# L0SG/grouped-ssd-pytorch

Measured on AMD Instinct MI355X. Metric: 512x512 4-phase CT img/s (fwd+loss), higher is better.
Workload: dtype f32; 1 GPU; gssdpp (BASELINE configs[2], GSSD++: self-attention + SA-base + 1 DCN layer x 4 deformable groups, dcn_cat_sab) fwd + MultiBoxLoss, train-mode BN, batch 32, [B,12,300,300] slices; batch_per_gpu=32, global_batch=32

## Files before the change

### grouped-ssd-pytorch_amd/gssd/_lib.py

```python
import ctypes as C
import os

import torch

_HERE = os.path.dirname(os.path.abspath(__file__))
LIB_PATH = os.environ.get('GSSD_LIB_PATH') or os.path.join(_HERE, 'lib', 'libgssd_hip.so')

c_fp = C.c_void_p
c_i = C.c_int
c_f = C.c_float
c_d = C.c_double
c_i64 = C.c_int64


class ConvDesc(C.Structure):
    _fields_ = [
        ('in_', c_fp), ('wgt', c_fp), ('bias', c_fp), ('out', c_fp), ('out_b', c_fp), ('alpha', c_fp),
        ('gate', c_fp), ('resid', c_fp), ('out2', c_fp), ('in_scale', c_fp), ('in_shift', c_fp), ('in_pad', c_fp),
        ('stats', c_fp), ('wgt_wino', c_fp), ('pool_sign', c_fp), ('wgt_x6', c_fp), ('wgt_patch', c_fp),
        ('B', c_i), ('H', c_i), ('W', c_i), ('in_stride', c_i), ('in_ch_off', c_i), ('Ho', c_i), ('Wo', c_i),
        ('Cout', c_i), ('groups', c_i), ('cin_g', c_i), ('KH', c_i), ('KW', c_i), ('stride', c_i), ('pad', c_i),
        ('dil', c_i), ('K', c_i), ('wgt_row_stride', c_i), ('out_stride', c_i), ('out_ch_off', c_i),
        ('out_mode', c_i), ('relu', c_i), ('m_per_image', c_i), ('split_n', c_i), ('split_k', c_i),
        ('out_b_stride', c_i), ('flags', c_i), ('stats_rep', c_i),
        ('in_batch_stride', c_i64), ('wgt_batch_stride', c_i64), ('out_batch_stride', c_i64),
        ('outb_batch_stride', c_i64), ('out_off', c_i64), ('outb_off', c_i64),
    ]


class DcnGeom(C.Structure):
    _fields_ = [(n, C.c_int32) for n in ('B', 'H', 'W', 'C', 'x_stride', 'Ho', 'Wo', 'kh', 'kw', 'sh', 'sw', 'ph', 'pw', 'dh', 'dw', 'dg',
                                         'off_stride', 'mask_stride', 'mask_logit')]


class PlanOp(C.Structure):
    _fields_ = [('kind', c_i), ('fn', c_i), ('stream', c_i), ('nargs', c_i), ('args', C.c_uint64 * 24)]


PLAN_LAUNCH, PLAN_WAIT = 0, 1


class SnItem(C.Structure):
    _fields_ = [('w', c_fp), ('u', c_fp), ('v', c_fp), ('inv_sigma', c_fp), ('rows', c_i), ('cols', c_i)]


OUT_NHWC, OUT_TRANSPOSED, OUT_HEADS, OUT_SPLIT_T = 0, 1, 2, 3
CONV_OUT_F32, CONV_OUTB_BF16_PERM32, CONV_HEADS_SLICES, CONV_POOL2, CONV_RESID_F32, CONV_F16_OK = 1, 2, 4, 8, 16, 32
CONV_IN_NCHW3, CONV_OUT_GROUPCAT = 64, 128

SIGNATURES = {
    'gssd_abi_version': (c_i, []),
    'gssd_event_create': (c_i, [C.POINTER(C.c_void_p)]),
    'gssd_event_destroy': (c_i, [c_fp]),
    'gssd_event_record_node': (c_i, [c_fp, c_fp]),
    'gssd_event_elapsed_ms': (c_i, [c_fp, c_fp, C.POINTER(C.c_float)]),
    'gssd_conv_desc_size': (c_i, []),
    'gssd_last_error': (C.c_char_p, []),
    'gssd_build_arch': (C.c_char_p, []),
    'gssd_pack_input_nhwc': (c_i, [c_fp, c_fp, c_i, c_i, c_i, c_i, c_i, c_i, c_fp]),
    'gssd_unpack_nhwc_to_nchw': (c_i, [c_fp, c_fp, c_i, c_i, c_i, c_i, c_i, c_fp]),
    'gssd_pack_conv_weight': (c_i, [c_fp, c_fp, c_i, c_i, c_i, c_i, c_i, c_i, c_fp]),
    'gssd_conv2d_nhwc_f32': (c_i, [C.POINTER(ConvDesc), c_fp]),
    'gssd_conv2d_nhwc_bf16': (c_i, [C.POINTER(ConvDesc), c_fp]),
    'gssd_conv_x6_tile': (c_i, [c_i, c_i, c_i64]),
    'gssd_conv_x6_weight_elems': (c_i64, [c_i, c_i, c_i, c_i, c_i]),
    'gssd_conv_x6_pack_weight': (c_i, [c_fp, c_fp, c_i, c_i, c_i, c_i, c_i, c_i, c_fp]),
    'gssd_conv_x6_takes': (c_i, [C.POINTER(ConvDesc)]),
    'gssd_conv_wino_x6_takes': (c_i, [C.POINTER(ConvDesc)]),
    'gssd_conv_thin_x6_takes': (c_i, [C.POINTER(ConvDesc)]),
    'gssd_conv_thin_nchw3_takes': (c_i, [C.POINTER(ConvDesc)]),
    'gssd_plan_fn_count': (c_i, []),
    'gssd_plan_fn_name': (C.c_char_p, [c_i]),
    'gssd_plan_fn_index': (c_i, [C.c_char_p]),
    'gssd_plan_fn_nargs': (c_i, [c_i]),
    'gssd_plan_op_size': (c_i, []),
    'gssd_plan_run': (c_i, [C.POINTER(PlanOp), c_i, C.POINTER(c_fp), c_i, C.POINTER(c_i)]),
    'gssd_pack_conv_weight_bf16': (c_i, [c_fp, c_fp, c_i, c_i, c_i, c_i, c_i, c_i, c_fp]),
    'gssd_cast_f32_bf16': (c_i, [c_fp, c_fp, c_i64, c_fp]),
    'gssd_cast_rows_f32_bf16': (c_i, [c_fp, c_fp, c_i64, c_i, c_i, c_i, c_fp]),
    'gssd_transpose_cast_f32_bf16': (c_i, [c_fp, c_fp, c_i64, c_i, c_i64, c_i64, c_fp]),
    'gssd_cast_bf16_f32': (c_i, [c_fp, c_fp, c_i64, c_fp]),
    'gssd_pack_input_nhwc_bf16': (c_i, [c_fp, c_fp, c_i, c_i, c_i, c_i, c_i, c_fp]),
    'gssd_bn_relu_pool_bf16': (c_i, [c_fp, c_fp, c_i, c_i, c_i, c_i, c_i, c_i, c_i, c_i, c_i, c_fp, c_d, c_fp, c_fp,
                                     c_fp, c_fp, c_f, c_f, c_i, c_i, c_i, c_fp]),
    'gssd_bn_finalize_bf16': (c_i, [c_fp, c_d, c_fp, c_fp, c_fp, c_fp, c_f, c_f, c_i, c_i, c_fp, c_fp, c_fp, c_i, c_fp]),
    'gssd_l2norm_bf16': (c_i, [c_fp, c_fp, c_fp, c_i64, c_i, c_f, c_fp]),
    'gssd_dcn_packed_weight_elems_bf16': (C.c_longlong, [c_i, c_i]),
    'gssd_dcn_pack_weight_bf16': (c_i, [c_fp, c_fp, c_i, c_i, c_i, c_fp]),
    'gssd_dcn_forward_bf16': (c_i, [c_fp, c_fp, c_fp, c_fp, c_fp, c_i, c_i, c_i, c_i, c_i, c_i, c_i, c_fp]),
    'gssd_winograd_weight_elems': (C.c_longlong, [c_i, c_i, c_i]),
    'gssd_winograd_weight_f32': (c_i, [c_fp, c_fp, c_i, c_i, c_i, c_i, c_fp]),
    'gssd_conv2d_wgrad_f32': (c_i, [C.POINTER(ConvDesc), c_fp, c_fp, c_fp]),
    'gssd_conv2d_wgrad_bf16': (c_i, [C.POINTER(ConvDesc), c_fp, c_fp, c_fp]),
    'gssd_conv2d_wgrad_bf16_supported': (c_i, [C.POINTER(ConvDesc)]),
    'gssd_unpack_conv_weight_grad': (c_i, [c_fp, c_fp, c_i, c_i, c_i, c_i, c_i, c_i, c_i, c_fp]),
    'gssd_pack_conv_weight_dgrad': (c_i, [c_fp, c_fp, c_i, c_i, c_i, c_i, c_i, c_fp]),
    'gssd_bn_relu_pool_f32': (c_i, [c_fp, c_fp, c_i, c_i, c_i, c_i, c_i, c_i, c_i, c_i, c_i, c_fp, c_d, c_fp, c_fp,
                                    c_fp, c_fp, c_f, c_f, c_i, c_i, c_i, c_fp]),
    'gssd_bn_finalize_f32': (c_i, [c_fp, c_d, c_fp, c_fp, c_fp, c_fp, c_f, c_f, c_i, c_i, c_fp, c_fp, c_fp, c_i, c_fp]),
    'gssd_bn_bwd_reduce_f32': (c_i, [c_fp, c_fp, c_fp, c_fp, c_fp, c_fp, c_i, c_i, c_i, c_i, c_i, c_i, c_i, c_i, c_i, c_i, c_fp]),
    'gssd_bn_bwd_finalize_f32': (c_i, [c_fp, c_d, c_fp, c_fp, c_f, c_i, c_fp, c_fp, c_fp, c_fp, c_fp, c_i, c_fp]),
    'gssd_bn_bwd_apply_f32': (c_i, [c_fp, c_fp, c_fp, c_fp, c_fp, c_i64, c_i, c_fp, c_fp]),
    'gssd_bn_bwd_reduce_mixed': (c_i, [c_fp, c_i, c_fp, c_fp, c_fp, c_fp, c_fp, c_fp, c_i, c_i, c_i, c_i, c_i, c_i, c_i, c_i, c_i, c_i, c_fp]),
    'gssd_bn_bwd_apply_mixed': (c_i, [c_fp, c_i, c_fp, c_fp, c_fp, c_fp, c_fp, c_i, c_fp, c_fp, c_fp, c_i64, c_i, c_fp, c_i, c_fp]),
    'gssd_bn_bwd_apply_masked_f32': (c_i, [c_fp, c_fp, c_fp, c_fp, c_i, c_fp, c_fp, c_fp, c_fp, c_i64, c_i, c_fp, c_fp]),
    'gssd_colsum_f32': (c_i, [c_fp, c_i64, c_i, c_i, c_fp, c_fp]),
    'gssd_cast_f64_f32': (c_i, [c_fp, c_fp, c_i, c_i, c_fp]),
    'gssd_l2norm_bwd_f32': (c_i, [c_fp, c_fp, c_fp, c_fp, c_fp, c_fp, c_i64, c_i, c_f, c_fp]),
    'gssd_heads_gather_f32': (c_i, [c_fp, c_fp, c_fp, c_i, c_i, c_i, c_i, c_i, c_i, c_fp]),
    'gssd_upsample_insert_f32': (c_i, [c_fp, c_fp, c_i, c_i, c_i, c_i, c_i, c_i, c_i, c_fp]),
    'gssd_l2norm_f32': (c_i, [c_fp, c_fp, c_fp, c_i64, c_i, c_f, c_fp]),
    'gssd_self_attn_core_f32': (c_i, [c_fp, c_fp, c_fp, c_i, c_i, c_i, c_i, c_i, c_i, c_fp]),
    'gssd_self_attn_core_kv_f32': (c_i, [c_fp, c_fp, c_fp, c_fp, c_i, c_i, c_i, c_i, c_i, c_i, c_i, c_i, c_fp, c_fp]),
    'gssd_sa_pool_kv_f32': (c_i, [c_fp, c_fp, c_fp, c_fp, c_i, c_i, c_i, c_i, c_i, c_i, c_i, c_fp]),
    'gssd_sa_unpool_f32': (c_i, [c_fp, c_fp, c_i, c_i, c_i, c_i, c_i, c_fp]),
    'gssd_pack_conv_weights_batched': (c_i, [c_fp, c_i, c_fp]),
    'gssd_gemm_slot_takes': (c_i, [c_fp]),
    'gssd_conv_flat_bf16_takes': (c_i, [c_fp]),
    'gssd_conv_flat_bf16_tile': (c_i, [c_i]),
    'gssd_heads_reduce_f32': (c_i, [c_fp, c_fp, c_fp, c_i, c_i, c_i, c_fp]),
    'gssd_interp_add_f32': (c_i, [c_fp, c_fp, c_fp, c_fp, c_i, c_i, c_i, c_i, c_i, c_i, c_fp]),
    'gssd_pixellink_final_f32': (c_i, [c_fp, c_fp, c_fp, c_fp, c_i, c_fp, c_fp, c_fp, c_fp, c_fp, c_fp, c_i, c_i, c_fp]),
    'gssd_pixellink_loss_f32': (c_i, [c_fp, c_fp, c_fp, c_fp, c_fp, c_fp, c_fp, c_fp, c_i, c_i, c_i, c_i, c_fp]),
    'gssd_interp_add_bwd_f32': (c_i, [c_fp, c_fp, c_fp, c_fp, c_i, c_i, c_i, c_i, c_i, c_i, c_i, c_fp]),
    'gssd_pixellink_final_bwd_f32': (c_i, [c_fp] * 6 + [c_i, c_fp, c_fp, c_fp, c_fp, c_fp, c_fp, c_i, c_fp, c_fp, c_i, c_i, c_i, c_fp]),
    'gssd_pixellink_loss_bwd_f32': (c_i, [c_fp] * 10 + [c_i, c_i, c_i, c_fp]),
    'gssd_pixellink_decode_f32': (c_i, [c_fp, c_fp, c_fp, c_fp, c_fp, c_i, c_i, c_i, C.c_float, C.c_float, c_i, c_fp]),
    'gssd_self_attn_flash_bwd_bf16': (c_i, [c_fp, c_fp, c_fp, c_fp, c_fp, c_fp, c_fp, c_fp, c_i, c_i, c_i, c_i, c_fp]),
    'gssd_cast_split_f32_bf16': (c_i, [c_fp, c_fp, c_fp, c_i64, c_fp]),
    'gssd_self_attn_flash_bwd_supported': (c_i, [c_i, c_i]),
    'gssd_self_attn_core_x6_supported': (c_i, [c_i, c_i]),
    'gssd_self_attn_core_x6_ws_bytes': (C.c_longlong, [c_i, c_i, c_i, c_i]),
    'gssd_self_attn_core_x6_f32': (c_i, [c_fp, c_fp, c_fp, c_i, c_i, c_i, c_i, c_i, c_fp, c_fp, c_fp]),
    'gssd_self_attn_core_bf16v': (c_i, [c_fp, c_fp, c_fp, c_i, c_i, c_i, c_i, c_i, c_fp, c_fp]),
    'gssd_softmax_rows_f32': (c_i, [c_fp, c_i64, c_i, c_i, c_fp]),
    'gssd_slice_and_cat_f32': (c_i, [c_fp, c_fp, c_fp, c_i64, c_i, c_i, c_i, c_fp]),
    'gssd_spectral_norm_f32': (c_i, [c_fp, c_i, c_i, c_f, c_fp]),
    'gssd_dcn_im2col_f32': (c_i, [c_fp, c_fp, c_fp, c_i, c_i, c_i, c_i, c_i, c_i, c_fp]),
    'gssd_dcn_im2col_bf16': (c_i, [c_fp, c_fp, c_fp, c_i, c_i, c_i, c_i, c_i, c_i, c_fp]),
    'gssd_dcn_packed_weight_elems_x6': (C.c_longlong, [c_i, c_i]),
    'gssd_dcn_pack_weight_x6': (c_i, [c_fp, c_fp, c_i, c_i, c_i, c_fp]),
    'gssd_dcn_forward_x6': (c_i, [c_fp, c_fp, c_fp, c_fp, c_fp, c_i, c_i, c_i, c_i, c_i, c_i, c_i, c_fp]),
    'gssd_conv_patch_x6_weight_elems': (C.c_longlong, [c_i, c_i]),
    'gssd_conv_patch_x6_pack_weight': (c_i, [c_fp, c_fp, c_i, c_i, c_i, c_fp]),
    'gssd_conv_patch_x6_takes': (c_i, [C.POINTER(ConvDesc)]),
    'gssd_dcn_forward_x6_ex': (c_i, [c_fp, c_fp, c_fp, c_fp, c_fp, c_i, c_i, c_i, c_i, c_i, c_i, c_i, c_i, c_fp]),
    'gssd_dcn_packed_weight_elems': (C.c_longlong, [c_i, c_i]),
    'gssd_dcn_pack_weight_f32': (c_i, [c_fp, c_fp, c_i, c_i, c_i, c_fp]),
    'gssd_dcn_streamk': (c_i, [c_i]),
    'gssd_dcn_streamk_status': (c_i, [c_fp]),
    'gssd_dcn_streamk_reset': (c_i, [c_fp]),
    'gssd_dcn_streamk_release': (c_i, [c_fp]),
    'gssd_dcn_forward_f32': (c_i, [c_fp, c_fp, c_fp, c_fp, c_fp, c_i, c_i, c_i, c_i, c_i, c_i, c_i, c_fp]),
    'gssd_resample_ksize': (c_i, [c_i, c_i, c_i]),
    'gssd_resample_coeffs': (c_i, [c_i, c_i, c_i, c_fp, c_fp]),
    'gssd_resize_u8_horizontal': (c_i, [c_fp, c_fp, c_fp, c_fp, c_i, c_i, c_i, c_i, c_i, c_i, c_fp]),
    'gssd_resize_u8_vertical': (c_i, [c_fp, c_fp, c_fp, c_fp, c_i, c_i, c_i, c_i, c_i, c_i, c_i, c_fp, c_fp]),
    'gssd_input_finish_f32': (c_i, [c_fp, c_fp, c_f, c_f, c_f, c_fp, c_i, c_i, c_i, c_i, c_i, c_fp]),
    'gssd_aug_desc_size': (c_i, []),
    'gssd_augment_minmax': (c_i, [c_fp, c_i, c_i, c_i, c_fp, c_fp]),
    'gssd_augment_horizontal': (c_i, [c_fp, c_fp, c_fp, c_f, c_f, c_f, c_fp, c_i, c_i, c_i, c_i, c_i, c_fp]),
    'gssd_augment_vertical': (c_i, [c_fp, c_fp, c_fp, c_fp, c_i, c_i, c_i, c_fp]),
    'gssd_pixellink_targets': (c_i, [c_fp, c_fp, c_i, c_i, c_i, c_fp, c_fp, c_fp, c_fp, c_fp]),
    'gssd_pixellink_final5_f32': (c_i, [c_fp] * 5 + [c_i] + [c_fp] * 6 + [c_i, c_i, c_fp]),
    'gssd_pixellink_final5_bwd_f32': (c_i, [c_fp] * 7 + [c_i] + [c_fp] * 7 + [c_i, c_fp, c_fp, c_i, c_i, c_i, c_fp]),
    'gssd_self_attn_flash_bwd_f32_supported': (c_i, [c_i, c_i]),
    'gssd_self_attn_flash_bwd_f32': (c_i, [c_fp, c_i, c_fp, c_i, c_fp, c_i, c_fp, c_fp, c_fp, c_fp, c_i, c_fp, c_fp, c_i, c_i, c_i, c_i, c_i,
                                           c_i, c_fp]),
    'gssd_eval_match': (c_i, [c_fp, C.c_longlong, c_i, c_i, c_fp, c_fp, c_fp, c_i, c_d, c_fp, c_i, c_i, c_fp, c_fp, c_fp]),
    'gssd_eval_workspace_bytes': (C.c_longlong, [c_i]),
    'gssd_eval_ap': (c_i, [c_fp, c_fp, c_i, c_i, c_d, c_i, c_fp, C.c_longlong, c_fp, c_fp]),
    'gssd_bgemm_f32': (c_i, [c_fp, c_fp, c_fp, c_i, c_i, c_i, c_i, c_i, c_i, c_i, c_i, C.c_longlong, C.c_longlong, C.c_longlong, c_i, c_f,
                             c_i, c_fp]),
    'gssd_softmax_bwd_rows_f32': (c_i, [c_fp, c_fp, c_i64, c_i, c_i, c_fp]),
    'gssd_sn_weight_grad_f32': (c_i, [c_fp, c_i, c_fp, c_fp, c_fp, c_fp, c_fp, c_fp, c_fp, c_i, c_i, c_fp]),
    'gssd_scaled_transpose_f32': (c_i, [c_fp, c_fp, c_fp, c_i, c_i, c_fp]),
    'gssd_dot_f32': (c_i, [c_fp, c_fp, c_i64, c_fp, c_fp]),
    'gssd_rowdot_f32': (c_i, [c_fp, c_fp, c_fp, c_i64, c_i, c_fp]),
    'gssd_bgemm_ex_f32': (c_i, [c_fp, c_fp, c_fp, c_i, c_i, c_i, c_i, c_i, c_i, c_i, c_i, C.c_longlong, C.c_longlong, C.c_longlong, c_i, c_f,
                                c_i, c_fp, c_fp, c_fp]),
    'gssd_axpby_f32': (c_i, [c_fp, c_fp, c_fp, c_i64, c_f, c_f, c_fp]),
    'gssd_scale_cast_f64_f32': (c_i, [c_fp, c_fp, c_fp, c_i, c_fp]),
    'gssd_sa_sigma_grad_f32': (c_i, [c_fp, c_fp, c_fp, c_i, c_fp, c_fp]),
    'gssd_dcn_col2im_f32': (c_i, [c_fp, c_fp, c_fp, c_fp, c_fp, c_i, c_i, c_i, c_i, c_i, c_i, c_fp]),
    'gssd_dcn_geo_im2col_f32': (c_i, [c_fp, c_fp, c_fp, c_fp, C.POINTER(DcnGeom), c_i, c_i, c_fp]),
    'gssd_dcn_geo_col2im_f32': (c_i, [c_fp] * 7 + [C.POINTER(DcnGeom), c_i, c_i, c_fp]),
    'gssd_match_batch': (c_i, [c_fp, c_fp, c_fp, c_i, c_i, c_f, c_f, c_f, c_fp, c_fp, c_fp]),
    'gssd_reduce_max_f32': (c_i, [c_fp, c_i64, c_fp, c_i, c_fp]),
    'gssd_hnm_loss': (c_i, [c_fp, c_fp, c_fp, c_fp, c_fp, c_i, c_i, c_i, c_i, c_i, c_fp, c_fp, c_fp, c_fp]),
    'gssd_loss_finalize': (c_i, [c_fp, c_i, c_fp, c_fp, c_fp]),
    'gssd_loss_finalize_global': (c_i, [c_fp, c_i, c_fp, c_i, c_fp, c_fp, c_fp]),
    'gssd_loss_backward': (c_i, [c_fp, c_fp, c_fp, c_fp, c_fp, c_fp, c_fp, c_fp, c_i, c_i, c_i, c_fp, c_fp, c_fp]),
    'gssd_detect': (c_i, [c_fp, c_fp, c_fp, c_i, c_i, c_i, c_i, c_f, c_f, c_f, c_f, c_i, c_i, c_fp, c_fp, c_fp, c_fp]),
    'gssd_softmax_lastdim_f32': (c_i, [c_fp, c_fp, c_i64, c_i, c_fp]),
}


class GssdError(RuntimeError):
    pass


def _load():
    if not os.path.exists(LIB_PATH):
        raise GssdError(
            f'{LIB_PATH} is missing: the HIP kernels are not built.  Run `make -C '
            f'{os.path.join(_HERE, "csrc")}` (needs hipcc, --offload-arch=gfx950) or '
            f'`python -c "import __graft_entry__ as g; g.build()"`.  There is no CPU fallback.')
    lib = C.CDLL(LIB_PATH)
    for name, (res, args) in SIGNATURES.items():
        try:
            fn = getattr(lib, name)
        except AttributeError as e:
            raise GssdError(f'{LIB_PATH} does not export {name}; rebuild it') from e
        fn.restype = res
        fn.argtypes = args
    if lib.gssd_plan_op_size() != C.sizeof(PlanOp):
        raise GssdError(f'{LIB_PATH}: struct gssd_plan_op is {lib.gssd_plan_op_size()} bytes in the library, {C.sizeof(PlanOp)} in this '
                        f'binding; rebuild the library')
    if lib.gssd_conv_desc_size() != C.sizeof(ConvDesc):
        raise GssdError(f'{LIB_PATH}: struct gssd_conv_desc is {lib.gssd_conv_desc_size()} bytes in the library, '
                        f'{C.sizeof(ConvDesc)} in this binding; rebuild the library')
    return lib


lib = _load()


def check(rc):
    if rc != 0:
        raise GssdError(f'libgssd_hip: error {rc}: {lib.gssd_last_error().decode()}')
```

### grouped-ssd-pytorch_amd/gssd/csrc/conv_bf16.hip

```cpp
#include <stdlib.h>
#include "common.h"
#include "kernel_util.h"

namespace {

constexpr int BK = 64;

__device__ __attribute__((aligned(16))) u16 g_zero_page_h[8] = {0, 0, 0, 0, 0, 0, 0, 0};

template <int BN>
__device__ __forceinline__ int tile_chan_of_row(int row) { return BN < 32 ? row : chan_of_row(row); }

template <int BM, int BN, int WM, int WN, int NSTG>
__global__ __launch_bounds__(WM * WN * 64) void conv_bf16_kernel(const gssd_conv_desc p, const int M, const int tiles_per_group) {
    extern __shared__ __attribute__((aligned(16))) u16 smem_h[];
    constexpr int WTM = BM / WM, WTN = BN / WN, MT = WTM / 16, NT = WTN / 16;
    constexpr int NW = WM * WN, NTHR = NW * 64;
    constexpr int AR = BM / (8 * NW);
    constexpr int BPIECES = BN / 8;
    constexpr int BR = (BPIECES + NW - 1) / NW;
    constexpr int STAGE = (BM + BN) * BK;
    static_assert(NT == 1 || NT % 2 == 0, "channel pairing needs an even tile count per wave");

    const int tid = threadIdx.x, lane = tid & 63;
// ... 308 lines not shown

    if (p.stats) {
        __syncthreads();
        float* red = reinterpret_cast<float*>(smem_h);
#pragma unroll
        for (int u = 0; u < NG; ++u)
#pragma unroll
            for (int c = 0; c < CPL; ++c) {
                float s = ssum[u][c], q = ssq[u][c];
#pragma unroll
                for (int o = 1; o < 16; o <<= 1) {
                    s += __shfl_xor(s, o, 64);
                    q += __shfl_xor(q, o, 64);
                }
                if (r == 0) {
                    const int cl = wn * WTN + (NT == 1 ? 4 * kq : 32 * u + 8 * kq) + c;
                    red[(wm * BN + cl) * 2 + 0] = s;
                    red[(wm * BN + cl) * 2 + 1] = q;
                }
            }
        __syncthreads();
        if (tid < BN && n0g + tid < cout_g) {
            double s = 0.0, q = 0.0;
#pragma unroll
            for (int w = 0; w < WM; ++w) {
                s += (double)red[(w * BN + tid) * 2 + 0];
                q += (double)red[(w * BN + tid) * 2 + 1];
            }
            const int n = g * cout_g + n0g + tid;
            double* st = gssd_stats_replica(p.stats, p.stats_rep, p.Cout);
            unsafeAtomicAdd(st + n, s);
            unsafeAtomicAdd(st + p.Cout + n, q);
        }
    }
}

template <int BM, int BN, int WM, int WN, int NSTG = 2>
int launch_cfg(const gssd_conv_desc& d, int M, int images, hipStream_t stream) {
    static unsigned attr_mask = 0;
    constexpr size_t smem_base = NSTG * (size_t)(BM + BN) * BK * sizeof(u16);
    const size_t smem = smem_base + (d.in_scale ? 2 * (size_t)d.cin_g * sizeof(float) : 0);
    auto kern = conv_bf16_kernel<BM, BN, WM, WN, NSTG>;
    if (const int rc = gssd_max_dynamic_lds(&attr_mask, kern, smem_base + 8192)) return rc;
    const int cout_g = d.Cout / d.groups;
    const int tiles = (cout_g + BN - 1) / BN;
    const int mtiles = (M + BM - 1) / BM;
    dim3 grid = d.m_per_image ? dim3(mtiles, d.groups * tiles, images) : dim3((mtiles + 7) / 8 * 8 * d.groups * tiles, 1, d.split_k);
    hipLaunchKernelGGL(kern, grid, dim3(WM * WN * 64), smem, stream, d, M, tiles);
    GSSD_CHECK_LAUNCH();
    return GSSD_OK;
}

__global__ void pack_weight_bf16_kernel(const float* __restrict__ w, u16* __restrict__ wp, int Cout, int cin_g, int KH, int KW,
                                        int cin_g_pad, int Kpad) {
    const long long total = (long long)Cout * Kpad;
    for (long long i = blockIdx.x * (long long)blockDim.x + threadIdx.x; i < total; i += (long long)gridDim.x * blockDim.x) {
        const int k = (int)(i % Kpad), n = (int)(i / Kpad);
        const int tap = k / cin_g_pad, c = k - tap * cin_g_pad;
        float v = 0.f;
        if (tap < KH * KW && c < cin_g) v = w[((size_t)n * cin_g + c) * KH * KW + tap];
        wp[i] = f2bf(v);
    }
}

__global__ void cast_f32_bf16_kernel(const float* __restrict__ x, u16* __restrict__ y, long long n) {
    for (long long i = blockIdx.x * (long long)blockDim.x + threadIdx.x; i < n; i += (long long)gridDim.x * blockDim.x) y[i] = f2bf(x[i]);
}

__global__ void cast_bf16_f32_kernel(const u16* __restrict__ x, float* __restrict__ y, long long n) {
    const long long n8 = n >> 3;
    for (long long i = blockIdx.x * (long long)blockDim.x + threadIdx.x; i < n8; i += (long long)gridDim.x * blockDim.x) {
        const bf16x8 v = *reinterpret_cast<const bf16x8*>(x + 8 * i);
        f32x4 a, b;
#pragma unroll
        for (int e = 0; e < 4; ++e) {
            a[e] = (float)v[e];
            b[e] = (float)v[e + 4];
        }
        *reinterpret_cast<f32x4*>(y + 8 * i) = a;
        *reinterpret_cast<f32x4*>(y + 8 * i + 4) = b;
    }
    if (blockIdx.x == 0 && threadIdx.x < (n & 7)) y[8 * n8 + threadIdx.x] = bf2f(x[8 * n8 + threadIdx.x]);
}

__global__ void cast_split_bf16_kernel(const float* __restrict__ x, u16* __restrict__ hi, u16* __restrict__ lo, long long n) {
    for (long long i = blockIdx.x * (long long)blockDim.x + threadIdx.x; i < n; i += (long long)gridDim.x * blockDim.x) {
        const float v = x[i];
        const u16 h = f2bf(v);
        hi[i] = h;
        lo[i] = f2bf(v - bf2f(h));
    }
}

__global__ void cast_rows_bf16_kernel(const float* __restrict__ x, u16* __restrict__ y, long long rows, int cols, int ld_x, int ld_y) {
    const long long total = rows * ld_y;
    for (long long i = blockIdx.x * (long long)blockDim.x + threadIdx.x; i < total; i += (long long)gridDim.x * blockDim.x) {
        const long long r = i / ld_y;
        const int c = (int)(i - r * ld_y);
        y[i] = c < cols ? f2bf(x[r * ld_x + c]) : (u16)0;
    }
}

}

extern "C" int gssd_cast_split_f32_bf16(const float* x, void* hi, void* lo, int64_t n, gssd_stream_t stream) {
    GSSD_CHECK_ARG(x && hi && lo && n > 0);
    hipLaunchKernelGGL(cast_split_bf16_kernel, dim3((int)((n + 255) / 256 > 8192 ? 8192 : (n + 255) / 256)), dim3(256), 0, as_stream(stream), x,
                       reinterpret_cast<u16*>(hi), reinterpret_cast<u16*>(lo), (long long)n);
    GSSD_CHECK_LAUNCH();
    return GSSD_OK;
}

extern "C" int gssd_cast_rows_f32_bf16(const float* x, void* y, int64_t rows, int cols, int ld_x, int ld_y, gssd_stream_t stream) {
    GSSD_CHECK_ARG(x && y && rows > 0 && cols > 0 && ld_x >= cols && ld_y >= cols);
    const long long total = rows * ld_y;
    hipLaunchKernelGGL(cast_rows_bf16_kernel, dim3((int)((total + 255) / 256 > 8192 ? 8192 : (total + 255) / 256)), dim3(256), 0,
                       as_stream(stream), x, reinterpret_cast<u16*>(y), (long long)rows, cols, ld_x, ld_y);
    GSSD_CHECK_LAUNCH();
    return GSSD_OK;
}

extern "C" int gssd_cast_bf16_f32(const void* x, float* y, int64_t n, gssd_stream_t stream) {
    GSSD_CHECK_ARG(x && y && n > 0 && ((uintptr_t)x % 16) == 0 && ((uintptr_t)y % 16) == 0);
    const long long thr = (n / 8 + 255) / 256;
    hipLaunchKernelGGL(cast_bf16_f32_kernel, dim3((int)(thr > 16384 ? 16384 : (thr < 1 ? 1 : thr))), dim3(256), 0, as_stream(stream),
                       reinterpret_cast<const u16*>(x), y, (long long)n);
    GSSD_CHECK_LAUNCH();
    return GSSD_OK;
}

extern "C" int gssd_pack_conv_weight_bf16(const float* w_oihw, void* w_packed, int Cout, int cin_g, int KH, int KW, int cin_g_pad,
                                          int Kpad, gssd_stream_t stream) {
    GSSD_CHECK_ARG(w_oihw && w_packed && Cout > 0 && cin_g > 0 && KH > 0 && KW > 0 && cin_g_pad >= cin_g && cin_g_pad % 8 == 0);
    GSSD_CHECK_ARG(Kpad >= KH * KW * cin_g_pad && Kpad % 8 == 0);
    const long long total = (long long)Cout * Kpad;
    hipLaunchKernelGGL(pack_weight_bf16_kernel, dim3((int)((total + 255) / 256 > 8192 ? 8192 : (total + 255) / 256)), dim3(256), 0,
                       as_stream(stream), w_oihw, reinterpret_cast<u16*>(w_packed), Cout, cin_g, KH, KW, cin_g_pad, Kpad);
    GSSD_CHECK_LAUNCH();
    return GSSD_OK;
}

extern "C" int gssd_cast_f32_bf16(const float* x, void* y, int64_t n, gssd_stream_t stream) {
    GSSD_CHECK_ARG(x && y && n > 0);
    hipLaunchKernelGGL(cast_f32_bf16_kernel, dim3((int)((n + 255) / 256 > 8192 ? 8192 : (n + 255) / 256)), dim3(256), 0,
                       as_stream(stream), x, reinterpret_cast<u16*>(y), (long long)n);
    GSSD_CHECK_LAUNCH();
    return GSSD_OK;
}

extern "C" int gssd_conv2d_nhwc_bf16(const gssd_conv_desc* dp, gssd_stream_t stream) {
    GSSD_CHECK_ARG(dp != nullptr);
    const gssd_conv_desc& d = *dp;
    GSSD_CHECK_ARG(d.in && d.wgt && d.out);
    GSSD_CHECK_ARG(!(d.flags & (GSSD_CONV_IN_NCHW3 | GSSD_CONV_OUT_GROUPCAT)));
    GSSD_CHECK_ARG(d.B > 0 && d.H > 0 && d.W > 0 && d.Ho > 0 && d.Wo > 0);
    GSSD_CHECK_ARG(d.groups > 0 && d.Cout > 0 && d.Cout % d.groups == 0);
    GSSD_CHECK_ARG(d.cin_g > 0 && d.cin_g % 8 == 0 && d.in_stride % 8 == 0 && d.in_ch_off % 8 == 0);
    GSSD_CHECK_ARG(d.KH > 0 && d.KW > 0 && d.stride > 0 && d.dil > 0 && d.pad >= 0);
    GSSD_CHECK_ARG(d.K == d.KH * d.KW * d.cin_g && d.wgt_row_stride >= d.K && d.wgt_row_stride % 8 == 0);
    GSSD_CHECK_ARG(((uintptr_t)d.in % 16) == 0 && ((uintptr_t)d.wgt % 16) == 0 && ((uintptr_t)d.out % 16) == 0);
    GSSD_CHECK_ARG(d.out_mode >= 0 && d.out_mode <= 3);
    const bool out_f32 = (d.flags & GSSD_CONV_OUT_F32) != 0;
    if (d.out_mode == GSSD_OUT_TRANSPOSED)
        GSSD_CHECK_ARG(d.m_per_image && out_f32 && d.out_stride % 4 == 0 && d.out_batch_stride % 4 == 0 && !d.gate && !d.resid);
    if (d.out_mode == GSSD_OUT_HEADS) GSSD_CHECK_ARG(d.out_b && d.split_n > 0 && d.split_n < d.Cout && !d.m_per_image && out_f32);
    if (d.out_mode == GSSD_OUT_SPLIT_T) {
        GSSD_CHECK_ARG(d.m_per_image && d.groups == 1 && d.out_b && d.split_n > 0 && d.split_n < d.Cout && d.split_n % 64 == 0 && out_f32);
        GSSD_CHECK_ARG(d.out_b_stride % 4 == 0 && d.out_b_stride >= d.Ho * d.Wo && d.outb_batch_stride % 4 == 0);
        if (d.flags & GSSD_CONV_OUTB_BF16_PERM32) GSSD_CHECK_ARG(d.out_b_stride % 32 == 0 && d.outb_batch_stride % 8 == 0);
        GSSD_CHECK_ARG(!d.gate && !d.resid && !d.relu && !d.stats && d.split_k == 1);
    }
    if (d.out_mode == GSSD_OUT_NHWC) GSSD_CHECK_ARG((d.out_stride % 8 == 0 && d.out_ch_off % 8 == 0) || out_f32);
    if (d.m_per_image) GSSD_CHECK_ARG(d.in_batch_stride % 8 == 0 && d.wgt_batch_stride % 8 == 0);
    GSSD_CHECK_ARG(d.split_k >= 1 && d.split_k <= 64);
    GSSD_CHECK_ARG((d.in_scale == nullptr) == (d.in_shift == nullptr) && (d.in_scale == nullptr) == (d.in_pad == nullptr));
    if (d.split_k > 1)
        GSSD_CHECK_ARG(out_f32 && !d.m_per_image && !d.stats && !d.relu && !d.gate && !d.resid &&
                       (d.out_mode == GSSD_OUT_HEADS || d.out_mode == GSSD_OUT_NHWC));
    GSSD_CHECK_ARG((d.H + 2 * d.pad - d.dil * (d.KH - 1) - 1) / d.stride + 1 == d.Ho);
    GSSD_CHECK_ARG((d.W + 2 * d.pad - d.dil * (d.KW - 1) - 1) / d.stride + 1 == d.Wo);
    const int images = d.m_per_image ? d.B : 1;
    const long long Mll = (long long)(d.m_per_image ? 1 : d.B) * d.Ho * d.Wo;
    GSSD_CHECK_ARG(Mll < (1ll << 31));
    GSSD_CHECK_ARG((long long)(d.m_per_image ? 1 : d.B) * d.H * d.W * d.in_stride < (1ll << 31));
    GSSD_CHECK_ARG((long long)(d.Cout / d.groups + 256) * d.wgt_row_stride < (1ll << 31));
    const int M = (int)Mll;
    const int cout_g = d.Cout / d.groups;
    hipStream_t s = as_stream(stream);
    {
        const int rc = gssd_try_conv_thin_bf16(d, s);
        if (rc != 1) return rc;
    }
    if (d.flags & GSSD_CONV_POOL2) {
        gssd_set_error("GSSD_CONV_POOL2: no bf16 kernel with a pooled epilogue takes this descriptor (thin trunk shapes only)");
        return GSSD_EINVAL;
    }
    {
        const int rc = gssd_try_conv_flat_bf16(d, s);
        if (rc != 1) return rc;
    }
    if (d.in_scale) GSSD_CHECK_ARG(d.cin_g <= 1024 && !d.m_per_image);
    static const bool no_small = getenv("GSSD_NO_SMALL_TILES") != nullptr;
    if (!no_small && cout_g > 32 && d.split_k == 1 && !(d.out_mode == GSSD_OUT_SPLIT_T && d.split_n % 64 != 0)) {
        const long long mtot = (long long)M * images;
        if (mtot <= 512 || (d.m_per_image && mtot <= 4096 && M <= 128)) return launch_cfg<32, 64, 1, 4, 3>(d, M, images, s);
        if (mtot <= 4096) return launch_cfg<64, 64, 2, 2, 3>(d, M, images, s);
    }
    static const int big = [] { const char* e = getenv("GSSD_BF16_BIG_TILES"); return e ? atoi(e) : 0; }();
    if (big && !d.m_per_image && d.split_k == 1 && M >= 8192 && cout_g % 128 == 0 && d.K % BK == 0 && d.K >= 256 &&
        (d.out_mode == GSSD_OUT_NHWC || (d.out_mode == GSSD_OUT_SPLIT_T && d.split_n % 128 == 0))) {
        if (big == 2) return launch_cfg<256, 128, 4, 2, 3>(d, M, images, s);
        if (big == 3) return launch_cfg<192, 128, 4, 2, 3>(d, M, images, s);
        if (big == 4) return launch_cfg<128, 128, 2, 2, 4>(d, M, images, s);
        if (big == 5) return launch_cfg<128, 128, 2, 2, 3>(d, M, images, s);
        if (big == 6) return launch_cfg<128, 128, 4, 2, 4>(d, M, images, s);
        return launch_cfg<256, 128, 4, 2>(d, M, images, s);
    }
    if (cout_g > 64) {
        const long long mt = (M + 127) / 128, z = d.m_per_image ? images : d.split_k;
        const long long b128 = mt * d.groups * ((cout_g + 127) / 128) * z, b64 = mt * d.groups * ((cout_g + 63) / 64) * z;
        const double e128 = (double)b128 / (double)(((b128 + 511) / 512) * 512);
        const double e64 = 0.94 * (double)b64 / (double)(((b64 + 767) / 768) * 768);
        if (e64 > e128 || d.K <= 256 || (d.out_mode == GSSD_OUT_SPLIT_T && d.split_n % 128 != 0)) return launch_cfg<128, 64, 2, 2>(d, M, images, s);
        return launch_cfg<128, 128, 2, 2>(d, M, images, s);
    }
    if (cout_g > 32) return launch_cfg<128, 64, 2, 2>(d, M, images, s);
    if (cout_g > 16) return launch_cfg<128, 32, 4, 1>(d, M, images, s);
    return launch_cfg<128, 16, 4, 1>(d, M, images, s);
}
```

### grouped-ssd-pytorch_amd/gssd/csrc/conv_igemm.hip

```cpp
#include <stdlib.h>
#include "common.h"
#include "kernel_util.h"

namespace {

constexpr int BK = 32;

__device__ __attribute__((aligned(16))) float g_zero_page[4] = {0.f, 0.f, 0.f, 0.f};

template <int BM, int BN, int WM, int WN, int NSTG>
__global__ __launch_bounds__(WM * WN * 64) void conv_igemm_kernel(const gssd_conv_desc p, const int M,
                                                         const int tiles_per_group) {
    extern __shared__ __attribute__((aligned(16))) float smem[];
    constexpr int WTM = BM / WM, WTN = BN / WN, MT = WTM / 16, NT = WTN / 16;
    constexpr int NW = WM * WN, NTHR = NW * 64;
    constexpr int AR = BM / (8 * NW);
    constexpr int BPIECES = BN / 8;
    constexpr int BR = (BPIECES + NW - 1) / NW;
    constexpr int STAGE = (BM + BN) * BK;

    const int tid = threadIdx.x, lane = tid & 63;
    const int wave = __builtin_amdgcn_readfirstlane(tid >> 6);
    const int wm = wave / WN, wn = wave % WN;
    const int r = lane & 15, kq = lane >> 4;
// ... 204 lines not shown
                    f32x4 o;
#pragma unroll
                    for (int e = 0; e < 4; ++e) o[e] = (mb + e < M) ? v[e] : 0.f;
                    *reinterpret_cast<f32x4*>(p.out_b + (size_t)bi * p.outb_batch_stride + (size_t)(n - p.split_n) * p.out_b_stride + ml) = o;
                }
            } else if (p.out_mode == GSSD_OUT_TRANSPOSED) {
                if (mb < p.out_stride) {
                    f32x4 o;
#pragma unroll
                    for (int e = 0; e < 4; ++e) {
                        float t = v[e];
                        if (p.relu) t = fmaxf(t, 0.f);
                        o[e] = (mb + e < M) ? t : 0.f;
                    }
                    *reinterpret_cast<f32x4*>(p.out + (size_t)img * p.out_batch_stride + (size_t)n * p.out_stride + mb) = o;
                }
            } else {
#pragma unroll
                for (int e = 0; e < 4; ++e) {
                    const int m = mb + e;
                    if (m >= M) continue;
                    float t = v[e];
                    if (p.out_mode == GSSD_OUT_HEADS) {
                        const int b = m / HoWo, pix = m - b * HoWo;
                        float* dst = (n < p.split_n)
                                         ? p.out + ((size_t)b * p.out_batch_stride + p.out_off + (size_t)pix * p.split_n + n)
                                         : p.out_b + ((size_t)b * p.outb_batch_stride + p.outb_off +
                                                      (size_t)pix * (p.Cout - p.split_n) + (n - p.split_n));
                        if (p.flags & GSSD_CONV_HEADS_SLICES) {
                            dst[(size_t)kz * ((n < p.split_n) ? (size_t)p.B * p.out_batch_stride
                                                                   : (size_t)p.B * p.outb_batch_stride)] = t;
                        } else if (p.split_k > 1) {
                            unsafeAtomicAdd(dst, t);
                        } else {
                            *dst = t;
                        }
                    } else {
                        const size_t o = (size_t)img * p.out_batch_stride + (size_t)m * p.out_stride + p.out_ch_off + n;
                        if (p.gate) {
                            t *= gate;
                            if (p.out2) p.out2[o] = t;
                            if (p.resid) t += p.resid[o];
                        } else if (p.resid) {
                            t += p.resid[o];
                        }
                        if (p.relu) t = fmaxf(t, 0.f);
                        if (p.split_k > 1) unsafeAtomicAdd(p.out + o, t);
                        else p.out[o] = t;
                    }
                }
            }
        }
    }

    if (p.stats) {
        __syncthreads();
        float* red = smem;
#pragma unroll
        for (int j = 0; j < NT; ++j) {
            float s = ssum[j], q = ssq[j];
            s += __shfl_xor(s, 16, 64);
            s += __shfl_xor(s, 32, 64);
            q += __shfl_xor(q, 16, 64);
            q += __shfl_xor(q, 32, 64);
            if (kq == 0) {
                red[(wm * BN + wn * WTN + j * 16 + r) * 2 + 0] = s;
                red[(wm * BN + wn * WTN + j * 16 + r) * 2 + 1] = q;
            }
        }
        __syncthreads();
        if (tid < BN && n0g + tid < cout_g) {
            double s = 0.0, q = 0.0;
#pragma unroll
            for (int w = 0; w < WM; ++w) {
                s += (double)red[(w * BN + tid) * 2 + 0];
                q += (double)red[(w * BN + tid) * 2 + 1];
            }
            const int n = g * cout_g + n0g + tid;
            double* st = gssd_stats_replica(p.stats, p.stats_rep, p.Cout);
            unsafeAtomicAdd(st + n, s);
            unsafeAtomicAdd(st + p.Cout + n, q);
        }
    }
}

template <int BM, int BN, int WM, int WN, int NSTG = 2>
int launch_cfg(const gssd_conv_desc& d, int M, int images, hipStream_t stream) {
    static unsigned attr_mask = 0;
    constexpr size_t smem_base = NSTG * (size_t)(BM + BN) * BK * sizeof(float);
    const size_t smem = smem_base + (d.in_scale ? 2 * (size_t)d.cin_g * sizeof(float) : 0);
    auto kern = conv_igemm_kernel<BM, BN, WM, WN, NSTG>;
    if (const int rc = gssd_max_dynamic_lds(&attr_mask, kern, smem_base + 4096)) return rc;
    const int cout_g = d.Cout / d.groups;
    const int tiles = (cout_g + BN - 1) / BN;
    const int mtiles = (M + BM - 1) / BM;
    dim3 grid = d.m_per_image ? dim3(mtiles, d.groups * tiles, images) : dim3((mtiles + 7) / 8 * 8 * d.groups * tiles, 1, d.split_k);
    static_assert(BM % (8 * WM * WN) == 0, "A rows must split evenly over the waves");
    hipLaunchKernelGGL(kern, grid, dim3(WM * WN * 64), smem, stream, d, M, tiles);
    GSSD_CHECK_LAUNCH();
    return GSSD_OK;
}

}

extern "C" int gssd_conv2d_nhwc_f32(const gssd_conv_desc* dp, gssd_stream_t stream) {
    GSSD_CHECK_ARG(dp != nullptr);
    const gssd_conv_desc& d = *dp;
    GSSD_CHECK_ARG(d.in && d.wgt && d.out);
    GSSD_CHECK_ARG(d.B > 0 && d.H > 0 && d.W > 0 && d.Ho > 0 && d.Wo > 0);
    GSSD_CHECK_ARG(d.groups > 0 && d.Cout > 0 && d.Cout % d.groups == 0);
    GSSD_CHECK_ARG(d.cin_g > 0 && d.cin_g % 4 == 0 && d.in_stride % 4 == 0 && d.in_ch_off % 4 == 0);
    GSSD_CHECK_ARG(d.KH > 0 && d.KW > 0 && d.stride > 0 && d.dil > 0 && d.pad >= 0);
    GSSD_CHECK_ARG(d.K == d.KH * d.KW * d.cin_g && d.wgt_row_stride >= d.K && d.wgt_row_stride % 4 == 0);
    GSSD_CHECK_ARG(((uintptr_t)d.in % ((d.flags & GSSD_CONV_IN_NCHW3) ? 4 : 16)) == 0 && ((uintptr_t)d.wgt % 16) == 0);
    GSSD_CHECK_ARG(d.out_mode >= 0 && d.out_mode <= 3);
    if (d.out_mode == GSSD_OUT_SPLIT_T) {
        GSSD_CHECK_ARG((d.m_per_image || (d.Ho * d.Wo) % 4 == 0) && d.groups == 1 && d.out_b && d.split_n > 0 && d.split_n < d.Cout &&
                       d.split_n % 64 == 0);
        GSSD_CHECK_ARG(d.out_b_stride % 4 == 0 && d.out_b_stride >= d.Ho * d.Wo && d.outb_batch_stride % 4 == 0 && ((uintptr_t)d.out_b % 16) == 0);
        GSSD_CHECK_ARG(!d.gate && !d.resid && !d.relu && !d.stats && d.split_k == 1);
    }
    if (d.out_mode == GSSD_OUT_TRANSPOSED) {
        GSSD_CHECK_ARG(d.m_per_image && d.out_stride % 4 == 0 && ((uintptr_t)d.out % 16) == 0);
        GSSD_CHECK_ARG(d.out_batch_stride % 4 == 0 && !d.gate && !d.resid);
    }
    if (d.out_mode == GSSD_OUT_HEADS) GSSD_CHECK_ARG(d.out_b && d.split_n > 0 && d.split_n < d.Cout && !d.m_per_image);
    if (d.m_per_image) GSSD_CHECK_ARG(d.in_batch_stride % 4 == 0 && d.wgt_batch_stride % 4 == 0);
    GSSD_CHECK_ARG(d.split_k >= 1 && d.split_k <= 64);
    GSSD_CHECK_ARG((d.in_scale == nullptr) == (d.in_shift == nullptr) && (d.in_scale == nullptr) == (d.in_pad == nullptr));
    if (d.split_k > 1) GSSD_CHECK_ARG(!d.m_per_image && !d.stats && !d.relu && !d.gate && !d.resid && d.out_mode != GSSD_OUT_TRANSPOSED);
    GSSD_CHECK_ARG((d.H + 2 * d.pad - d.dil * (d.KH - 1) - 1) / d.stride + 1 == d.Ho);
    GSSD_CHECK_ARG((d.W + 2 * d.pad - d.dil * (d.KW - 1) - 1) / d.stride + 1 == d.Wo);

    const int images = d.m_per_image ? d.B : 1;
    const long long Mll = (long long)(d.m_per_image ? 1 : d.B) * d.Ho * d.Wo;
    GSSD_CHECK_ARG(Mll < (1ll << 31));
    GSSD_CHECK_ARG((long long)(d.m_per_image ? 1 : d.B) * d.H * d.W * d.in_stride < (1ll << 31));
    GSSD_CHECK_ARG((long long)(d.Cout / d.groups + 256) * d.wgt_row_stride < (1ll << 31));
    const int M = (int)Mll;
    const int cout_g = d.Cout / d.groups;
    hipStream_t s = as_stream(stream);
    if (d.flags & GSSD_CONV_IN_NCHW3) {
        const int rc = gssd_try_conv_thin(d, s);
        if (rc != 1) return rc;
        gssd_set_error("GSSD_CONV_IN_NCHW3: not conv1_1's shape (see gssd_conv_thin_nchw3_takes)");
        return GSSD_EINVAL;
    }
    if (d.flags & GSSD_CONV_OUT_GROUPCAT) {
        const int rc = d.wgt_x6 ? gssd_try_conv_x6(d, s) : 1;
        if (rc != 1) return rc;
        gssd_set_error("GSSD_CONV_OUT_GROUPCAT: csrc/conv_x6.hip does not take this descriptor (see gssd_conv_x6_takes)");
        return GSSD_EINVAL;
    }
    if (d.wgt_patch) {
        const int rc = gssd_try_conv_patch_x6(d, s);
        if (rc != 1) return rc;
    }
    if (d.wgt_x6) {
        const int rc = gssd_try_conv_x6(d, s);
        if (rc != 1) return rc;
    }
    {
        const int rc = gssd_try_conv_thin_x6(d, s);
        if (rc != 1) return rc;
    }
    {
        const int rc = gssd_try_conv_thin_wino(d, s);
        if (rc != 1) return rc;
    }
    {
        const int rc = gssd_try_conv_thin(d, s);
        if (rc != 1) return rc;
    }
    {
        const int rc = gssd_try_conv_wino(d, s);
        if (rc != 1) return rc;
    }
    if (d.flags & GSSD_CONV_POOL2) {
        gssd_set_error("GSSD_CONV_POOL2: no fp32 kernel with a pooled epilogue takes this descriptor (Winograd trunk shapes only)");
        return GSSD_EINVAL;
    }
    if (d.in_scale) GSSD_CHECK_ARG(d.cin_g <= 512 && !d.m_per_image);
    {
        static const bool no_slot = getenv("GSSD_NO_GEMM_SLOT") != nullptr;
        const int rc = no_slot ? 1 : gssd_try_gemm_slot(d, s);
        if (rc != 1) return rc;
    }
    static const bool no_small = getenv("GSSD_NO_SMALL_TILES") != nullptr;
    if (!no_small && cout_g > 32 && d.split_k == 1 && !(d.out_mode == GSSD_OUT_SPLIT_T && d.split_n % 64 != 0)) {
        const long long mtot = (long long)M * images;
        if (mtot <= 512 || (d.m_per_image && mtot <= 4096 && M <= 128)) return launch_cfg<32, 64, 1, 4, 3>(d, M, images, s);
        if (mtot <= 4096) return launch_cfg<64, 64, 2, 2, 3>(d, M, images, s);
    }
    if (cout_g > 64) {
        const long long mt = (M + 127) / 128, z = d.m_per_image ? images : d.split_k;
        const long long b128 = mt * d.groups * ((cout_g + 127) / 128) * z, b64 = mt * d.groups * ((cout_g + 63) / 64) * z;
        const double e128 = (double)b128 / (double)(((b128 + 511) / 512) * 512);
        const double e64 = 0.94 * (double)b64 / (double)(((b64 + 767) / 768) * 768);
        if (e64 > e128 || d.K <= 256 || (d.out_mode == GSSD_OUT_SPLIT_T && d.split_n % 128 != 0)) return launch_cfg<128, 64, 2, 2>(d, M, images, s);
        return launch_cfg<128, 128, 2, 2>(d, M, images, s);
    }
    if (cout_g > 32) return launch_cfg<128, 64, 2, 2>(d, M, images, s);
    if (cout_g > 16) return launch_cfg<128, 32, 4, 1>(d, M, images, s);
    return launch_cfg<128, 16, 4, 1>(d, M, images, s);
}
```

### grouped-ssd-pytorch_amd/gssd/csrc/conv_x6.hip

```cpp
#include <stdlib.h>
#include <type_traits>
#include "common.h"
#include "kernel_util.h"

namespace {

#ifndef X6_SCHED
#define X6_SCHED 0
#endif
#ifndef X6_KO
#define X6_KO 0
#endif
#ifndef X6_LOCAL_SUM
#define X6_LOCAL_SUM 1
#endif
constexpr int BM = 128, BKC = 32;
constexpr int NP = 3;
constexpr int A_STAGE = BM * BKC;


#ifndef X6_V2
#define X6_V2 1
#endif

// ... 145 lines not shown
        }
    };

    gather_issue(gvA, gokA, false);
    b_issue(0, 0);
    if (nchunks > 1) advance_ld();
    if (xf) __syncthreads();
#pragma unroll
    for (int part = 0; part < 4; ++part) finish_part(part, gvA, gokA, 0);
    if (nchunks > 1) advance_fin();
    gather_issue(gvA, gokA, false);
    if (nchunks > 2) advance_ld();
    __syncthreads();

    auto chunk = [&](const int ch, f32x4 (&gv_use)[2][2], const bool (&gok_use)[2], f32x4 (&gv_ld)[2][2], bool (&gok_ld)[2]) {
        const int buf = ch & 1;
        const u16* Ab = As + buf * NP * A_STAGE + wm * WTM * BKC + fo;
        const u16* Bb = Bs + (NBS == 2 ? buf : 0) * NP * B_STAGE + wn * WTN * BKC + fo;
        bf16x8 afr[2][NP], bf[NP][NT];
        auto a_row = [&](int i) {
#pragma unroll
            for (int pl = 0; pl < NP; ++pl) {
                if (X6_KO & 16) asm volatile("" : "=v"(afr[i & 1][pl]));
                else afr[i & 1][pl] = *reinterpret_cast<const bf16x8*>(Ab + pl * A_STAGE + i * 16 * BKC);
            }
        };
        a_row(0);
#pragma unroll
        for (int pl = 0; pl < NP; ++pl) {
#pragma unroll
            for (int j = 0; j < NT; ++j) {
                if (X6_KO & 16) {
                    asm volatile("" : "=v"(bf[pl][j]));
                    continue;
                }
                bf[pl][j] = *reinterpret_cast<const bf16x8*>(Bb + pl * B_STAGE + j * 16 * BKC);
            }
        }
        if (NBS == 1) {
            asm volatile("s_waitcnt lgkmcnt(0)" ::: "memory");
            __builtin_amdgcn_s_barrier();
        }
        b_issue(min(ch + 1, nchunks - 1), buf ^ 1);
        __builtin_amdgcn_sched_barrier(0);
        gather_issue(gv_ld, gok_ld, true);
        if (!(X6_KO & 8)) {
            constexpr int YOUNGER = ((X6_KO & 4) ? 0 : NP * (B_STAGE / 512 / 4)) + 4;
            asm volatile("s_waitcnt vmcnt(%4)" : "+v"(gv_use[0][0]), "+v"(gv_use[0][1]), "+v"(gv_use[1][0]), "+v"(gv_use[1][1]) : "n"(YOUNGER));
        }
        __builtin_amdgcn_sched_barrier(0);
#pragma unroll
        for (int i = 0; i < MT; ++i) {
            if (i + 1 < MT) a_row(i + 1);
            const bf16x8 (&af)[NP] = afr[i & 1];
#pragma unroll
            for (int j = 0; j < NT; ++j) {
                if (X6_KO & 2) continue;
#if X6_LOCAL_SUM
                f32x4 c = zero4;
#else
                f32x4 c = acc[i][j];
#endif
                c = __builtin_amdgcn_mfma_f32_16x16x32_bf16(bf[1][j], af[1], c, 0, 0, 0);
                c = __builtin_amdgcn_mfma_f32_16x16x32_bf16(bf[2][j], af[0], c, 0, 0, 0);
                c = __builtin_amdgcn_mfma_f32_16x16x32_bf16(bf[0][j], af[2], c, 0, 0, 0);
                c = __builtin_amdgcn_mfma_f32_16x16x32_bf16(bf[1][j], af[0], c, 0, 0, 0);
                c = __builtin_amdgcn_mfma_f32_16x16x32_bf16(bf[0][j], af[1], c, 0, 0, 0);
                c = __builtin_amdgcn_mfma_f32_16x16x32_bf16(bf[0][j], af[0], c, 0, 0, 0);
#if X6_LOCAL_SUM
#pragma unroll
                for (int e = 0; e < 4; ++e) acc[i][j][e] += c[e];
#else
                acc[i][j] = c;
#endif
            }
            finish_part(i, gv_use, gok_use, buf ^ 1);
        }
#if X6_SCHED
#define X6_ROW(DS_READS)                                                                                                   \
    __builtin_amdgcn_sched_group_barrier(0x100, DS_READS, 0);                     \
    _Pragma("unroll") for (int k = 0; k < NT * 6; ++k) {                                                                   \
        __builtin_amdgcn_sched_group_barrier(0x008, 1, 0);                                                                 \
        __builtin_amdgcn_sched_group_barrier(0x002, BN == 64 ? X6_SCHED + 2 : BN == 128 ? X6_SCHED + 1 : X6_SCHED, 0);     \
    }                                                                                                                      \
    __builtin_amdgcn_sched_group_barrier(0x200, NP, 0);
        static_assert(MT == 4, "the schedule below is written for four fragment rows");
        X6_ROW(NP + (XF ? 2 : 0))
        X6_ROW(NP + (XF ? 2 : 0))
        X6_ROW(NP + (XF ? 2 : 0))
        X6_ROW((XF ? 2 : 0))
#undef X6_ROW
#endif
        __builtin_amdgcn_sched_barrier(0);
        if (ch + 2 < nchunks) advance_fin();
        if (ch + 3 < nchunks) advance_ld();
        if (X6_KO & 8) asm volatile("s_waitcnt vmcnt(0) lgkmcnt(0)\n\ts_barrier" ::: "memory");
        else asm volatile("s_waitcnt vmcnt(4) lgkmcnt(0)\n\ts_barrier" ::: "memory");
    };
    for (int ch = 0; ch < nchunks; ch += 2) {
        chunk(ch, gvA, gokA, gvB, gokB);
        if (ch + 1 < nchunks) chunk(ch + 1, gvB, gokB, gvA, gokA);
    }
    asm volatile("s_waitcnt vmcnt(0)" : "+v"(gvA[0][0]), "+v"(gvA[0][1]), "+v"(gvA[1][0]), "+v"(gvA[1][1]),
                                        "+v"(gvB[0][0]), "+v"(gvB[0][1]), "+v"(gvB[1][0]), "+v"(gvB[1][1]) : : "memory");
    __syncthreads();

    float* red = reinterpret_cast<float*>(smem_h);
    const float gate = p.gate ? *p.gate : 0.f;
    const bool split_t = p.out_mode == GSSD_OUT_SPLIT_T && n0g >= p.split_n;
    const bool gcat = (p.flags & GSSD_CONV_OUT_GROUPCAT) != 0;
#pragma unroll
    for (int u = 0; u < NT / 2; ++u) {
        const int nl = wn * WTN + 32 * u + 8 * kq;
        const int ng = n0g + nl;
        const bool n_ok = ng + 8 <= cout_g;
        const int n = g * cout_g + ng;
        const int ncat = gcat ? (n / p.split_n) * p.split_n : 0;
        float bv[8], av[8], ssum[8], ssq[8];
#pragma unroll
        for (int c = 0; c < 8; ++c) {
            bv[c] = (p.bias && n_ok) ? p.bias[n + c] : 0.f;
            av[c] = (p.alpha && n_ok) ? p.alpha[n + c] : 1.f;
            ssum[c] = ssq[c] = 0.f;
        }
#pragma unroll
        for (int i = 0; i < MT; ++i) {
            const int m = m0 + wm * WTM + i * 16 + r;
            if (m >= M || !n_ok) continue;
            float v[8];
#pragma unroll
            for (int c = 0; c < 8; ++c) {
                v[c] = acc[i][2 * u + (c >> 2)][c & 3] * av[c] + bv[c];
                ssum[c] += v[c];
                ssq[c] += v[c] * v[c];
            }
            if (split_t) {
                const int bi = m / HoWo, ml = m - bi * HoWo;
                float* dst = p.out_b + (size_t)bi * p.outb_batch_stride + (size_t)(n - p.split_n) * p.out_b_stride + ml;
#pragma unroll
                for (int c = 0; c < 8; ++c) dst[(size_t)c * p.out_b_stride] = v[c];
                continue;
            }
            const size_t o = (size_t)m * p.out_stride + p.out_ch_off + n + ncat;
            const size_t ro = gcat ? (size_t)m * p.Cout + n : o;
            if (p.gate) {
#pragma unroll
                for (int c = 0; c < 8; ++c) v[c] *= gate;
                if (p.out2) {
                    *reinterpret_cast<f32x4*>(p.out2 + o) = f32x4{v[0], v[1], v[2], v[3]};
                    *reinterpret_cast<f32x4*>(p.out2 + o + 4) = f32x4{v[4], v[5], v[6], v[7]};
                }
            }
            if (p.resid) {
                const f32x4 r0 = *reinterpret_cast<const f32x4*>(p.resid + ro), r1 = *reinterpret_cast<const f32x4*>(p.resid + ro + 4);
#pragma unroll
                for (int c = 0; c < 4; ++c) {
                    v[c] += r0[c];
                    v[4 + c] += r1[c];
                }
            }
            if (p.relu) {
#pragma unroll
                for (int c = 0; c < 8; ++c) v[c] = fmaxf(v[c], 0.f);
            }
            *reinterpret_cast<f32x4*>(p.out + o) = f32x4{v[0], v[1], v[2], v[3]};
            *reinterpret_cast<f32x4*>(p.out + o + 4) = f32x4{v[4], v[5], v[6], v[7]};
        }
        if (p.stats) {
#pragma unroll
            for (int c = 0; c < 8; ++c) {
                float s = ssum[c], q = ssq[c];
#pragma unroll
                for (int o = 1; o < 16; o <<= 1) {
                    s += __shfl_xor(s, o, 64);
                    q += __shfl_xor(q, o, 64);
                }
                if (r == 0) {
                    red[(wm * BN + nl + c) * 2 + 0] = s;
                    red[(wm * BN + nl + c) * 2 + 1] = q;
                }
            }
        }
    }
    if (p.stats) {
        __syncthreads();
        if (tid < BN && n0g + tid < cout_g) {
            const double s = (double)red[tid * 2 + 0] + (double)red[(BN + tid) * 2 + 0];
            const double q = (double)red[tid * 2 + 1] + (double)red[(BN + tid) * 2 + 1];
            const int n = g * cout_g + n0g + tid;
            double* st = gssd_stats_replica(p.stats, p.stats_rep, p.Cout);
            unsafeAtomicAdd(st + n, s);
            unsafeAtomicAdd(st + p.Cout + n, q);
        }
    }
}

#if X6_V2
template <int BN>
struct Cfg2 {
    static constexpr int WTN = BN / 2, NT = WTN / 16, NTH = NT / 2, MT = 4;
    static constexpr int NG = NTH * MT;
    static constexpr int HB_ROWS = BN / 2, HB_PLANE = HB_ROWS * BKC, HB_ELEMS = NP * HB_PLANE;
    static constexpr int PH = NP * HB_ROWS / 16;
    static constexpr int DPW = 2 * PH / 4;
    static constexpr int NY = (PH + 3) / 4;
    static constexpr int LDS_BYTES = (NP * A_STAGE + 4 * HB_ELEMS) * 2;
    static_assert(BN == 64 || BN == 128, "tiles");
};

template <int BN, bool XF, bool F16>
__global__ __launch_bounds__(256, 2) void conv_x6_v2_kernel(const gssd_conv_desc p, const int M, const int ntn, const int mtiles,
                                                           const long long plane_elems) {
    using K = Cfg2<BN>;
    constexpr int NPL = (F16 && BN == 64) ? 2 : NP;
    constexpr int WTM = 64, WTN = K::WTN, MT = K::MT, NT = K::NT, NTH = K::NTH, NG = K::NG;
    constexpr int PH = NPL * K::HB_ROWS / 16;
    constexpr int DPW = 2 * PH / 4;
    constexpr int NY = (PH + 3) / 4;
    constexpr int HB_PLANE = K::HB_PLANE, HB_ELEMS = K::HB_ELEMS, B_STAGE = BN * BKC;
    extern __shared__ __attribute__((aligned(16))) u16 smem_h[];
    u16* const As = smem_h;
    u16* const Bh = smem_h + NP * A_STAGE;
    float* const xtab = reinterpret_cast<float*>(smem_h + NP * A_STAGE + 4 * HB_ELEMS);
    const int tid = threadIdx.x, lane = tid & 63;
    const int wave = __builtin_amdgcn_readfirstlane(tid >> 6);
    const int wm = wave >> 1, wn = wave & 1;
    const int r = lane & 15, kq = lane >> 4;
    const int ny = p.groups * ntn;
    const int slot = blockIdx.x >> 3;
    const int mt = (slot / ny) * 8 + (blockIdx.x & 7);
    const int by = slot % ny;
    if (mt >= mtiles) return;
    const int g = by / ntn, nt = by - g * ntn;
    const int cout_g = p.Cout / p.groups;
    const int n0g = nt * BN;
    const int m0 = mt * BM;
    const int HoWo = p.Ho * p.Wo;
    const int taps = p.KH * p.KW;
    const int cpc = p.cin_g / BKC;
    const int nchunks = cpc * taps;
    const float* __restrict__ in = p.in + p.in_ch_off + g * p.cin_g;
    const u16* wslab = reinterpret_cast<const u16*>(p.wgt_x6) + (F16 ? 3 * plane_elems : 0) + (size_t)by * nchunks * B_STAGE;
    constexpr bool xf = XF;

    f32x4 acc[MT][NT];
    const f32x4 zero4 = {0.f, 0.f, 0.f, 0.f};
#pragma unroll
    for (int i = 0; i < MT; ++i)
#pragma unroll
        for (int j = 0; j < NT; ++j) acc[i][j] = zero4;

    const int gq = tid & 3, gp = tid >> 2;
    const int a_wr0 = gp * BKC + ((gq ^ swz64(gp)) << 3);
    const int fo = r * BKC + ((kq ^ swz64(r)) << 3);
    int g_iy0[2], g_ix0[2], g_off[2];
#pragma unroll
    for (int j = 0; j < 2; ++j) {
        const int m = m0 + gp + 64 * j;
        const bool ok = m < M;
        const int mm = ok ? m : 0;
        const int b = mm / HoWo, pix = mm - b * HoWo;
        const int oy = pix / p.Wo, ox = pix - oy * p.Wo;
        g_iy0[j] = ok ? oy * p.stride - p.pad : -(1 << 20);
        g_ix0[j] = ox * p.stride - p.pad;
        g_off[j] = ((b * p.H + oy * p.stride - p.pad) * p.W + g_ix0[j]) * p.in_stride + gq * 8;
    }
    if (xf) {
        const float* xsc = p.in_scale + p.in_ch_off + g * p.cin_g;
        const float* xsh = p.in_shift + p.in_ch_off + g * p.cin_g;
        for (int c = tid; c < p.cin_g; c += 256) {
            xtab[c] = xsc[c];
            xtab[p.cin_g + c] = xsh[c];
        }
    }

    int ld_ty = 0, ld_tx = 0, ld_c = 0, ld_tap = 0;
    f32x4 gv[2][2];
    bool gok[2] = {false, false};
    const float* src[2] = {in, in};
    gv[0][0] = gv[0][1] = gv[1][0] = gv[1][1] = zero4;
    auto load_addr = [&]() {
        const int dy = ld_ty * p.dil, dx = ld_tx * p.dil;
        const int toff = (dy * p.W + dx) * p.in_stride + ld_c * BKC;
#pragma unroll
        for (int j = 0; j < 2; ++j) {
            gok[j] = (unsigned)(g_iy0[j] + dy) < (unsigned)p.H && (unsigned)(g_ix0[j] + dx) < (unsigned)p.W;
            src[j] = in + (gok[j] ? g_off[j] + toff : gq * 8);
        }
    };
    auto load_req = [&](int q) {
        if (X6_KO & 8) return;
        const int j = q >> 1;
        if (q & 1) asm volatile("global_load_dwordx4 %0, %1, off offset:16" : "=v"(gv[j][1]) : "v"(src[j]) : "memory");
        else asm volatile("global_load_dwordx4 %0, %1, off" : "=v"(gv[j][0]) : "v"(src[j]) : "memory");
    };
    int fin_c = 0;
    auto advance_ld = [&]() {
        ++ld_tap;
        if (++ld_tx == p.KW) {
            ld_tx = 0;
            ++ld_ty;
        }
        if (ld_tap == taps) {
            ld_tap = ld_ty = ld_tx = 0;
            ++ld_c;
        }
    };
// ... 88 lines not shown
        }
    };
    auto mma_row = [&](int i, int j, int which) {
        if (X6_KO & 2) return;
#if X6_LOCAL_SUM
        f32x4 c = zero4;
#else
        f32x4 c = acc[i][j];
#endif
        if constexpr (F16) {
            c = __builtin_amdgcn_mfma_f32_16x16x32_f16(__builtin_bit_cast(f16x8, breg[which][2]), __builtin_bit_cast(f16x8, areg[i][1]), c, 0, 0, 0);
            c = __builtin_amdgcn_mfma_f32_16x16x32_f16(__builtin_bit_cast(f16x8, breg[which][1]), __builtin_bit_cast(f16x8, areg[i][2]), c, 0, 0, 0);
            c = __builtin_amdgcn_mfma_f32_16x16x32_f16(__builtin_bit_cast(f16x8, breg[which][0]), __builtin_bit_cast(f16x8, areg[i][0]), c, 0, 0, 0);
        } else {
            c = __builtin_amdgcn_mfma_f32_16x16x32_bf16(breg[which][1], areg[i][1], c, 0, 0, 0);
            c = __builtin_amdgcn_mfma_f32_16x16x32_bf16(breg[which][2], areg[i][0], c, 0, 0, 0);
            c = __builtin_amdgcn_mfma_f32_16x16x32_bf16(breg[which][0], areg[i][2], c, 0, 0, 0);
            c = __builtin_amdgcn_mfma_f32_16x16x32_bf16(breg[which][1], areg[i][0], c, 0, 0, 0);
            c = __builtin_amdgcn_mfma_f32_16x16x32_bf16(breg[which][0], areg[i][1], c, 0, 0, 0);
            c = __builtin_amdgcn_mfma_f32_16x16x32_bf16(breg[which][0], areg[i][0], c, 0, 0, 0);
        }
#if X6_LOCAL_SUM
#pragma unroll
        for (int e = 0; e < 4; ++e) acc[i][j][e] += c[e];
#else
        acc[i][j] = c;
#endif
    };
    constexpr int NGQ = (X6_KO & 8) ? 0 : 4, NDQ = (X6_KO & 4) ? 0 : DPW, NYQ = (X6_KO & 4) ? 0 : NY;
#define X6_LOADS_WAIT(N) \
    if (!(X6_KO & 8)) asm volatile("s_waitcnt vmcnt(%4)" : "+v"(gv[0][0]), "+v"(gv[0][1]), "+v"(gv[1][0]), "+v"(gv[1][1]) : "n"(N))

    load_addr();
#pragma unroll
    for (int q = 0; q < 4; ++q) load_req(q);
    if (xf) __syncthreads();
    if (!(X6_KO & 4)) {
        for (int pc = wave; pc < PH; pc += 4) {
            const int pl = pc / (2 * NTH), g8 = pc - pl * (2 * NTH);
            const int G = (g8 / NTH) * NT + (g8 % NTH);
            dma16(wslab + (size_t)pl * plane_elems + G * 512 + lane * 8, Bh + pl * HB_PLANE + g8 * 512);
        }
    }
    asm volatile("s_waitcnt vmcnt(0)" : "+v"(gv[0][0]), "+v"(gv[0][1]), "+v"(gv[1][0]), "+v"(gv[1][1]));
#pragma unroll
    for (int part = 0; part < 4; ++part) finish_part(part);
    if (nchunks > 1) {
        advance_ld();
    }
    asm volatile("s_waitcnt vmcnt(0) lgkmcnt(0)" ::: "memory");
    __syncthreads();

    auto iteration = [&](int it, auto first_c, auto last_c) {
        constexpr bool FIRST = decltype(first_c)::value, LAST = decltype(last_c)::value;
        const int par = it & 1;
        const int cy = min(it, nchunks - 1), cx = min(it + 1, nchunks - 1);
        __builtin_amdgcn_sched_barrier(0);
        if (!FIRST) {
#pragma unroll
            for (int jj = 0; jj < NTH; ++jj) {
                if (jj + 1 == NTH && !LAST) {
                    constexpr int K_B1 = NTH == 1 ? 0 : NYQ + NGQ;
                    if (X6_KO & 64) asm volatile("s_waitcnt vmcnt(%0) lgkmcnt(0)" ::"n"(K_B1) : "memory");
                    else asm volatile("s_waitcnt vmcnt(%0) lgkmcnt(0)\n\ts_barrier" ::"n"(K_B1) : "memory");
                }
                if (jj + 1 < NTH) b_load((jj + 1) & 1, 1, par ^ 1, jj + 1);
#pragma unroll
                for (int i = 0; i < MT; ++i) {
                    const int gidx = jj * MT + i;
                    if (!LAST && gidx == 0) load_addr();
                    if (jj + 1 == NTH && !LAST && i == 0) b_load((jj + 1) & 1, 0, par, 0);
                    mma_row(i, NTH + jj, jj & 1);
                    if (!LAST) {
                        if (NTH == 2) {
                            if (gidx < NY) dma_piece(gidx, cy, cx, par);
                            if (gidx < 4) load_req(gidx);
                            if (gidx >= 4 && gidx < 4 + DPW - NY) dma_piece(gidx - 4 + NY, cy, cx, par);
                        } else {
                            if (gidx < NY) dma_piece(gidx, cy, cx, par);
                            if (gidx < 2) {
                                load_req(2 * gidx);
                                load_req(2 * gidx + 1);
                            }
                            if (gidx >= NY && gidx < DPW) dma_piece(gidx, cy, cx, par);
                        }
                        if (jj + 1 == NTH) a_load_row(i);
                    }
                    __builtin_amdgcn_sched_barrier(0);
                }
            }
        } else {
            load_addr();
#pragma unroll
            for (int q = 0; q < NY; ++q) dma_piece(q, cy, cx, par);
#pragma unroll
            for (int q = 0; q < 4; ++q) load_req(q);
#pragma unroll
            for (int q = NY; q < DPW; ++q) dma_piece(q, cy, cx, par);
#pragma unroll
            for (int i = 0; i < MT; ++i) a_load_row(i);
            b_load(NTH & 1, 0, par, 0);
        }
        if (!LAST) {
#pragma unroll
            for (int jj = 0; jj < NTH; ++jj) {
                if (jj + 1 < NTH) b_load((NTH + jj + 1) & 1, 0, par, jj + 1);
#pragma unroll
                for (int i = 0; i < MT; ++i) {
                    const int gidx = jj * MT + i;
                    mma_row(i, jj, (NTH + jj) & 1);
                    if (gidx == 0) {
                        __builtin_amdgcn_sched_barrier(0);
                        constexpr int K_B2 = NDQ - NYQ;
                        if (X6_KO & 64) asm volatile("s_waitcnt vmcnt(%0) lgkmcnt(0)" ::"n"(K_B2) : "memory");
                        else asm volatile("s_waitcnt vmcnt(%0) lgkmcnt(0)\n\ts_barrier" ::"n"(K_B2) : "memory");
                        X6_LOADS_WAIT(DPW - NY);
                    }
#ifndef X6_FIN
#define X6_FIN 1
#endif
                    if (NTH == 2) {
                        if (X6_FIN) {
                            if (gidx == 1) finish_part(0);
                            if (gidx == 3) finish_part(1);
                            if (gidx == 5) finish_part(2);
                            if (gidx == 7) finish_part(3);
                        } else {
                            if (gidx == 1) finish_part(0);
                            if (gidx == 2) finish_part(1);
                            if (gidx == 4) finish_part(2);
                            if (gidx == 5) finish_part(3);
                        }
                    } else {
                        if (gidx == 1) finish_part(0), finish_part(1);
                        if (gidx == 2) finish_part(2);
                        if (gidx == 3) finish_part(3);
                    }
                    if (gidx == NG - 1) b_load(0, 1, par, 0);
                    if (!(X6_FIN && NTH == 2) || (gidx & 1) == 0 || gidx == NG - 1) __builtin_amdgcn_sched_barrier(0);
                }
            }
            if (it + 2 < nchunks) advance_ld();
            fin_c = ld_c;
        }
    };
    fin_c = ld_c;
    iteration(0, std::true_type{}, std::false_type{});
    for (int it = 1; it < nchunks; ++it) iteration(it, std::false_type{}, std::false_type{});
    iteration(nchunks, std::false_type{}, std::true_type{});
    asm volatile("s_waitcnt vmcnt(0) lgkmcnt(0)" : "+v"(gv[0][0]), "+v"(gv[0][1]), "+v"(gv[1][0]), "+v"(gv[1][1]) : : "memory");
    __syncthreads();
#undef X6_LOADS_WAIT

    float* red = reinterpret_cast<float*>(smem_h);
    const float gate = p.gate ? *p.gate : 0.f;
    const bool split_t = p.out_mode == GSSD_OUT_SPLIT_T && n0g >= p.split_n;
    const bool gcat = (p.flags & GSSD_CONV_OUT_GROUPCAT) != 0;
#pragma unroll
    for (int u = 0; u < NT / 2; ++u) {
        const int nl = wn * WTN + 32 * u + 8 * kq;
        const int ng = n0g + nl;
        const bool n_ok = ng + 8 <= cout_g;
        const int n = g * cout_g + ng;
        const int ncat = gcat ? (n / p.split_n) * p.split_n : 0;
        float bv[8], av[8], ssum[8], ssq[8];
#pragma unroll
        for (int c = 0; c < 8; ++c) {
            bv[c] = (p.bias && n_ok) ? p.bias[n + c] : 0.f;
            av[c] = (p.alpha && n_ok) ? p.alpha[n + c] : 1.f;
            ssum[c] = ssq[c] = 0.f;
        }
#pragma unroll
        for (int i = 0; i < MT; ++i) {
            const int m = m0 + wm * WTM + i * 16 + r;
            if (m >= M || !n_ok) continue;
            float v[8];
#pragma unroll
            for (int c = 0; c < 8; ++c) {
                v[c] = acc[i][2 * u + (c >> 2)][c & 3] * av[c] + bv[c];
                ssum[c] += v[c];
                ssq[c] += v[c] * v[c];
            }
            if (split_t) {
                const int bi = m / HoWo, ml = m - bi * HoWo;
                float* dst = p.out_b + (size_t)bi * p.outb_batch_stride + (size_t)(n - p.split_n) * p.out_b_stride + ml;
#pragma unroll
                for (int c = 0; c < 8; ++c) dst[(size_t)c * p.out_b_stride] = v[c];
                continue;
            }
            const size_t o = (size_t)m * p.out_stride + p.out_ch_off + n + ncat;
            const size_t ro = gcat ? (size_t)m * p.Cout + n : o;
            if (p.gate) {
#pragma unroll
                for (int c = 0; c < 8; ++c) v[c] *= gate;
                if (p.out2) {
                    *reinterpret_cast<f32x4*>(p.out2 + o) = f32x4{v[0], v[1], v[2], v[3]};
                    *reinterpret_cast<f32x4*>(p.out2 + o + 4) = f32x4{v[4], v[5], v[6], v[7]};
                }
            }
            if (p.resid) {
                const f32x4 r0 = *reinterpret_cast<const f32x4*>(p.resid + ro), r1 = *reinterpret_cast<const f32x4*>(p.resid + ro + 4);
#pragma unroll
                for (int c = 0; c < 4; ++c) {
                    v[c] += r0[c];
                    v[4 + c] += r1[c];
                }
            }
            if (p.relu) {
#pragma unroll
                for (int c = 0; c < 8; ++c) v[c] = fmaxf(v[c], 0.f);
            }
            *reinterpret_cast<f32x4*>(p.out + o) = f32x4{v[0], v[1], v[2], v[3]};
            *reinterpret_cast<f32x4*>(p.out + o + 4) = f32x4{v[4], v[5], v[6], v[7]};
        }
        if (p.stats) {
#pragma unroll
            for (int c = 0; c < 8; ++c) {
                float s = ssum[c], q = ssq[c];
#pragma unroll
                for (int o = 1; o < 16; o <<= 1) {
                    s += __shfl_xor(s, o, 64);
                    q += __shfl_xor(q, o, 64);
                }
                if (r == 0) {
                    red[(wm * BN + nl + c) * 2 + 0] = s;
                    red[(wm * BN + nl + c) * 2 + 1] = q;
                }
            }
        }
    }
    if (p.stats) {
        __syncthreads();
        if (tid < BN && n0g + tid < cout_g) {
            const double s = (double)red[tid * 2 + 0] + (double)red[(BN + tid) * 2 + 0];
            const double q = (double)red[tid * 2 + 1] + (double)red[(BN + tid) * 2 + 1];
            const int n = g * cout_g + n0g + tid;
            double* st = gssd_stats_replica(p.stats, p.stats_rep, p.Cout);
            unsafeAtomicAdd(st + n, s);
            unsafeAtomicAdd(st + p.Cout + n, q);
        }
    }
}

#endif

__global__ void conv_x6_pack_kernel(const float* __restrict__ w, u16* __restrict__ wp, int Cout, int groups, int cin_g, int taps, int row_stride,
                                    int BN, long long total) {
    const int cout_g = Cout / groups, ntn = (cout_g + BN - 1) / BN, nchunks = (cin_g / BKC) * taps;
    for (long long i = blockIdx.x * (long long)blockDim.x + threadIdx.x; i < total; i += (long long)gridDim.x * blockDim.x) {
        const int e = (int)(i & 7);
        const int slot = (int)((i >> 3) & 3);
        const int row = (int)((i >> 5) % BN);
        long long t = (i >> 5) / BN;
        const int chunk = (int)(t % nchunks);
        t /= nchunks;
        const int nt = (int)(t % ntn), g = (int)(t / ntn);
        const int q = slot ^ swz64(row);
        const int tap = chunk % taps, c32 = chunk / taps;
        const int c = c32 * BKC + q * 8 + e;
        const int ng = nt * BN + chan_of_row(row);
        const float v = ng < cout_g ? w[(size_t)(g * cout_g + ng) * row_stride + tap * cin_g + c] : 0.f;
        __bf16 h, m, l;
        split3(v, h, m, l);
        wp[i] = __builtin_bit_cast(u16, h);
        wp[i + total] = __builtin_bit_cast(u16, m);
        wp[i + 2 * total] = __builtin_bit_cast(u16, l);
        const _Float16 fh = (_Float16)v;
        wp[i + 3 * total] = __builtin_bit_cast(u16, fh);
        wp[i + 4 * total] = __builtin_bit_cast(u16, (_Float16)((v - (float)fh) * 64.f));
        wp[i + 5 * total] = __builtin_bit_cast(u16, (_Float16)(fh * (_Float16)0.015625f));
    }
}

template <int BN, bool XF>
int launch(const gssd_conv_desc& d, int M, hipStream_t stream) {
    static unsigned attr_mask = 0;
    auto kern = conv_x6_kernel<BN, XF>;
    if (const int rc = gssd_max_dynamic_lds(&attr_mask, kern, Cfg<BN>::LDS_BYTES + 4096)) return rc;
    const int cout_g = d.Cout / d.groups;
    const int ntn = (cout_g + BN - 1) / BN, mtiles = (M + BM - 1) / BM;
    const long long plane = (long long)d.groups * ntn * BN * d.KH * d.KW * d.cin_g;
    hipLaunchKernelGGL(kern, dim3((mtiles + 7) / 8 * 8 * d.groups * ntn), dim3(256), Cfg<BN>::LDS_BYTES + (d.in_scale ? 8 * d.cin_g : 0), stream, d, M, ntn, mtiles, plane);
    GSSD_CHECK_LAUNCH();
    return GSSD_OK;
}

#if X6_V2
template <int BN, bool XF, bool F16>
int launch2_impl(const gssd_conv_desc& d, int M, hipStream_t stream) {
    static unsigned attr_mask = 0;
    auto kern = conv_x6_v2_kernel<BN, XF, F16>;
    constexpr int lds = Cfg2<BN>::LDS_BYTES;
    if (const int rc = gssd_max_dynamic_lds(&attr_mask, kern, lds + 4096)) return rc;
    const int cout_g = d.Cout / d.groups;
    const int ntn = (cout_g + BN - 1) / BN, mtiles = (M + BM - 1) / BM;
    const long long plane = (long long)d.groups * ntn * BN * d.KH * d.KW * d.cin_g;
    hipLaunchKernelGGL(kern, dim3((mtiles + 7) / 8 * 8 * d.groups * ntn), dim3(256), lds + (d.in_scale ? 8 * d.cin_g : 0), stream, d, M, ntn, mtiles, plane);
    GSSD_CHECK_LAUNCH();
    return GSSD_OK;
}
template <int BN, bool XF>
int launch2(const gssd_conv_desc& d, int M, hipStream_t stream) {
    if (gssd_x6_f16_enabled() && (d.flags & GSSD_CONV_F16_OK)) return launch2_impl<BN, XF, true>(d, M, stream);
    return launch2_impl<BN, XF, false>(d, M, stream);
}
#endif

bool shape_ok(int cin_g, int cout_g, int groups) {
    return cin_g > 0 && cin_g % BKC == 0 && cout_g >= 32 && cout_g % 8 == 0 && groups > 0;
}

}

extern "C" int gssd_conv_x6_tile(int cout_g, int groups, long long M) {
    static const int forced = getenv("GSSD_X6_BN") ? atoi(getenv("GSSD_X6_BN")) : 0;
    if (forced == 64 || forced == 128 || forced == 256) return forced;
    (void)groups;
    (void)M;
    return cout_g > 64 ? 128 : 64;
}

extern "C" long long gssd_conv_x6_weight_elems(int Cout, int groups, int cin_g, int taps, int BN) {
    if (Cout <= 0 || groups <= 0 || Cout % groups != 0 || taps <= 0 || !(BN == 64 || BN == 128 || BN == 256)) return -1;
    if (!shape_ok(cin_g, Cout / groups, groups)) return -1;
    const int cout_g = Cout / groups;
    return 6ll * groups * ((cout_g + BN - 1) / BN) * BN * taps * cin_g;
}

extern "C" int gssd_conv_x6_pack_weight(const float* w_packed, void* w_x6, int Cout, int groups, int cin_g, int taps, int row_stride, int BN,
                                        gssd_stream_t stream) {
    const long long n = gssd_conv_x6_weight_elems(Cout, groups, cin_g, taps, BN);
    GSSD_CHECK_ARG(w_packed && w_x6 && n > 0 && row_stride >= taps * cin_g);
    const long long total = n / 6;
    hipLaunchKernelGGL(conv_x6_pack_kernel, dim3((int)((total + 255) / 256 > 16384 ? 16384 : (total + 255) / 256)), dim3(256), 0,
                       as_stream(stream), w_packed, reinterpret_cast<u16*>(w_x6), Cout, groups, cin_g, taps, row_stride, BN, total);
    GSSD_CHECK_LAUNCH();
    return GSSD_OK;
}

extern "C" int gssd_conv_x6_takes(const gssd_conv_desc* dp) {
    if (!dp) return 0;
    const gssd_conv_desc& d = *dp;
    if (!d.wgt_x6 || d.groups <= 0 || d.Cout % d.groups != 0) return 0;
    if (!shape_ok(d.cin_g, d.Cout / d.groups, d.groups)) return 0;
    if (d.split_k > 1 || (d.flags & ~(GSSD_CONV_OUT_F32 | GSSD_CONV_F16_OK | GSSD_CONV_OUT_GROUPCAT)) || (d.out2 && !d.gate)) return 0;
    if (d.flags & GSSD_CONV_OUT_GROUPCAT) {
        if (d.out_mode != GSSD_OUT_NHWC || d.groups != 1 || d.m_per_image || d.relu || d.stats || d.split_n <= 0 || d.split_n % 8 != 0 ||
            d.Cout % d.split_n != 0 || d.out_stride < 2 * d.Cout)
            return 0;
    }
    if (d.out_mode == GSSD_OUT_SPLIT_T) {
        const int bn = gssd_conv_x6_tile(d.Cout / d.groups, d.groups, (long long)d.B * d.Ho * d.Wo);
        if (d.groups != 1 || !d.out_b || d.split_n <= 0 || d.split_n % bn != 0 || d.out_b_stride < d.Ho * d.Wo) return 0;
    } else if (d.out_mode != GSSD_OUT_NHWC) {
        return 0;
    }
    if (d.m_per_image) {
        if (d.wgt_batch_stride != 0 || d.in_batch_stride != (long long)d.H * d.W * d.in_stride ||
            d.out_batch_stride != (long long)d.Ho * d.Wo * d.out_stride)
            return 0;
    }
    if ((d.resid && ((uintptr_t)d.resid % 16)) || (d.out2 && ((uintptr_t)d.out2 % 16))) return 0;
    if (d.in_stride % 4 || d.in_ch_off % 4 || d.out_stride % 4 || d.out_ch_off % 4) return 0;
    if (((uintptr_t)d.in % 16) || ((uintptr_t)d.out % 16) || ((uintptr_t)d.wgt_x6 % 16)) return 0;
    if ((long long)d.B * d.H * d.W * d.in_stride >= (1ll << 31)) return 0;
    if (d.in_scale && d.cin_g > 512) return 0;
    return 1;
}

int gssd_try_conv_x6(const gssd_conv_desc& d, hipStream_t stream) {
    if (!gssd_conv_x6_takes(&d)) return 1;
    const long long Mll = (long long)d.B * d.Ho * d.Wo;
    const int M = (int)Mll;
    switch (gssd_conv_x6_tile(d.Cout / d.groups, d.groups, Mll)) {
#if X6_V2
        case 64: return d.in_scale ? launch2<64, true>(d, M, stream) : launch2<64, false>(d, M, stream);
        case 128: return d.in_scale ? launch2<128, true>(d, M, stream) : launch2<128, false>(d, M, stream);
#else
        case 64: return d.in_scale ? launch<64, true>(d, M, stream) : launch<64, false>(d, M, stream);
        case 128: return d.in_scale ? launch<128, true>(d, M, stream) : launch<128, false>(d, M, stream);
#endif
        default: return d.in_scale ? launch<256, true>(d, M, stream) : launch<256, false>(d, M, stream);
    }
}
```

### grouped-ssd-pytorch_amd/gssd/csrc/flash_attn_x6.hip

```cpp
#include <math.h>
#include <stdlib.h>
#include "common.h"
#include "kernel_util.h"

namespace {

constexpr int NP = 3;

__device__ __attribute__((aligned(16))) u16 g_zero16_x6[8] = {0, 0, 0, 0, 0, 0, 0, 0};

template <bool F16>
__global__ void split_planes_kernel(const float* __restrict__ in, u16* __restrict__ out, long long rows, int cols, int ld_in, int cols_out,
                                    long long plane, int perm32) {
    const long long i = blockIdx.x * (long long)blockDim.x + threadIdx.x;
    const int units = cols_out >> 3;
    if (i >= rows * units) return;
    const long long row = i / units;
    const int u = (int)(i - row * units);
    const float* src = in + row * ld_in;
    bf16x8 h, m, l;
#pragma unroll
    for (int e = 0; e < 8; ++e) {
        int c = 8 * u + e;
        if (perm32) {
// ... 140 lines not shown
        float mx = -INFINITY;
#pragma unroll
        for (int kt = 0; kt < KT; ++kt)
#pragma unroll
            for (int e = 0; e < 4; ++e) {
                if (key0 + kt * 16 + 4 * kq + e >= N) s[kt][e] = -INFINITY;
                mx = fmaxf(mx, s[kt][e]);
            }
        mx = fmaxf(mx, __shfl_xor(mx, 16, 64));
        mx = fmaxf(mx, __shfl_xor(mx, 32, 64));
        const float m_new = fmaxf(m_run, mx);
        const float alpha = __expf(m_run - m_new);
        float psum = 0.f;
        bf16x8 pb[KB][NPX];
        if constexpr (F16) {
#pragma unroll
            for (int kb = 0; kb < KB; ++kb) {
                u32x4 ph, pl;
#pragma unroll
                for (int e2 = 0; e2 < 4; ++e2) {
                    const float p0 = __expf(s[2 * kb + (e2 >> 1)][(2 * e2) & 3] - m_new), p1 = __expf(s[2 * kb + (e2 >> 1)][(2 * e2 + 1) & 3] - m_new);
                    psum += p0;
                    psum += p1;
                    const f32x2 ps = f32x2{p0, p1} * 1024.f;
                    unsigned h, l;
                    split2_pair(ps[0], ps[1], h, l);
                    ph[e2] = h;
                    pl[e2] = l;
                }
                pb[kb][0] = __builtin_bit_cast(bf16x8, ph);
                pb[kb][1] = __builtin_bit_cast(bf16x8, pl);
            }
        } else {
#pragma unroll
            for (int kb = 0; kb < KB; ++kb)
#pragma unroll
                for (int e = 0; e < 8; ++e) {
                    const float p = __expf(s[2 * kb + (e >> 2)][e & 3] - m_new);
                    psum += p;
                    __bf16 h, m, l;
                    split3(p, h, m, l);
                    pb[kb][0][e] = h;
                    pb[kb][1][e] = m;
                    pb[kb][NPX - 1][e] = l;
                }
        }
        l_run = l_run * alpha + psum;
        m_run = m_new;
        if (__any(alpha != 1.f)) {
#pragma unroll
            for (int c = 0; c < CT; ++c) o[c] *= alpha;
        }
#pragma unroll
        for (int c = 0; c < CT; ++c) {
            const int row = c * 16 + r;
            f32x4 acc = zero4, accx = zero4;
#pragma unroll
            for (int kb = 0; kb < KB; ++kb) {
                bf16x8 vf[NPX];
                const int unit = (4 * kb + kq) ^ (BKV == 32 ? ((row & 8) ? 3 : 0) : (row & 7));
#pragma unroll
                for (int pl = 0; pl < NPX; ++pl) vf[pl] = *reinterpret_cast<const bf16x8*>(Vs + pl * V_PLANE + row * BKV + (unit << 3));
                if constexpr (F16) {
                    accx = __builtin_amdgcn_mfma_f32_16x16x32_f16(__builtin_bit_cast(f16x8, vf[1]), __builtin_bit_cast(f16x8, pb[kb][0]), accx, 0, 0, 0);
                    accx = __builtin_amdgcn_mfma_f32_16x16x32_f16(__builtin_bit_cast(f16x8, vf[0]), __builtin_bit_cast(f16x8, pb[kb][1]), accx, 0, 0, 0);
                    acc = __builtin_amdgcn_mfma_f32_16x16x32_f16(__builtin_bit_cast(f16x8, vf[0]), __builtin_bit_cast(f16x8, pb[kb][0]), acc, 0, 0, 0);
                } else {
                    acc = __builtin_amdgcn_mfma_f32_16x16x32_bf16(vf[1], pb[kb][1], acc, 0, 0, 0);
                    acc = __builtin_amdgcn_mfma_f32_16x16x32_bf16(vf[NPX - 1], pb[kb][0], acc, 0, 0, 0);
                    acc = __builtin_amdgcn_mfma_f32_16x16x32_bf16(vf[0], pb[kb][NPX - 1], acc, 0, 0, 0);
                    acc = __builtin_amdgcn_mfma_f32_16x16x32_bf16(vf[1], pb[kb][0], acc, 0, 0, 0);
                    acc = __builtin_amdgcn_mfma_f32_16x16x32_bf16(vf[0], pb[kb][1], acc, 0, 0, 0);
                    acc = __builtin_amdgcn_mfma_f32_16x16x32_bf16(vf[0], pb[kb][0], acc, 0, 0, 0);
                }
            }
#pragma unroll
            for (int e = 0; e < 4; ++e) o[c][e] += F16 ? __builtin_fmaf(accx[e], 1.f / 2048.f, acc[e]) : acc[e];
            if (F16 && (c & 1)) __builtin_amdgcn_sched_barrier(0);
            if (FX6_SPREAD)
#pragma unroll
                for (int j = 0; j < VW; ++j)
                    if (j * (3 * CT / 4) / VW == c) {
                        __builtin_amdgcn_sched_barrier(0);
                        stage_piece(tn, buf ^ 1, KW + j);
                        __builtin_amdgcn_sched_barrier(0);
                    }
        }
    }
    l_run += __shfl_xor(l_run, 16, 64);
    l_run += __shfl_xor(l_run, 32, 64);
    const float inv = (F16 ? 1.f / 1024.f : 1.f) / l_run;
    if (lse != nullptr && q < N && kq == 0) lse[(size_t)b * N + q] = m_run + logf(l_run);
    if (q < N) {
        float* dst = out + ((size_t)b * N + q) * C2 + 4 * kq;
#pragma unroll
        for (int c = 0; c < CT; ++c) *reinterpret_cast<f32x4*>(dst + 16 * c) = o[c] * inv;
    }
}

template <int D, int C2, int BKV, int NW, bool F16>
int launch_x6(const u16* tpp, const u16* gp, float* out, int B, int N, int Np32, float* lse, hipStream_t stream) {
    constexpr int smem = 2 * (F16 ? 2 : 3) * (BKV * D + C2 * BKV) * (int)sizeof(u16);
    static unsigned attr_mask = 0;
    auto kern = flash_attn_x6_kernel<D, C2, BKV, NW, F16>;
    if (const int rc = gssd_max_dynamic_lds(&attr_mask, kern, smem)) return rc;
    const int qtiles = (N + 16 * NW - 1) / (16 * NW);
    hipLaunchKernelGGL(kern, dim3(B * qtiles), dim3(64 * NW), smem, stream, tpp, gp, out, N, Np32, qtiles, (long long)B * N * 2 * D,
                       (long long)B * C2 * Np32, lse);
    GSSD_CHECK_LAUNCH();
    return GSSD_OK;
}

inline long long round32(long long n) { return (n + 31) / 32 * 32; }

}

extern "C" int gssd_self_attn_core_x6_supported(int D, int C2) { return D == 64 && C2 == 256; }

extern "C" long long gssd_self_attn_core_x6_ws_bytes(int B, int N, int D, int C2) {
    if (B <= 0 || N <= 0 || !gssd_self_attn_core_x6_supported(D, C2)) return -1;
    return 2ll * NP * ((long long)B * N * 2 * D + (long long)B * C2 * round32(N));
}

extern "C" int gssd_self_attn_core_x6_f32(const float* tp, const float* gT, float* out, int B, int N, int Np, int D, int C2, void* ws,
                                          float* lse, gssd_stream_t stream) {
    GSSD_CHECK_ARG(tp && gT && out && ws && B > 0 && N > 0 && Np >= N && Np % 4 == 0);
    GSSD_CHECK_ARG(((uintptr_t)tp % 16) == 0 && ((uintptr_t)gT % 16) == 0 && ((uintptr_t)out % 16) == 0 && ((uintptr_t)ws % 16) == 0);
    GSSD_CHECK_ARG((long long)B * ((N + 63) / 64) < (1ll << 31));
    if (!gssd_self_attn_core_x6_supported(D, C2)) {
        gssd_set_error("self-attention core (three-plane): unsupported (theta/phi channels %d, g channels %d); built: (64,256)", D, C2);
        return GSSD_EINVAL;
    }
    hipStream_t s = as_stream(stream);
    const int Np32 = (int)round32(N);
    u16* tpp = reinterpret_cast<u16*>(ws);
    const long long tp_plane = (long long)B * N * 2 * D, g_plane = (long long)B * C2 * Np32;
    u16* gp = tpp + NP * tp_plane;
    static const bool f16 = [] { const char* e = getenv("GSSD_FLASH_X6_F16"); return e && e[0] == '1'; }();
    {
        const long long n = (long long)B * N * (2 * D / 8);
        if (f16) hipLaunchKernelGGL(split_planes_kernel<true>, dim3((unsigned)((n + 255) / 256)), dim3(256), 0, s, tp, tpp, (long long)B * N, 2 * D, 2 * D, 2 * D, tp_plane, 0);
        else hipLaunchKernelGGL(split_planes_kernel<false>, dim3((unsigned)((n + 255) / 256)), dim3(256), 0, s, tp, tpp, (long long)B * N, 2 * D, 2 * D, 2 * D, tp_plane, 0);
        GSSD_CHECK_LAUNCH();
    }
    {
        const long long n = (long long)B * C2 * (Np32 / 8);
        if (f16) hipLaunchKernelGGL(split_planes_kernel<true>, dim3((unsigned)((n + 255) / 256)), dim3(256), 0, s, gT, gp, (long long)B * C2, N, Np, Np32, g_plane, 1);
        else hipLaunchKernelGGL(split_planes_kernel<false>, dim3((unsigned)((n + 255) / 256)), dim3(256), 0, s, gT, gp, (long long)B * C2, N, Np, Np32, g_plane, 1);
        GSSD_CHECK_LAUNCH();
    }
    if (f16) return N > 1024 ? launch_x6<64, 256, 32, 12, true>(tpp, gp, out, B, N, Np32, lse, s) : launch_x6<64, 256, 32, 4, true>(tpp, gp, out, B, N, Np32, lse, s);
    return N > 1024 ? launch_x6<64, 256, 32, 12, false>(tpp, gp, out, B, N, Np32, lse, s) : launch_x6<64, 256, 32, 4, false>(tpp, gp, out, B, N, Np32, lse, s);
}
```

### grouped-ssd-pytorch_amd/gssd/csrc/plan_run.hip

```cpp
#include <hip/hip_runtime.h>
#include <cstdint>
#include <cstring>
#include <mutex>
#include <tuple>
#include <type_traits>
#include <utility>
#include "common.h"

namespace {

template <class T>
inline T plan_arg(uint64_t w) {
    if constexpr (std::is_pointer_v<T>) {
        return reinterpret_cast<T>(static_cast<uintptr_t>(w));
    } else if constexpr (std::is_same_v<T, float>) {
        const uint32_t b = static_cast<uint32_t>(w);
        float f;
        memcpy(&f, &b, 4);
        return f;
    } else if constexpr (std::is_same_v<T, double>) {
        double d;
        memcpy(&d, &w, 8);
        return d;
    } else {
        static_assert(std::is_integral_v<T>, "plan argument types: pointers, integers, float, double");
        return static_cast<T>(static_cast<int64_t>(w));
    }
}

template <class... P, size_t... I>
inline int plan_call(int (*f)(P...), const uint64_t* a, gssd_stream_t s, std::index_sequence<I...>) {
    using T = std::tuple<P...>;
    static_assert(sizeof...(P) - 1 <= GSSD_PLAN_MAX_ARGS, "GSSD_PLAN_MAX_ARGS");
    static_assert(std::is_same_v<std::tuple_element_t<sizeof...(P) - 1, T>, gssd_stream_t>, "the last parameter is the stream");
    return f(plan_arg<std::tuple_element_t<I, T>>(a[I])..., s);
}

template <class... P>
constexpr int plan_nargs(int (*)(P...)) { return (int)sizeof...(P) - 1; }

struct PlanFn {
    const char* name;
    int nargs;
    int (*thunk)(const uint64_t*, gssd_stream_t);
};

template <auto F>
int plan_thunk(const uint64_t* a, gssd_stream_t s) {
    return plan_call(F, a, s, std::make_index_sequence<plan_nargs(F)>{});
}

#define GSSD_PLAN_FN(f) PlanFn{#f, plan_nargs(&f), &plan_thunk<&f>}
const PlanFn g_plan_fns[] = {
    GSSD_PLAN_FN(gssd_event_record_node),
    GSSD_PLAN_FN(gssd_pack_input_nhwc),
    GSSD_PLAN_FN(gssd_unpack_nhwc_to_nchw),
    GSSD_PLAN_FN(gssd_pack_conv_weight),
    GSSD_PLAN_FN(gssd_pack_conv_weights_batched),
    GSSD_PLAN_FN(gssd_conv2d_nhwc_f32),
    GSSD_PLAN_FN(gssd_conv_x6_pack_weight),
    GSSD_PLAN_FN(gssd_conv_patch_x6_pack_weight),
    GSSD_PLAN_FN(gssd_conv2d_nhwc_bf16),
    GSSD_PLAN_FN(gssd_pack_conv_weight_bf16),
    GSSD_PLAN_FN(gssd_cast_f32_bf16),
    GSSD_PLAN_FN(gssd_cast_bf16_f32),
    GSSD_PLAN_FN(gssd_pack_input_nhwc_bf16),
    GSSD_PLAN_FN(gssd_bn_relu_pool_bf16),
    GSSD_PLAN_FN(gssd_bn_finalize_bf16),
    GSSD_PLAN_FN(gssd_l2norm_bf16),
    GSSD_PLAN_FN(gssd_winograd_weight_f32),
    GSSD_PLAN_FN(gssd_conv2d_wgrad_f32),
    GSSD_PLAN_FN(gssd_conv2d_wgrad_bf16),
    GSSD_PLAN_FN(gssd_unpack_conv_weight_grad),
    GSSD_PLAN_FN(gssd_pack_conv_weight_dgrad),
    GSSD_PLAN_FN(gssd_bn_relu_pool_f32),
    GSSD_PLAN_FN(gssd_bn_finalize_f32),
    GSSD_PLAN_FN(gssd_bn_bwd_reduce_f32),
    GSSD_PLAN_FN(gssd_bn_bwd_finalize_f32),
    GSSD_PLAN_FN(gssd_bn_bwd_apply_f32),
    GSSD_PLAN_FN(gssd_bn_bwd_reduce_mixed),
    GSSD_PLAN_FN(gssd_bn_bwd_apply_mixed),
    GSSD_PLAN_FN(gssd_bn_bwd_apply_masked_f32),
    GSSD_PLAN_FN(gssd_colsum_f32),
    GSSD_PLAN_FN(gssd_cast_f64_f32),
    GSSD_PLAN_FN(gssd_l2norm_bwd_f32),
    GSSD_PLAN_FN(gssd_heads_gather_f32),
    GSSD_PLAN_FN(gssd_upsample_insert_f32),
    GSSD_PLAN_FN(gssd_l2norm_f32),
    GSSD_PLAN_FN(gssd_self_attn_core_f32),
    GSSD_PLAN_FN(gssd_self_attn_core_kv_f32),
    GSSD_PLAN_FN(gssd_sa_pool_kv_f32),
    GSSD_PLAN_FN(gssd_sa_unpool_f32),
    GSSD_PLAN_FN(gssd_self_attn_core_bf16v),
    GSSD_PLAN_FN(gssd_self_attn_core_x6_f32),
    GSSD_PLAN_FN(gssd_self_attn_flash_bwd_bf16),
    GSSD_PLAN_FN(gssd_softmax_rows_f32),
    GSSD_PLAN_FN(gssd_slice_and_cat_f32),
    GSSD_PLAN_FN(gssd_spectral_norm_f32),
    GSSD_PLAN_FN(gssd_dcn_im2col_f32),
    GSSD_PLAN_FN(gssd_dcn_im2col_bf16),
    GSSD_PLAN_FN(gssd_dcn_geo_im2col_f32),
    GSSD_PLAN_FN(gssd_dcn_geo_col2im_f32),
    GSSD_PLAN_FN(gssd_dcn_pack_weight_f32),
    GSSD_PLAN_FN(gssd_dcn_forward_f32),
    GSSD_PLAN_FN(gssd_dcn_streamk_reset),
    GSSD_PLAN_FN(gssd_dcn_pack_weight_x6),
    GSSD_PLAN_FN(gssd_dcn_forward_x6),
    GSSD_PLAN_FN(gssd_dcn_forward_x6_ex),
    GSSD_PLAN_FN(gssd_dcn_pack_weight_bf16),
    GSSD_PLAN_FN(gssd_dcn_forward_bf16),
    GSSD_PLAN_FN(gssd_dcn_col2im_f32),
    GSSD_PLAN_FN(gssd_resize_u8_horizontal),
    GSSD_PLAN_FN(gssd_resize_u8_vertical),
    GSSD_PLAN_FN(gssd_input_finish_f32),
    GSSD_PLAN_FN(gssd_augment_minmax),
    GSSD_PLAN_FN(gssd_augment_horizontal),
    GSSD_PLAN_FN(gssd_augment_vertical),
    GSSD_PLAN_FN(gssd_pixellink_targets),
    GSSD_PLAN_FN(gssd_bgemm_f32),
    GSSD_PLAN_FN(gssd_bgemm_ex_f32),
    GSSD_PLAN_FN(gssd_rowdot_f32),
    GSSD_PLAN_FN(gssd_softmax_bwd_rows_f32),
    GSSD_PLAN_FN(gssd_sn_weight_grad_f32),
    GSSD_PLAN_FN(gssd_scaled_transpose_f32),
    GSSD_PLAN_FN(gssd_cast_split_f32_bf16),
    GSSD_PLAN_FN(gssd_cast_rows_f32_bf16),
    GSSD_PLAN_FN(gssd_transpose_cast_f32_bf16),
    GSSD_PLAN_FN(gssd_dot_f32),
    GSSD_PLAN_FN(gssd_axpby_f32),
    GSSD_PLAN_FN(gssd_scale_cast_f64_f32),
    GSSD_PLAN_FN(gssd_sa_sigma_grad_f32),
    GSSD_PLAN_FN(gssd_match_batch),
    GSSD_PLAN_FN(gssd_reduce_max_f32),
    GSSD_PLAN_FN(gssd_hnm_loss),
    GSSD_PLAN_FN(gssd_loss_finalize),
    GSSD_PLAN_FN(gssd_loss_finalize_global),
    GSSD_PLAN_FN(gssd_loss_backward),
    GSSD_PLAN_FN(gssd_detect),
    GSSD_PLAN_FN(gssd_softmax_lastdim_f32),
    GSSD_PLAN_FN(gssd_eval_match),
    GSSD_PLAN_FN(gssd_eval_ap),
    GSSD_PLAN_FN(gssd_heads_reduce_f32),
    GSSD_PLAN_FN(gssd_interp_add_f32),
    GSSD_PLAN_FN(gssd_pixellink_final_f32),
    GSSD_PLAN_FN(gssd_pixellink_loss_f32),
    GSSD_PLAN_FN(gssd_interp_add_bwd_f32),
    GSSD_PLAN_FN(gssd_pixellink_final_bwd_f32),
    GSSD_PLAN_FN(gssd_pixellink_loss_bwd_f32),
    GSSD_PLAN_FN(gssd_pixellink_decode_f32),
    GSSD_PLAN_FN(gssd_pixellink_final5_f32),
    GSSD_PLAN_FN(gssd_pixellink_final5_bwd_f32),
    GSSD_PLAN_FN(gssd_self_attn_flash_bwd_f32),
};
#undef GSSD_PLAN_FN
constexpr int N_PLAN_FNS = (int)(sizeof(g_plan_fns) / sizeof(g_plan_fns[0]));

constexpr int N_EVENTS = 64;
struct EventRing {
    hipEvent_t ev[N_EVENTS];
    int next = 0;
    bool ready = false;
    std::mutex mu;
};
EventRing g_rings[32];

int record_and_wait(hipStream_t src, hipStream_t dst) {
    int cur = 0, dev = -1;
    (void)hipGetDevice(&cur);
    hipDevice_t sdev;
    if (src && hipStreamGetDevice(src, &sdev) == hipSuccess) dev = (int)sdev;
    if (dev < 0) dev = cur;
    if (dev < 0 || dev >= 32) return 1;
    EventRing& r = g_rings[dev];
    std::lock_guard<std::mutex> lock(r.mu);
    if (!r.ready) {
        if (dev != cur && hipSetDevice(dev) != hipSuccess) return 1;
        bool ok = true;
        for (int i = 0; i < N_EVENTS && ok; ++i) ok = hipEventCreateWithFlags(&r.ev[i], hipEventDisableTiming) == hipSuccess;
        if (dev != cur) (void)hipSetDevice(cur);
        if (!ok) return 1;
        r.ready = true;
    }
    hipEvent_t e = r.ev[r.next];
    r.next = (r.next + 1) % N_EVENTS;
    return (hipEventRecord(e, src) != hipSuccess || hipStreamWaitEvent(dst, e, 0) != hipSuccess) ? 1 : 0;
}

}

extern "C" int gssd_plan_fn_count(void) { return N_PLAN_FNS; }

extern "C" const char* gssd_plan_fn_name(int index) { return index >= 0 && index < N_PLAN_FNS ? g_plan_fns[index].name : nullptr; }

extern "C" int gssd_plan_fn_index(const char* name) {
    if (!name) return -1;
    for (int i = 0; i < N_PLAN_FNS; ++i)
        if (!strcmp(g_plan_fns[i].name, name)) return i;
    return -1;
}

extern "C" int gssd_plan_fn_nargs(int index) { return index >= 0 && index < N_PLAN_FNS ? g_plan_fns[index].nargs : -1; }

extern "C" int gssd_plan_op_size(void) { return (int)sizeof(gssd_plan_op); }

extern "C" int gssd_plan_run(const gssd_plan_op* ops, int n_ops, const gssd_stream_t* streams, int n_streams, int* failed_at) {
    GSSD_CHECK_ARG(ops && n_ops >= 0 && streams && n_streams > 0);
    if (failed_at) *failed_at = -1;
    for (int i = 0; i < n_ops; ++i) {
        const gssd_plan_op& op = ops[i];
        int rc = GSSD_OK;
        if (op.stream < 0 || op.stream >= n_streams) {
            gssd_set_error("gssd_plan_run: stream index out of range");
            rc = GSSD_EINVAL;
        } else if (op.kind == GSSD_PLAN_LAUNCH) {
            if (op.fn < 0 || op.fn >= N_PLAN_FNS) {
                gssd_set_error("gssd_plan_run: function index out of range");
                rc = GSSD_EINVAL;
            } else if (op.nargs != g_plan_fns[op.fn].nargs) {
                gssd_set_error("gssd_plan_run: argument count does not match the function's parameters");
                rc = GSSD_EINVAL;
            } else {
                rc = g_plan_fns[op.fn].thunk(op.args, streams[op.stream]);
            }
        } else if (op.kind == GSSD_PLAN_WAIT) {
            if (op.fn < 0 || op.fn >= n_streams) {
                gssd_set_error("gssd_plan_run: awaited stream index out of range");
                rc = GSSD_EINVAL;
            } else if (op.fn != op.stream) {
                if (record_and_wait(as_stream(streams[op.fn]), as_stream(streams[op.stream]))) {
                    gssd_set_error("gssd_plan_run: event record / stream wait failed");
                    rc = GSSD_ELAUNCH;
                }
            }
        } else {
            gssd_set_error("gssd_plan_run: unknown op kind");
            rc = GSSD_EINVAL;
        }
        if (rc != GSSD_OK) {
            if (failed_at) *failed_at = i;
            return rc;
        }
    }
    return GSSD_OK;
}
```

### grouped-ssd-pytorch_amd/gssd/plan_common.py

```python
import ctypes as C
import os
import torch
from . import _lib, ops
from ._lib import lib

VGG_CFG = [64, 64, 'M', 128, 128, 'M', 256, 256, 256, 'C', 512, 512, 512, 'M', 512, 512, 512]
EXTRAS_CFG = [256, 'S', 512, 128, 'S', 256, 128, 256, 128, 256]
MBOX = [4, 6, 6, 6, 4, 4]
SRC_HW = [38, 19, 10, 5, 3, 1]
HEAD_OFF = [sum(h * h * a for h, a in zip(SRC_HW[:i], MBOX[:i])) for i in range(6)]
FUSE_NAMES = ['11', '21', '31', '41', '51', '61']


USE_HEADS_WINO = os.environ.get('GSSD_HEADS_WINO', '1') != '0'
USE_PATCH_X6 = os.environ.get('GSSD_PATCH_X6', '1') != '0'
USE_CONV_X6 = os.environ.get('GSSD_CONV_X6', '1') != '0'
USE_WINOGRAD = os.environ.get('GSSD_NO_WINOGRAD', '0') != '1'
DCN_X6 = os.environ.get('GSSD_DCN_X6', '1') != '0'
USE_GRAPH = os.environ.get('GSSD_NO_GRAPH', '0') != '1'
USE_FLASH_X6 = os.environ.get('GSSD_FLASH_X6', '1') != '0'
USE_BRANCH_STREAMS = os.environ.get('GSSD_NO_BRANCH_STREAMS', '0') != '1'
FUSE_PACK = os.environ.get('GSSD_FUSE_PACK', '1') != '0'
FUSE_CAT = os.environ.get('GSSD_FUSE_CAT', '1') != '0'
SN_STREAM = 9
ALL_STREAMS = -1

class Tag(tuple):
    layer = None


class _Step:
    __slots__ = ('fn', 'args', 'keep', 'tag', 'sid', 'wait')

    def __init__(self, fn, args, keep=None, tag=None, sid=0, wait=None):
        self.fn, self.args, self.keep, self.tag, self.sid, self.wait = fn, args, keep, tag, sid, wait


def conv_tag(d, real_cin_g=None, bf16=False):
    cout_g = d.Cout // d.groups
    inst = '128x128' if cout_g > 64 else '128x64' if cout_g > 32 else '128x32' if cout_g > 16 else '128x16'
    if cout_g > 64:
        mt = -(-(d.Ho * d.Wo * (1 if d.m_per_image else d.B)) // 128)
        z = d.B if d.m_per_image else d.split_k
        b128 = mt * d.groups * (-(-cout_g // 128)) * z
        b64 = mt * d.groups * (-(-cout_g // 64)) * z
        e128 = b128 / (-(-b128 // 512) * 512)
        e64 = 0.94 * b64 / (-(-b64 // 768) * 768)
        if e64 > e128 or d.K <= 256:
            inst = '128x64'
    Ms, Mtot = d.Ho * d.Wo * (1 if d.m_per_image else d.B), d.Ho * d.Wo * d.B
    if (cout_g > 32 and d.split_k == 1 and Mtot <= 4096 and os.environ.get('GSSD_NO_SMALL_TILES') is None
            and not (d.out_mode == _lib.OUT_SPLIT_T and d.split_n % 64 != 0)):
        inst = '32x64' if (Mtot <= 512 or (d.m_per_image and Ms <= 128)) else '64x64'
    if (bf16 and os.environ.get('GSSD_BF16_BIG_TILES', '0') == '1' and not d.m_per_image and d.split_k == 1 and d.B * d.Ho * d.Wo >= 8192
            and cout_g % 128 == 0 and d.K % 64 == 0 and d.K >= 256
            and (d.out_mode == _lib.OUT_NHWC or (d.out_mode == _lib.OUT_SPLIT_T and d.split_n % 128 == 0))):
        inst = '256x128'
    name = ('conv_bf16<' if bf16 else 'conv_igemm<') + inst + '>'
    if not bf16 and d.wgt_patch and lib.gssd_conv_patch_x6_takes(C.byref(d)) == 1:
        M6 = d.B * d.Ho * d.Wo
        return ('conv_patch_x6<128>', 2.0 * M6 * d.Cout * 9 * d.cin_g, 4.0 * (d.B * d.H * d.W * d.cin_g + M6 * d.Cout + d.Cout * 9 * d.cin_g))
    if not bf16 and d.wgt_x6 and lib.gssd_conv_x6_takes(C.byref(d)) == 1:
        M6 = d.B * d.Ho * d.Wo
        flops = 2.0 * M6 * d.Cout * d.KH * d.KW * d.cin_g
        return (f'conv_x6<{ops.x6_tile(cout_g, d.groups, M6)}>', flops, 4.0 * (d.B * d.H * d.W * d.cin_g * d.groups + M6 * d.Cout + d.Cout * d.KH * d.KW * d.cin_g))
    if bf16:
        if (d.groups == 4 and d.KH == 3 and d.stride == 1 and d.pad == 1 and d.dil == 1 and d.H * d.W >= 75 * 75
                and (d.cin_g, cout_g) in ((8, 16), (16, 16), (16, 32), (32, 32)) and not d.m_per_image and d.split_k == 1
                and d.flags in (0, _lib.CONV_POOL2)):
            name = f'conv_thin_bf16<{d.cin_g},{cout_g}>' + ('/pool2' if d.flags & _lib.CONV_POOL2 else '')
    elif (d.groups == 4 and d.KH == 3 and d.stride == 1 and d.pad == 1 and d.dil == 1 and d.H * d.W >= 75 * 75
            and (d.cin_g, cout_g) in ((4, 16), (16, 16), (16, 32)) and not d.m_per_image and d.split_k == 1):
        name = f'conv_thin<{d.cin_g},{cout_g}>'
        if d.wgt_wino and (d.cin_g, cout_g) == (16, 32) and os.environ.get('GSSD_CONV21_WINO', '1') != '0':
            name = 'conv_wino<32>'
        if d.wgt_wino and (d.cin_g, cout_g) == (16, 16) and not d.resid:
            name = 'conv_thin_wino<16,16>'
    elif (d.wgt_wino and ops.winograd_eligible(d.KH, d.stride, d.pad, d.dil, d.cin_g, cout_g, d.groups) and not d.m_per_image
          and d.split_k <= 1 and not d.relu):
        name = f'conv_wino<{64 if (cout_g % 64 == 0 or (cout_g % 32 != 0 and cout_g > 32)) else 32}>'
    igemm_name = ('conv_bf16<' if bf16 else 'conv_igemm<') + inst + '>'
    if name.startswith('conv_wino<') and lib.gssd_conv_wino_x6_takes(C.byref(d)) == 1:
        name = f'conv_wino_x6<{64 if cout_g > 32 else 32}>'
    elif name.startswith('conv_wino<') and d.out_mode == _lib.OUT_HEADS:
        name = igemm_name
    if not bf16 and lib.gssd_conv_thin_x6_takes(C.byref(d)) == 1:
        name = f'conv_thin_x6<{d.cin_g},{cout_g}>'
    if name.startswith(('conv_wino<', 'conv_wino_x6<', 'conv_thin_x6<')):
        name += ('' if d.in_scale else '/plain') + ('/pool2' if d.flags & _lib.CONV_POOL2 else '')
    if bf16 and name.startswith('conv_bf16'):
        bm = lib.gssd_conv_flat_bf16_takes(C.byref(d))
        if bm:
            name = f'conv_flat_bf16<{d.cin_g},{min(cout_g, 128) if cout_g % 128 == 0 else 64},{bm}>'
    if not bf16 and name.startswith('conv_igemm') and lib.gssd_gemm_slot_takes(C.byref(d)) == 1:
        name = 'gemm_slot<128x128>'
    M = d.B * d.Ho * d.Wo
    cin_g = real_cin_g if real_cin_g is not None else d.cin_g
    flops = 2.0 * M * d.Cout * d.KH * d.KW * cin_g
    esz = 2.0 if bf16 else 4.0
    out_elems = M * d.Cout // 4 if (d.flags & _lib.CONV_POOL2) else M * d.Cout
    byts = esz * (d.B * d.H * d.W * cin_g * d.groups + out_elems + d.Cout * d.KH * d.KW * cin_g)
    return (name, flops, byts)
```

### grouped-ssd-pytorch_amd/gssd/plan_graph.py

```python
import ctypes as C
import os
import torch
from . import _lib, ops, plan_common
from ._lib import lib
from .plan_common import ALL_STREAMS, FUSE_NAMES, SN_STREAM, VGG_CFG


class PlanGraphMixin:
    def _place_branch0(self):
        if (os.environ.get('GSSD_BRANCH0_LATE', '1') == '0' or getattr(self, '_mark_conv7', None) is None
                or not self.eng.net.use_self_attention):
            return
        idx = [i for i, st in enumerate(self.steps) if st.sid == 1]
        if not idx or idx[-1] - idx[0] + 1 != len(idx) or idx[-1] >= self._mark_conv7:
            return
        a, b, c = idx[0], idx[-1] + 1, self._mark_conv7
        block = self.steps[a:b]
        self.steps[a:c] = self.steps[b:c] + block

    def _place_sn_step(self):
        sn = next((i for i, st in enumerate(self.steps) if st.sid == SN_STREAM), None)
        if sn is None or sn > self._pack_step:
            return
        st = self.steps.pop(sn)
        self._pack_step -= 1
        self.steps.insert(self._pack_step + 2, st)

    def _fuse_input_pack(self):
        i = self._pack_step
        if (not plan_common.FUSE_PACK or not getattr(self, 'nograd', False) or self.bf16 or i + 1 >= len(self.steps)
                or self.steps[i].fn is not lib.gssd_pack_input_nhwc):
            return
        st, x16_ptr = self.steps[i + 1], self.steps[i].args[1]
        d = st.keep
        if (st.fn is not lib.gssd_conv2d_nhwc_f32 or not isinstance(d, _lib.ConvDesc) or d.in_ != x16_ptr or st.wait is not None
                or lib.gssd_conv_thin_nchw3_takes(C.byref(d)) != 1):
            return
        d.flags |= _lib.CONV_IN_NCHW3
        del self.steps[i]
        self._reduce_steps = tuple(k - 1 for k in self._reduce_steps)
        self._pack_step, self._in_desc = None, d

    def _set_input(self, ptr):
        d = self.__dict__.get('_in_desc')
        if d is not None:
            d.in_ = ptr
        else:
            self.steps[self._pack_step].args[0] = ptr

    def _build_bn_graph(self, x16):
        net = self.eng.net
        g = net.groups_vgg
        cur, H, Cc = x16, 300, self.cpad * g
        vi = 0
        cfg = list(VGG_CFG)
        i = 0
        x43 = None
        xf = None
        while i < len(cfg):
            v = cfg[i]
            assert v not in ('M', 'C')
            conv, bn = net.vgg[vi], net.vgg[vi + 1]
            pool = None
            nxt = cfg[i + 1] if i + 1 < len(cfg) else None
            is_conv4_3 = (vi == 30)
            last = (i == len(cfg) - 1)
            if nxt in ('M', 'C') and not is_conv4_3:
                pool = (2, 2, 0, nxt == 'C')
            if last:
                pool = (3, 1, 1, False)
            defer = (pool is None and not is_conv4_3)
            cur, H, Cc, xf = self._conv_bn(f'vgg.{vi}', conv, bn, cur, H, Cc, g, relu=True, pool=pool, in_xf=xf,
                                           defer_bn=defer)
            vi += 3
            if nxt in ('M', 'C'):
                vi += 1
                i += 1
            i += 1
            if is_conv4_3:
                x43 = cur
                cur, H, Cc, src0 = self._after_conv4_3(cur, H, Cc)
        vi += 1
        xf = None
        for li in range(2):
            conv, bn = net.vgg[vi], net.vgg[vi + 1]
            cur, H, Cc, xf = self._conv_bn(f'vgg.{vi}', conv, bn, cur, H, Cc, g, relu=True, in_xf=xf, defer_bn=(li == 0))
            vi += 3
        sources = [src0]
        self._mark_conv7 = len(self.steps)
        sab_i, sa_i = 1, 1
        if net.use_self_attention_base:
            cur, _ = self._self_attn('self_attn_base_list', sab_i, cur, H, Cc, need_out2=False, want_map=self.want_maps)
            sab_i += 1
        sources.append(self._branch(cur, H, Cc, sa_i, '21'))
        sa_i += 1
        ge = net.groups_extra
        n_ex = len(net.extras)
        fi = 2
        xf = None
        for k in range(0, n_ex, 2):
            conv, bn = net.extras[k], net.extras[k + 1]
            cur, H, Cc, xf = self._conv_bn(f'extras.{k}', conv, bn, cur, H, Cc, ge, relu=True, in_xf=xf,
                                           defer_bn=((k + 1) % 4 != 3))
            if (k + 1) % 4 == 3:
                if net.use_self_attention_base:
                    cur, _ = self._self_attn('self_attn_base_list', sab_i, cur, H, Cc, need_out2=False, want_map=self.want_maps)
                    sab_i += 1
                sources.append(self._branch(cur, H, Cc, sa_i, FUSE_NAMES[fi]))
                sa_i += 1
                fi += 1
        self.sources = sources

    def _build_plain_graph(self, x16):
        net = self.eng.net
        g, ge = net.groups_vgg, net.groups_extra
        cur, H, Cc = x16, 300, self.cpad * g
        mods = list(net.vgg)
        i = 0
        src0 = None
        while i < len(mods):
            m = mods[i]
            if isinstance(m, torch.nn.Conv2d):
                cur, H, Cc = self._conv_act(f'vgg.{i}', m, cur, H, Cc, g)
                i += 2
                if i - 2 == 21:
                    cur, H, Cc, src0 = self._after_conv4_3(cur, H, Cc)
                    i += 1
            else:
                cur, H = self._pool_only(cur, H, Cc, m.kernel_size, m.stride, m.padding, m.ceil_mode)
                i += 1
        sources = [src0]
        sab_i, sa_i = 1, 1
        if net.use_self_attention_base:
            cur, _ = self._self_attn('self_attn_base_list', sab_i, cur, H, Cc, need_out2=False, want_map=self.want_maps)
            sab_i += 1
        sources.append(self._branch(cur, H, Cc, sa_i, '21'))
        sa_i += 1
        fi = 2
        for k, m in enumerate(net.extras):
            cur, H, Cc = self._conv_act(f'extras.{k}', m, cur, H, Cc, ge)
            if k % 2 == 1:
                if net.use_self_attention_base:
                    cur, _ = self._self_attn('self_attn_base_list', sab_i, cur, H, Cc, need_out2=False, want_map=self.want_maps)
                    sab_i += 1
                sources.append(self._branch(cur, H, Cc, sa_i, FUSE_NAMES[fi]))
                sa_i += 1
                fi += 1
        self.sources = sources

    def _finish_heads(self):
        B, dev = self.B, self.dev
        smax = max(d.split_k for d in self.head_descs)
        splits = torch.ones(self.P, dtype=torch.int8)
        off = 0
        for d in self.head_descs:
            A = d.split_n // 4
            n = d.Ho * d.Wo * A
            splits[off:off + n] = d.split_k
            off += n
        assert off == self.P
        self._head_splits = splits.to(dev)
        self._ws_loc = torch.empty(smax, B, self.P, 4, device=dev, dtype=torch.float32)
        self._ws_conf = torch.empty(smax, B, self.P, self.nc, device=dev, dtype=torch.float32)
        for d in self.head_descs:
            d.out, d.out_b = self._ws_loc.data_ptr(), self._ws_conf.data_ptr()
            d.flags |= _lib.CONV_HEADS_SLICES
        prev, self._sid = getattr(self, '_sid', 0), 0
        self._pending_wait = ALL_STREAMS
        self._reduce_steps = (len(self.steps), len(self.steps) + 1)
        self._add(lib.gssd_heads_reduce_f32, [self._ws_loc.data_ptr(), self._head_splits.data_ptr(), 0, B, self.P, 4])
        self._add(lib.gssd_heads_reduce_f32, [self._ws_conf.data_ptr(), self._head_splits.data_ptr(), 0, B, self.P, self.nc])
        self._sid = prev

    def _set_outputs(self, loc, conf):
        self.steps[self._reduce_steps[0]].args[2] = loc.data_ptr()
        self.steps[self._reduce_steps[1]].args[2] = conf.data_ptr()

    def _after_conv4_3(self, x, H, Cc):
        net, B = self.eng.net, self.B
        attn_g, cat_g = None, 0
        if net.use_self_attention_base:
            cat_g = (net.groups_vgg if (plan_common.FUSE_CAT and getattr(self, 'nograd', False) and not self.bf16 and net.use_dcn
                                        and net.dcn_cat_sab) else 0)
            x, attn_g = self._self_attn('self_attn_base_list', 0, x, H, Cc, need_out2=bool(net.dcn_cat_sab), want_map=self.want_maps,
                                        cat_groups=cat_g)
        if net.use_dcn:
            xin, Cin = x, Cc
            if net.dcn_cat_sab and cat_g and attn_g is None:
                xin, Cin = x, 2 * Cc
            elif net.dcn_cat_sab:
                xc = self._abuf(B, H, H, 2 * Cc)
                esz = 2 if self.bf16 else 1
                self._add(lib.gssd_slice_and_cat_f32, (x.data_ptr(), attn_g.data_ptr(), xc.data_ptr(), B * H * H, Cc // esz, Cc // esz,
                                                       net.groups_vgg))
                self.rec.append(('slice_cat', dict(a=x, b=attn_g, out=xc, H=H, Ca=Cc, Cb=Cc, groups=net.groups_vgg,
                                                   detach_b=bool(net.detach_sab))))
                xin, Cin = xc, 2 * Cc
            for li in range(net.num_dcn_layers):
                xin, Cin = self._dcn(li, xin, H, Cin)
            x, Cc = xin, Cin
        self.x_after_block = x
        s = self._abuf(B, H, H, Cc)
        self._sid = 1
        self._add(lib.gssd_l2norm_bf16 if self.bf16 else lib.gssd_l2norm_f32,
                  (x.data_ptr(), net.L2Norm.weight.data_ptr(), s.data_ptr(), B * H * H, Cc, float(net.L2Norm.eps)))
        self.rec.append(('l2norm', dict(x_in=x, out=s, H=H, C=Cc, mod=net.L2Norm)))
        self._sid = 0
        src0 = self._branch(s, H, Cc, 0, '11')
        self._layer = 'vgg.33'
        pooled, Hp = self._pool_only(x, H, Cc, 2, 2, 0)
        self._layer = None
        return pooled, Hp, Cc, src0

    def _branch(self, s, H, Cc, sa_i, fuse):
        net = self.eng.net
        prev, self._sid = getattr(self, '_sid', 0), sa_i + 1
        if net.use_self_attention:
            s, _ = self._self_attn('self_attn_list', sa_i, s, H, Cc, need_out2=False, want_map=self.want_maps)
        if net.use_fuseconv and net.batch_norm:
            conv, bn = getattr(net, f'fuse_{fuse}'), getattr(net, f'bn_fuse_{fuse}')
            s, H, Cc, _ = self._conv_bn(f'fuse_{fuse}', conv, bn, s, H, Cc, 1, relu=True)
        elif net.use_fuseconv:
            s, H, Cc = self._conv_act(f'fuse_{fuse}', getattr(net, f'fuse_{fuse}'), s, H, Cc, 1)
        self._head(sa_i, s, H, Cc)
        self._sid = prev
        return (s, H, Cc)
```

### grouped-ssd-pytorch_amd/gssd/plan_ops.py

```python
import ctypes as C
import os
import torch
from . import _lib, ops
from ._lib import lib
from .plan_common import DCN_X6, HEAD_OFF, MBOX, SN_STREAM, USE_CONV_X6, USE_FLASH_X6, USE_HEADS_WINO, USE_PATCH_X6, USE_WINOGRAD


class PlanOpsMixin:
    @property
    def f16_ok(self):
        net = getattr(getattr(self, 'eng', None), 'net', None)
        bn = bool(getattr(net, 'batch_norm', False))
        return _lib.CONV_F16_OK if (bn and not getattr(self, 'bf16', False) and getattr(self, 'training', False)) else 0

    def _conv_act(self, name, conv, x, H, Cin, groups):
        B = self.B
        k, s, p, dl = conv.kernel_size[0], conv.stride[0], conv.padding[0], conv.dilation[0]
        Cout = conv.out_channels
        wp = self._packed_conv(name, conv)
        Ho = (H + 2 * p - dl * (k - 1) - 1) // s + 1
        out = self._buf(B, Ho, Ho, Cout)
        d, _, _ = ops.make_conv_desc(x, wp, out, B=B, H=H, W=H, in_stride=Cin, cin_g=Cin // groups, Cout=Cout, groups=groups, k=k,
                                     stride=s, pad=p, dil=dl, bias=conv.bias.detach(), relu=True)
        self._add(lib.gssd_conv2d_nhwc_f32, (C.byref(d),), keep=d)
        self.rec.append(('convrelu', dict(name=name, conv=conv, x_in=x, out=out, H=H, Cin=Cin, Ho=Ho, Cout=Cout, desc=d, k=k,
                                          stride=s, pad=p, dil=dl, groups=groups)))
        return out, Ho, Cout

    def _head(self, i, s, Hs, Cs):
        eng, net, B, dev, f32 = self.eng, self.eng.net, self.B, self.dev, torch.float32
        off = HEAD_OFF[i]
        A = MBOX[i]
        nloc, nconf = A * 4, A * self.nc
        lw, cw = net.loc[i], net.conf[i]
        cin_pad, K = ops.packed_k(Cs, 3, 3)

        def build_w(out, lw=lw, cw=cw, nloc=nloc, nconf=nconf, K=K):
            if out is None:
                out = torch.empty(nloc + nconf, K, device=dev, dtype=self.adt)
            pk = ops.pack_weight_bf16 if self.bf16 else ops.pack_weight
            pk(lw.weight, out, 0)
            pk(cw.weight, out, nloc)
            return out

        def build_b(out, lw=lw, cw=cw, nloc=nloc):
            if out is None:
                out = torch.empty(nloc + cw.bias.numel(), device=dev, dtype=f32)
            ops.copy_into(out[:nloc], lw.bias)
            ops.copy_into(out[nloc:], cw.bias)
            return out
        wp = eng._pack(f'heads.{i}.w', build_w)
        bp = eng._pack(f'heads.{i}.b', build_b)
        split = (ops.auto_split_k(B * Hs * Hs, nloc + nconf, 1, K, target_blocks=256, max_split=8)
                 if self.bf16 else ops.auto_split_k(B * Hs * Hs, nloc + nconf, 1, K))
        U = None
        if (self.f16_ok and USE_WINOGRAD and USE_HEADS_WINO and nloc % 4 == 0 and nconf % 4 == 0 and B * ((Hs + 1) // 2) ** 2 >= 8192
                and ops.winograd_eligible(3, 1, 1, 1, Cs, nloc + nconf, 1)):
            def build_u(out, key=f'heads.{i}.w', cin=Cs):
                return ops.winograd_weight(eng._packed[key], 1, cin, out)
            U = eng._pack(f'heads.{i}.U', build_u)
            split = 1
        d, _, _ = ops.make_conv_desc(s, wp, None, B=B, H=Hs, W=Hs, in_stride=Cs, cin_g=Cs, Cout=nloc + nconf, k=3,
                                     pad=1, bias=bp, out_mode=_lib.OUT_HEADS, out_b=None, split_n=nloc,
                                     out_batch_stride=self.P * 4, outb_batch_stride=self.P * self.nc,
                                     out_off=off * 4, outb_off=off * self.nc, split_k=split, wgt_wino=U,
                                     flags=_lib.CONV_OUT_F32 | (self.f16_ok if U is not None else 0))
        self.head_descs.append(d)
        self._add(self.conv_fn, (C.byref(d),), keep=d)
        self.rec.append(('head', dict(i=i, src=s, H=Hs, C=Cs, A=A, off=off, loc=lw, conf=cw, K=K)))

    def _setup_spectral_norm(self, lists):
        self.sn_items = []
        self.sa_state = {}
        for lst_name, lst in lists:
            for i, sa in enumerate(lst):
                Cc = sa.in_channels
                a_tpg = self._buf(Cc // 4 + Cc // 2)
                a_o = self._buf(Cc)
                self.sn_items += [
                    (sa.snconv1x1_theta.weight_orig, sa.snconv1x1_theta.weight_u, sa.snconv1x1_theta.weight_v, a_tpg[:Cc // 8]),
                    (sa.snconv1x1_phi.weight_orig, sa.snconv1x1_phi.weight_u, sa.snconv1x1_phi.weight_v, a_tpg[Cc // 8:Cc // 4]),
                    (sa.snconv1x1_g.weight_orig, sa.snconv1x1_g.weight_u, sa.snconv1x1_g.weight_v, a_tpg[Cc // 4:]),
                    (sa.snconv1x1_attn.weight_orig, sa.snconv1x1_attn.weight_u, sa.snconv1x1_attn.weight_v, a_o),
                ]
                self.sa_state[(lst_name, i)] = (a_tpg, a_o)
        if self.sn_items:
            self.sn_dev = ops.sn_items_tensor([(w.detach(), u, v, s) for (w, u, v, s) in self.sn_items], self.dev)
            prev, self._sid = getattr(self, '_sid', 0), SN_STREAM
            self._add(lib.gssd_spectral_norm_f32, (self.sn_dev.data_ptr(), len(self.sn_items), int(self.training), 1e-12))
            self._sid = prev
            self._sn_unjoined = True

    def _packed_conv(self, name, conv):
        eng = self.eng

        def build(out, conv=conv):
            if self.bf16:
                return ops.pack_weight_bf16(conv.weight, out)
            return ops.pack_weight(conv.weight, out)
        return eng._pack(name + '.w', build)

    def _conv_bn(self, name, conv, bn, x, H, Cin, groups, relu=True, pool=None, in_xf=None, defer_bn=False):
        B = self.B
        self._layer = name
        k, s, p, dl = conv.kernel_size[0], conv.stride[0], conv.padding[0], conv.dilation[0]
        Cout = conv.out_channels
        cin_g = Cin // groups
        if defer_bn and Cout // groups > 512:
            defer_bn = False
        wp = self._packed_conv(name, conv)
        U = None
        if not self.bf16 and USE_WINOGRAD and ops.winograd_eligible(k, s, p, dl, cin_g, Cout // groups, groups):
            def build_u(out, key=name + '.w', groups=groups, cin_g=cin_g):
                return ops.winograd_weight(self.eng._packed[key], groups, cin_g, out)
            U = self.eng._pack(name + '.U', build_u)
        Ho = (H + 2 * p - dl * (k - 1) - 1) // s + 1
        X6 = None
        if not self.bf16 and USE_CONV_X6 and ops.x6_wanted(k, cin_g, Cout // groups, groups, B * Ho * Ho, winograd=U is not None, forward=bool(self.f16_ok)):
            def build_x6(out, key=name + '.w', groups=groups, cin_g=cin_g, taps=k * k, bn=ops.x6_tile(Cout // groups, groups, B * Ho * Ho)):
                return ops.x6_weight(self.eng._packed[key], groups, cin_g, taps, bn, out)
            X6 = self.eng._pack(name + f'.x6@{ops.x6_tile(Cout // groups, groups, B * Ho * Ho)}', build_x6)
        st = self.eng_stat(bn)
        srep = getattr(self, 'stat_rep', {}).get(id(bn), 0) if self.training else 0
        cout_g = Cout // groups
        pooled = (getattr(self, 'nograd', False) and relu and pool is not None and pool[:3] == (2, 2, 0) and (pool[3] or Ho % 2 == 0) and k == 3 and s == 1
                  and p == 1 and dl == 1 and groups == 4 and
                  ((U is not None) if not self.bf16 else ((cin_g, cout_g) in ((16, 16), (32, 32)) and Ho % 2 == 0 and Ho * Ho >= 75 * 75)))
        if pooled:
            Hp = ops.pool_out_size(Ho, 2, 2, 0, pool[3])
            raw, pd = self._abuf_tail(Cout, B, Hp, Hp, Cout)
            d, _, _ = ops.make_conv_desc(x, wp, raw, B=B, H=H, W=H, in_stride=Cin, cin_g=cin_g, Cout=Cout, groups=groups, k=k,
                                         stride=s, pad=p, dil=dl, bias=conv.bias.detach(), wgt_wino=U,
                                         stats=st if self.training else None,
                                         in_scale=in_xf[0] if in_xf else None, in_shift=in_xf[1] if in_xf else None,
                                         in_pad=in_xf[2] if in_xf else None, flags=_lib.CONV_POOL2 | self.f16_ok, pool_sign=bn.weight.detach(), stats_rep=srep)
            self._add(self.conv_fn, (C.byref(d),), keep=d)
            sc, sh = self._buf(Cout), self._buf(Cout)
            self._add(lib.gssd_bn_finalize_bf16 if self.bf16 else lib.gssd_bn_finalize_f32,
                      (st.data_ptr(), float(B * Ho * Ho), bn.weight.data_ptr(), bn.bias.data_ptr(),
                       bn.running_mean.data_ptr(), bn.running_var.data_ptr(), float(bn.momentum), float(bn.eps),
                       int(self.training), Cout, sc.data_ptr(), sh.data_ptr(), pd.data_ptr(), srep))
            self.rec.append(('convbn', dict(name=name, conv=conv, bn=bn, x_in=x, in_xf=in_xf, H=H, Cin=Cin, groups=groups, raw=raw, Ho=Ho,
                                            Cout=Cout, desc=d, stats=st, stats_rep=srep, pool=pool, relu=relu, k=k, stride=s, pad=p, dil=dl, out=raw,
                                            Hp=Hp, xf=(sc, sh, pd), pooled=True)))
            self._layer = None
            return raw, Hp, Cout, (sc, sh, pd)
        raw, pd_tail = self._abuf_tail(Cout, B, Ho, Ho, Cout) if defer_bn else (self._abuf(B, Ho, Ho, Cout), None)
        d, _, _ = ops.make_conv_desc(x, wp, raw, B=B, H=H, W=H, in_stride=Cin, cin_g=cin_g, Cout=Cout, groups=groups, k=k,
                                     stride=s, pad=p, dil=dl, bias=conv.bias.detach(), wgt_wino=U, wgt_x6=X6,
                                     stats=st if self.training else None,
                                     in_scale=in_xf[0] if in_xf else None, in_shift=in_xf[1] if in_xf else None,
                                     in_pad=in_xf[2] if in_xf else None, stats_rep=srep,
                                     flags=self.f16_ok)
        self._add(self.conv_fn, (C.byref(d),), keep=d)
        rec = dict(name=name, conv=conv, bn=bn, x_in=x, in_xf=in_xf, H=H, Cin=Cin, groups=groups, raw=raw, Ho=Ho, Cout=Cout,
                   desc=d, stats=st, stats_rep=srep, pool=pool, relu=relu, k=k, stride=s, pad=p, dil=dl)
        self.rec.append(('convbn', rec))
        if defer_bn:
            assert pool is None and relu
            sc, sh, pd = self._buf(Cout), self._buf(Cout), pd_tail
            self._add(lib.gssd_bn_finalize_bf16 if self.bf16 else lib.gssd_bn_finalize_f32,
                      (st.data_ptr(), float(B * Ho * Ho), bn.weight.data_ptr(), bn.bias.data_ptr(),
                       bn.running_mean.data_ptr(), bn.running_var.data_ptr(), float(bn.momentum), float(bn.eps),
                       int(self.training), Cout, sc.data_ptr(), sh.data_ptr(), pd.data_ptr(), srep))
            rec.update(out=raw, Hp=Ho, xf=(sc, sh, pd))
            self._layer = None
            return raw, Ho, Cout, (sc, sh, pd)
        if pool:
            pk, ps, pp, ceil = pool
            Hp = ops.pool_out_size(Ho, pk, ps, pp, ceil)
        else:
            pk, ps, pp, Hp = 0, 1, 0, Ho
        act = self._abuf(B, Hp, Hp, Cout)
        self._add(lib.gssd_bn_relu_pool_bf16 if self.bf16 else lib.gssd_bn_relu_pool_f32,
                  (raw.data_ptr(), act.data_ptr(), B, Ho, Ho, Cout, Hp, Hp, pk, ps, pp, st.data_ptr(), float(B * Ho * Ho),
                   bn.weight.data_ptr(), bn.bias.data_ptr(), bn.running_mean.data_ptr(), bn.running_var.data_ptr(),
                   float(bn.momentum), float(bn.eps), int(self.training), int(relu), srep),
                  tag=('bn_relu_pool_bf16' if self.bf16 else 'bn_relu_pool', 0.0,
                       (2.0 if self.bf16 else 4.0) * B * Cout * (Ho * Ho + Hp * Hp)))
        rec.update(out=act, Hp=Hp, xf=None)
        self._layer = None
        return act, Hp, Cout, None

    def eng_stat(self, bn):
        return self.stat_of[id(bn)]

    def _pool_only(self, x, H, Cc, k, s, p, ceil=False):
        B = self.B
        Hp = ops.pool_out_size(H, k, s, p, ceil)
        out = self._abuf(B, Hp, Hp, Cc)
        self._add(lib.gssd_bn_relu_pool_bf16 if self.bf16 else lib.gssd_bn_relu_pool_f32,
                  (x.data_ptr(), out.data_ptr(), B, H, H, Cc, Hp, Hp, k, s, p, 0, 1.0, 0, 0, 0, 0, 0.1, 1e-5, 0, 0, 0),
                  tag=('bn_relu_pool_bf16' if self.bf16 else 'bn_relu_pool', 0.0, (2.0 if self.bf16 else 4.0) * B * Cc * (H * H + Hp * Hp)))
        self.rec.append(('pool', dict(x_in=x, out=out, H=H, C=Cc, k=k, s=s, p=p, Hp=Hp)))
        return out, Hp

    def _self_attn(self, lst_name, idx, x, H, Cc, need_out2, want_map=False, cat_groups=0):
        eng, B = self.eng, self.B
        sa = getattr(eng.net, lst_name)[idx]
        a_tpg, a_o = self.sa_state[(lst_name, idx)]
        if self.__dict__.pop('_sn_unjoined', False):
            self._pending_wait = SN_STREAM
        N = H * H
        Np = ops.round_up(N, 4)
        C8, C2, C4 = Cc // 8, Cc // 2, Cc // 4
        dev, f32 = self.dev, torch.float32
        name = f'{lst_name}.{idx}'

        def build_w(out):
            if out is None:
                out = torch.empty(C4 + C2, Cc, device=dev, dtype=self.adt)
            ops.copy_into(out[:C8], sa.snconv1x1_theta.weight_orig)
            ops.copy_into(out[C8:C4], sa.snconv1x1_phi.weight_orig)
            ops.copy_into(out[C4:], sa.snconv1x1_g.weight_orig)
            return out

        def build_wo(out):
            if out is None:
                out = torch.empty(Cc, C2, device=dev, dtype=self.adt)
            ops.copy_into(out, sa.snconv1x1_attn.weight_orig)
            return out

        def build_b(out):
            if out is None:
                out = torch.empty(C4 + C2, device=dev, dtype=f32)
            ops.copy_into(out[:C8], sa.snconv1x1_theta.bias)
            ops.copy_into(out[C8:C4], sa.snconv1x1_phi.bias)
            ops.copy_into(out[C4:], sa.snconv1x1_g.bias)
            return out
        w_tpg = eng._pack(name + '.tpg.w', build_w)
        b_tpg = eng._pack(name + '.tpg.b', build_b)
        w_o = eng._pack(name + '.o.w', build_wo) if self.bf16 else sa.snconv1x1_attn.weight_orig.detach().view(Cc, C2)
        tp = self._buf(B, N, C4)
        if self.bf16:
            Np = ops.round_up(N, 32)
            gT = self._abuf(B, C2, Np)
        else:
            gT = self._buf(B, C2, Np)
        ag = self._abuf(B, N, C2)
        out = self._abuf(B, H, H, Cc)
        out2 = self._abuf(B, H, H, Cc) if need_out2 else None
        mk = ops.make_conv_desc
        flat = not self.bf16 and N % 4 == 0 and Np == N
        x6_tpg = None
        if (not self.bf16 and USE_CONV_X6 and ops.x6_wanted(1, Cc, C4 + C2, 1, B * N) and C4 % ops.x6_tile(C4 + C2, 1, B * N) == 0):
            def build_x6p(out, key=name + '.tpg.w', bn=ops.x6_tile(C4 + C2, 1, B * N)):
                return ops.x6_weight(eng._packed[key], 1, Cc, 1, bn, out)
            x6_tpg = eng._pack(name + f'.tpg.x6@{ops.x6_tile(C4 + C2, 1, B * N)}', build_x6p)
            gT.zero_()
        d1, _, _ = mk(x, w_tpg, tp, B=B, H=H, W=H, in_stride=Cc, cin_g=Cc, Cout=C4 + C2, bias=b_tpg, alpha=a_tpg, wgt_x6=x6_tpg,
                      out_mode=_lib.OUT_SPLIT_T, out_b=gT, split_n=C4, out_stride=C4, out_b_stride=Np, m_per_image=not flat,
                      in_batch_stride=N * Cc, out_batch_stride=N * C4, outb_batch_stride=C2 * Np,
                      flags=_lib.CONV_OUT_F32 | (_lib.CONV_OUTB_BF16_PERM32 if self.bf16 else self.f16_ok))
        x6_o = None
        if not self.bf16 and USE_CONV_X6 and ops.x6_wanted(1, C2, Cc, 1, B * N):
            def build_x6o(out, bn=ops.x6_tile(Cc, 1, B * N)):
                return ops.x6_weight(sa.snconv1x1_attn.weight_orig.detach().view(Cc, C2), 1, C2, 1, bn, out)
            x6_o = eng._pack(name + f'.o.x6@{ops.x6_tile(Cc, 1, B * N)}', build_x6o)
        d5, _, _ = mk(ag, w_o, out, B=B, H=H, W=H, in_stride=C2, cin_g=C2, Cout=Cc, bias=sa.snconv1x1_attn.bias.detach(),
                      alpha=a_o, gate=sa.sigma.detach(), resid=x, out2=out2, wgt_x6=x6_o, flags=self.f16_ok)
        xc = None
        if cat_groups and need_out2 and x6_o is not None and Cc % cat_groups == 0:
            ga = Cc // cat_groups
            xc = self._abuf(B, H, H, 2 * Cc)
            dc, _, _ = mk(ag, w_o, xc, B=B, H=H, W=H, in_stride=C2, cin_g=C2, Cout=Cc, bias=sa.snconv1x1_attn.bias.detach(),
                          alpha=a_o, gate=sa.sigma.detach(), resid=x, out2=xc.view(-1)[ga:], wgt_x6=x6_o, out_stride=2 * Cc, split_n=ga,
                          flags=self.f16_ok | _lib.CONV_OUT_GROUPCAT)
            if lib.gssd_conv_x6_takes(C.byref(dc)) == 1:
                d5 = dc
                self.bufs[:] = [t for t in self.bufs if t is not out and t is not out2]
                v = xc.view(B, H, H, cat_groups, 2, ga)
                out, out2 = v[:, :, :, :, 0], v[:, :, :, :, 1]
            else:
                self.bufs[:] = [t for t in self.bufs if t is not xc]
                xc = None
        fn = self.conv_fn
        if C4 % 64 == 0:
            self._add(fn, (C.byref(d1),), keep=(d1, w_tpg, b_tpg))
        else:
            if self.bf16:
                raise _lib.GssdError('bf16 mode: Self_Attn needs >= 64 theta|phi channels (in_channels >= 256)')
            d1a, _, _ = mk(x, w_tpg, tp, B=B, H=H, W=H, in_stride=Cc, cin_g=Cc, Cout=C4, bias=b_tpg, alpha=a_tpg)
            d1b, _, _ = mk(x, w_tpg[C4:], gT, B=B, H=H, W=H, in_stride=Cc, cin_g=Cc, Cout=C2, bias=b_tpg[C4:], alpha=a_tpg[C4:],
                           out_mode=_lib.OUT_TRANSPOSED, out_stride=Np, m_per_image=True, in_batch_stride=N * Cc,
                           out_batch_stride=C2 * Np)
            self._add(fn, (C.byref(d1a),), keep=(d1a, w_tpg, b_tpg))
            self._add(fn, (C.byref(d1b),), keep=d1b)
        lse = self._buf(B, N) if self.training else None
        P = max(H // int(sa.max_pool_factor), 1)
        pooled = P != H
        Nk, Nkp, kp, gTp = N, Np, None, None
        if pooled:
            if self.bf16:
                raise _lib.GssdError('bf16 storage mode is built for max_pool_factor = 1 (BASELINE.json configs[4])')
            Nk, Nkp = P * P, ops.round_up(P * P, 4)
            kp, gTp = self._buf(B, Nk, C8), self._buf(B, C2, Nkp)
            self._add(lib.gssd_sa_pool_kv_f32, (tp.data_ptr(), gT.data_ptr(), kp.data_ptr(), gTp.data_ptr(), B, H, P, C8, C2, Np, Nkp))
            self._add(lib.gssd_self_attn_core_kv_f32, (tp.data_ptr(), kp.data_ptr(), gTp.data_ptr(), ag.data_ptr(), B, N, Nk, Nkp, C8, C2,
                                                       C8, 0, lse.data_ptr() if lse is not None else 0),
                      tag=(f'flash_attn<{C8},{C2}>', 2.0 * B * N * Nk * (C8 + C2), 4.0 * B * (N * C8 + Nk * C8 + C2 * Nkp + N * C2)))
        elif self.bf16:
            self._add(lib.gssd_self_attn_core_bf16v, (tp.data_ptr(), gT.data_ptr(), ag.data_ptr(), B, N, Np, C8, C2,
                                                      lse.data_ptr() if lse is not None else 0),
                      tag=(f'flash_attn_bf16v<{C8},{C2}>', 2.0 * B * N * N * (C8 + C2), B * (4.0 * N * C4 + 2.0 * C2 * Np + 2.0 * N * C2)))
        elif USE_FLASH_X6 and N >= 1024 and C8 == 64 and lib.gssd_self_attn_core_x6_supported(C8, C2):
            ws = self._buf(int(lib.gssd_self_attn_core_x6_ws_bytes(B, N, C8, C2)) // 4)
            self._add(lib.gssd_self_attn_core_x6_f32, (tp.data_ptr(), gT.data_ptr(), ag.data_ptr(), B, N, Np, C8, C2, ws.data_ptr(),
                                                       lse.data_ptr() if lse is not None else 0),
                      tag=(f'flash_attn_x6<{C8},{C2}>', 2.0 * B * N * N * (C8 + C2), 4.0 * B * (N * C4 + C2 * Np + N * C2)))
        else:
            self._add(lib.gssd_self_attn_core_kv_f32, (tp.data_ptr(), tp[0, 0, C8:].data_ptr(), gT.data_ptr(), ag.data_ptr(), B, N, N, Np,
                                                       C8, C2, C4, 0, lse.data_ptr() if lse is not None else 0),
                      tag=(f'flash_attn<{C8},{C2}>', 2.0 * B * N * N * (C8 + C2), 4.0 * B * (N * C4 + C2 * Np + N * C2)))
        S = None
        if want_map:
            S = self._buf(B, N, Nkp)
            keys, krow = (kp, C8) if pooled else (tp[0, 0, C8:], C4)
            d3, _, _ = mk(tp, keys, S, B=B, H=H, W=H, in_stride=C4, cin_g=C8, Cout=Nk, out_stride=Nkp, m_per_image=True,
                          in_batch_stride=N * C4, wgt_batch_stride=Nk * krow, out_batch_stride=N * Nkp, wgt_row_stride=krow)
            self._add(lib.gssd_conv2d_nhwc_f32, (C.byref(d3),), keep=d3)
            self._add(lib.gssd_softmax_rows_f32, (S.data_ptr(), B * N, Nk, Nkp))
        self._add(fn, (C.byref(d5),), keep=d5)
        self.attn_maps = getattr(self, 'attn_maps', {})
        self.attn_maps[(lst_name, idx)] = (S, Nk, Nkp)
        self.rec.append(('sa', dict(mod=sa, name=name, x_in=x, out=out, out2=out2, H=H, C=Cc, tp=tp, gT=gT, ag=ag, N=N, Np=Np,
                                    inv_sigma=(a_tpg, a_o), P=P, Nk=Nk, Nkp=Nkp, kp=kp, gTp=gTp, lse=lse)))
        if xc is not None:
            return xc, None
        return out, out2

    def _dcn(self, li, x, H, Cin):
        eng, B = self.eng, self.B
        m = eng.net.dcn_list[li]
        if not m.is_engine_geometry():
            raise _lib.GssdError(f'dcn_list.{li}: the engine runs 3x3 / stride 1 / pad 1 / dilation 1 DCN layers only (kernel '
                                 f'{m.kernel_size}, stride {m.stride}, padding {m.padding}, dilation {m.dilation})')
        dg, Cout = m.deformable_groups, m.out_channels
        w_om = self._packed_conv(f'dcn_list.{li}.om', m.conv_offset_mask)

        def build_w(out, m=m, Cin=Cin, dg=dg):
            elems = lib.gssd_dcn_packed_weight_elems_bf16 if self.bf16 else lib.gssd_dcn_packed_weight_elems_x6 if DCN_X6 else lib.gssd_dcn_packed_weight_elems
            pack = lib.gssd_dcn_pack_weight_bf16 if self.bf16 else lib.gssd_dcn_pack_weight_x6 if DCN_X6 else lib.gssd_dcn_pack_weight_f32
            if out is None:
                n = int(elems(m.out_channels, Cin))
                if n <= 0:
                    raise _lib.GssdError(f'deformable conv: unsupported shape Cin {Cin}, Cout {m.out_channels}')
                out = torch.empty(n, device=self.dev, dtype=torch.bfloat16 if (DCN_X6 and not self.bf16) else self.adt)
            _lib.check(pack(m.weight.detach().contiguous().data_ptr(), out.data_ptr(), m.out_channels, Cin, dg,
                            torch.cuda.current_stream().cuda_stream))
            return out
        w_main = eng._pack(f'dcn_list.{li}.wt' + ('.x6' if (DCN_X6 and not self.bf16) else ''), build_w)
        OMC = ops.round_up(27 * dg, 8 if self.bf16 else 4)
        om = self._buf(B, H, H, OMC)
        if OMC != 27 * dg:
            om.zero_()
        out = self._abuf(B, H, H, Cout)
        u_om = None
        if not self.bf16 and USE_WINOGRAD and ops.winograd_eligible(3, 1, 1, 1, Cin, 27 * dg, 1):
            def build_u(out, key=f'dcn_list.{li}.om.w', cin=Cin):
                return ops.winograd_weight(eng._packed[key], 1, cin, out)
            u_om = eng._pack(f'dcn_list.{li}.om.U', build_u)
        p_om = None
        if self.f16_ok and USE_PATCH_X6 and lib.gssd_conv_patch_x6_weight_elems(27 * dg, Cin) > 0:
            def build_p(out, key=f'dcn_list.{li}.om.w', cin=Cin):
                return ops.patch_x6_weight(eng._packed[key], cin, out)
            p_om = eng._pack(f'dcn_list.{li}.om.px6', build_p)
        d1, _, _ = ops.make_conv_desc(x, w_om, om, B=B, H=H, W=H, in_stride=Cin, cin_g=Cin, Cout=27 * dg, k=3, pad=1, out_stride=OMC,
                                      bias=m.conv_offset_mask.bias.detach(), wgt_wino=u_om, wgt_patch=p_om,
                                      flags=_lib.CONV_OUT_F32 | self.f16_ok)
        self._add(self.conv_fn, (C.byref(d1),), keep=d1)
        M = B * H * H
        esz = 2.0 if self.bf16 else 4.0
        self._add(lib.gssd_dcn_forward_bf16 if self.bf16 else lib.gssd_dcn_forward_x6_ex if DCN_X6 else lib.gssd_dcn_forward_f32,
                  (x.data_ptr(), om.data_ptr(), w_main.data_ptr(), m.bias.data_ptr(), out.data_ptr(), B, H, H, Cin, dg, OMC, Cout) +
                  ((self.f16_ok,) if DCN_X6 and not self.bf16 else ()),
                  keep=w_main, tag=('dcn_bf16<128x256>' if self.bf16 else 'dcn_x6<128x256>' if DCN_X6 else 'dcn_fused<128x256>', 2.0 * M * Cout * 9 * Cin,
                                    esz * (M * (Cin + Cout) + Cout * 9 * Cin) + 4.0 * M * 27 * dg))
        if not self.bf16 and not DCN_X6:
            self.__dict__.setdefault('_sk_outs', []).append(out.data_ptr())
        self.offsets = getattr(self, 'offsets', [])
        self.offsets.append((om, H, dg))
        self.rec.append(('dcn', dict(mod=m, x_in=x, out=out, H=H, Cin=Cin, Cout=Cout, om=om, d_om=d1, dg=dg, li=li, omc=OMC)))
        return out, Cout
```

### include/gssd_hip.h

```cpp
#ifndef GSSD_HIP_H
#define GSSD_HIP_H

#include <stdint.h>

#ifdef __cplusplus
extern "C" {
#endif

#define GSSD_OK 0
#define GSSD_EINVAL (-1)
#define GSSD_ELAUNCH (-2)

typedef void* gssd_stream_t;

int gssd_abi_version(void);
int gssd_conv_desc_size(void);
const char* gssd_last_error(void);
const char* gssd_build_arch(void);

typedef void* gssd_event_t;
int gssd_event_create(gssd_event_t* ev);
int gssd_event_destroy(gssd_event_t ev);
int gssd_event_record_node(gssd_event_t ev, gssd_stream_t stream);
int gssd_event_elapsed_ms(gssd_event_t start, gssd_event_t stop, float* ms);


int gssd_pack_input_nhwc(const float* x_nchw, float* y_nhwc, int B, int C, int H, int W, int groups,
                         int cpg_out, gssd_stream_t stream);

int gssd_unpack_nhwc_to_nchw(const float* x_nhwc, float* y_nchw, int B, int C, int H, int W, int x_stride,
                             gssd_stream_t stream);

int gssd_pack_conv_weight(const float* w_oihw, float* w_packed, int Cout, int cin_g, int KH, int KW,
                          int cin_g_pad, int Kpad, gssd_stream_t stream);

typedef struct gssd_pack_item {
    const float* w;
    float* wp;
    int32_t Cout, cin_g, taps, cin_g_pad, Kpad, reserved;
} gssd_pack_item;
int gssd_pack_conv_weights_batched(const gssd_pack_item* items_dev, int n_items, gssd_stream_t stream);

#define GSSD_OUT_NHWC 0
#define GSSD_OUT_TRANSPOSED 1
#define GSSD_OUT_HEADS 2
#define GSSD_OUT_SPLIT_T 3

typedef struct gssd_conv_desc {
    const float* in;
    const float* wgt;
    const float* bias;
    float* out;
    float* out_b;
    const float* alpha;
    const float* gate;
    const float* resid;
    float* out2;
    const float* in_scale;
    const float* in_shift;
    const float* in_pad;
    double* stats;
    const float* wgt_wino;
    const float* pool_sign;
    const void* wgt_x6;
    const void* wgt_patch;
    int B, H, W;
    int in_stride;
    int in_ch_off;
    int Ho, Wo;
    int Cout, groups;
    int cin_g;
    int KH, KW, stride, pad, dil;
    int K;
    int wgt_row_stride;
    int out_stride;
    int out_ch_off;
    int out_mode;
    int relu;
    int m_per_image;
    int split_n;
    int split_k;
    int out_b_stride;
    int flags;
    int stats_rep;
    int64_t in_batch_stride, wgt_batch_stride, out_batch_stride, outb_batch_stride;
    int64_t out_off, outb_off;
} gssd_conv_desc;

int gssd_conv2d_nhwc_f32(const gssd_conv_desc* d, gssd_stream_t stream);

int gssd_conv_x6_tile(int cout_g, int groups, long long M);
long long gssd_conv_x6_weight_elems(int Cout, int groups, int cin_g, int taps, int BN);
int gssd_conv_x6_pack_weight(const float* w_packed, void* w_x6, int Cout, int groups, int cin_g, int taps, int row_stride, int BN,
                             gssd_stream_t stream);
int gssd_conv_x6_takes(const gssd_conv_desc* d);

#define GSSD_CONV_OUT_F32 1
#define GSSD_CONV_OUTB_BF16_PERM32 2
#define GSSD_CONV_HEADS_SLICES 4
#define GSSD_CONV_POOL2 8
#define GSSD_CONV_RESID_F32 16
#define GSSD_CONV_F16_OK 32
#define GSSD_CONV_IN_NCHW3 64
#define GSSD_CONV_OUT_GROUPCAT 128
int gssd_conv2d_nhwc_bf16(const gssd_conv_desc* d, gssd_stream_t stream);
int gssd_pack_conv_weight_bf16(const float* w_oihw, void* w_packed, int Cout, int cin_g, int KH, int KW, int cin_g_pad, int Kpad,
                               gssd_stream_t stream);
int gssd_cast_f32_bf16(const float* x, void* y, int64_t n, gssd_stream_t stream);
int gssd_cast_bf16_f32(const void* x, float* y, int64_t n, gssd_stream_t stream);
int gssd_pack_input_nhwc_bf16(const float* x_nchw, void* y_nhwc, int B, int C, int H, int W, int groups, gssd_stream_t stream);
int gssd_bn_relu_pool_bf16(const void* raw, void* out, int B, int H, int W, int C, int Ho, int Wo, int pool_k, int pool_s, int pool_p,
                           const double* stats, double count, const float* gamma, const float* beta, float* running_mean,
                           float* running_var, float momentum, float eps, int training, int relu, int stats_rep,
                           gssd_stream_t stream);
int gssd_bn_finalize_bf16(const double* stats, double count, const float* gamma, const float* beta, float* running_mean,
                          float* running_var, float momentum, float eps, int training, int C, float* scale, float* shift,
                          void* pad_bf16, int stats_rep, gssd_stream_t stream);
int gssd_l2norm_bf16(const void* x, const float* weight, void* out, int64_t pixels, int C, float eps, gssd_stream_t stream);

long long gssd_winograd_weight_elems(int Cout, int groups, int cin_g);
int gssd_winograd_weight_f32(const float* w_packed, float* U, int Cout, int groups, int cin_g, int row_stride,
                             gssd_stream_t stream);

int gssd_conv2d_wgrad_f32(const gssd_conv_desc* d, const float* dy, float* dw_packed, gssd_stream_t stream);
int gssd_conv2d_wgrad_bf16(const gssd_conv_desc* d, const void* dy, float* dw_packed, gssd_stream_t stream);
int gssd_conv2d_wgrad_bf16_supported(const gssd_conv_desc* d);
int gssd_unpack_conv_weight_grad(const float* w_packed, float* w_oihw, int Cout, int cin_g, int KH, int KW,
                                 int cin_g_pad, int Kpad, int accumulate, gssd_stream_t stream);
int gssd_pack_conv_weight_dgrad(const float* w_oihw, float* w_packed, int Cout, int groups, int cin_g, int KH, int KW,
                                gssd_stream_t stream);

int gssd_bn_relu_pool_f32(const float* raw, float* out, int B, int H, int W, int C, int Ho, int Wo, int pool_k,
                          int pool_s, int pool_p, const double* stats, double count, const float* gamma,
                          const float* beta, float* running_mean, float* running_var, float momentum, float eps,
                          int training, int relu, int stats_rep, gssd_stream_t stream);

int gssd_bn_finalize_f32(const double* stats, double count, const float* gamma, const float* beta,
                         float* running_mean, float* running_var, float momentum, float eps, int training, int C,
                         float* scale, float* shift, float* pad, int stats_rep, gssd_stream_t stream);

int gssd_bn_bwd_reduce_f32(const float* dout, const float* raw, const float* scale, const float* shift, float* dz,
                           double* sums, int B, int H, int W, int C, int Ho, int Wo, int pool_k, int pool_s, int pool_p,
                           int relu, gssd_stream_t stream);
int gssd_bn_bwd_finalize_f32(const double* fwd_stats, double count, const double* bwd_sums, const float* gamma, float eps,
                             int C, float* coef_a, float* coef_b, float* coef_c, float* dgamma, float* dbeta,
                             int stats_rep, gssd_stream_t stream);
int gssd_bn_bwd_apply_f32(float* dz, const float* raw, const float* coef_a, const float* coef_b, const float* coef_c,
                          int64_t pixels, int C, double* colsum, gssd_stream_t stream);
int gssd_bn_bwd_reduce_mixed(const void* dout, int dout_bf16, const void* raw_bf16, const float* scale, const float* shift, float* dz,
                             void* dz_bf16, double* sums, int B, int H, int W, int C, int Ho, int Wo, int pool_k, int pool_s, int pool_p,
                             int relu, gssd_stream_t stream);
int gssd_bn_bwd_apply_mixed(const void* dout, int dout_bf16, float* dz, void* dz_bf16, const void* raw_bf16, const float* scale,
                            const float* shift, int relu, const float* coef_a, const float* coef_b, const float* coef_c, int64_t pixels,
                            int C, double* colsum, int store_f32, gssd_stream_t stream);
int gssd_bn_bwd_apply_masked_f32(const float* dout, const float* raw, const float* scale, const float* shift, int relu,
                                 const float* coef_a, const float* coef_b, const float* coef_c, float* draw, int64_t pixels, int C,
                                 double* colsum, gssd_stream_t stream);
int gssd_colsum_f32(const float* x, int64_t rows, int C, int row_stride, double* out, gssd_stream_t stream);
int gssd_cast_f64_f32(const double* x, float* y, int n, int accumulate, gssd_stream_t stream);
int gssd_l2norm_bwd_f32(const float* x, const float* weight, const float* dy, float* dx, const float* dx_add,
                        double* dweight, int64_t pixels, int C, float eps, gssd_stream_t stream);
int gssd_heads_gather_f32(const float* dloc, const float* dconf, float* out, int B, int HW, int A, int nc, int P,
                          int prior_off, gssd_stream_t stream);
int gssd_upsample_insert_f32(const float* dy, float* u, int B, int Ho, int Wo, int H, int W, int C, int s,
                             gssd_stream_t stream);

int gssd_l2norm_f32(const float* x, const float* weight, float* out, int64_t pixels, int C, float eps,
                    gssd_stream_t stream);

int gssd_self_attn_core_f32(const float* tp, const float* gT, void* out, int B, int N, int Np, int D, int C2, int out_bf16,
                            gssd_stream_t stream);

int gssd_self_attn_core_kv_f32(const float* tp, const float* kp, const float* gT, void* out, int B, int N, int Nk, int Nkp, int D,
                               int C2, int kstride, int out_bf16, float* lse, gssd_stream_t stream);

int gssd_sa_pool_kv_f32(const float* tp, const float* gT, float* kp, float* gTp, int B, int H, int P, int C8, int C2, int Np, int Nkp,
                        gssd_stream_t stream);

int gssd_sa_unpool_f32(const float* dkg, float* dst, int B, int H, int P, int CW, int ld, gssd_stream_t stream);

int gssd_gemm_slot_takes(const gssd_conv_desc* d);

int gssd_conv_flat_bf16_takes(const gssd_conv_desc* d);
int gssd_conv_flat_bf16_tile(int pixels_per_workgroup);

int gssd_self_attn_core_bf16v(const float* tp, const void* gT_bf16, void* out_bf16, int B, int N, int Np32, int D, int C2,
                              float* lse, gssd_stream_t stream);

int gssd_self_attn_flash_bwd_bf16(const float* tp, const void* tp_bf16, const void* tp_bf16_lo, const void* g_bf16, const void* dag_bf16,
                                  const float* lse, const float* dvec, float* dtpg, int B, int N, int D, int C2, gssd_stream_t stream);
int gssd_self_attn_flash_bwd_supported(int D, int C2);

int gssd_softmax_rows_f32(float* x, int64_t rows, int n, int row_stride, gssd_stream_t stream);

int gssd_slice_and_cat_f32(const float* a, const float* b, float* out, int64_t pixels, int Ca, int Cb,
                           int groups, gssd_stream_t stream);

typedef struct gssd_sn_item {
    const float* w;
    float* u;
    float* v;
    float* inv_sigma;
    int rows, cols;
} gssd_sn_item;
int gssd_spectral_norm_f32(const gssd_sn_item* items_dev, int n, int do_power_iteration, float eps,
                           gssd_stream_t stream);

int gssd_dcn_im2col_f32(const float* x, const float* om, float* cols, int B, int H, int W, int C, int dg,
                        int om_stride, gssd_stream_t stream);
int gssd_dcn_im2col_bf16(const void* x_bf16, const float* om, void* cols_bf16, int B, int H, int W, int C, int dg, int om_stride,
                         gssd_stream_t stream);

long long gssd_dcn_packed_weight_elems(int Cout, int C);
int gssd_dcn_pack_weight_f32(const float* w_oihw, float* w_packed, int Cout, int C, int dg, gssd_stream_t stream);
int gssd_dcn_forward_f32(const float* x, const float* om, const float* w_packed, const float* bias, float* out, int B, int H,
                         int W, int C, int dg, int om_stride, int Cout, gssd_stream_t stream);
int gssd_dcn_streamk(int mode);
#define GSSD_DCN_SK_UNSUPPORTED 1
#define GSSD_DCN_SK_MAPPING 2
#define GSSD_DCN_SK_TIMEOUT 4
int gssd_dcn_streamk_status(unsigned* xcc_map);
int gssd_dcn_streamk_reset(gssd_stream_t stream);
int gssd_dcn_streamk_release(const void* out);

long long gssd_dcn_packed_weight_elems_x6(int Cout, int C);
int gssd_dcn_pack_weight_x6(const float* w_oihw, void* w_packed, int Cout, int C, int dg, gssd_stream_t stream);
int gssd_dcn_forward_x6(const float* x, const float* om, const void* w_packed, const float* bias, float* out, int B, int H, int W, int C,
                        int dg, int om_stride, int Cout, gssd_stream_t stream);
long long gssd_conv_patch_x6_weight_elems(int Cout, int C);
int gssd_conv_patch_x6_pack_weight(const float* w_packed, void* out, int Cout, int C, int row_stride, gssd_stream_t stream);
int gssd_conv_patch_x6_takes(const gssd_conv_desc* d);
int gssd_dcn_forward_x6_ex(const float* x, const float* om, const void* w_packed, const float* bias, float* out, int B, int H, int W, int C,
                           int dg, int om_stride, int Cout, int flags, gssd_stream_t stream);
long long gssd_dcn_packed_weight_elems_bf16(int Cout, int C);
int gssd_dcn_pack_weight_bf16(const float* w_oihw, void* w_packed, int Cout, int C, int dg, gssd_stream_t stream);
int gssd_dcn_forward_bf16(const void* x, const float* om, const void* w_packed, const float* bias, void* out, int B, int H, int W,
                          int C, int dg, int om_stride, int Cout, gssd_stream_t stream);

int gssd_dcn_col2im_f32(const float* x, const float* om, const float* dcols, float* dx, float* dom, int B, int H, int W,
                        int C, int dg, int om_stride, gssd_stream_t stream);

typedef struct gssd_dcn_geom {
    int32_t B, H, W, C, x_stride;
    int32_t Ho, Wo;
    int32_t kh, kw, sh, sw, ph, pw, dh, dw;
    int32_t dg;
    int32_t off_stride, mask_stride;
    int32_t mask_logit;
} gssd_dcn_geom;
int gssd_dcn_geo_im2col_f32(const float* x, const float* offset, const float* mask, float* cols, const gssd_dcn_geom* geom, int b0,
                            int b1, gssd_stream_t stream);
int gssd_dcn_geo_col2im_f32(const float* x, const float* offset, const float* mask, const float* dcols, float* dx, float* doffset,
                            float* dmask, const gssd_dcn_geom* geom, int b0, int b1, gssd_stream_t stream);

#define GSSD_FILTER_BILINEAR 2
#define GSSD_FILTER_BICUBIC 3

int gssd_resample_ksize(int in_size, int out_size, int filter);
int gssd_resample_coeffs(int in_size, int out_size, int filter, int32_t* bounds, int32_t* kk);

int gssd_resize_u8_horizontal(const uint8_t* in, uint8_t* out, const int32_t* bounds, const int32_t* kk, int ksize,
                              int n_img, int H, int W_in, int W_out, int C, gssd_stream_t stream);
int gssd_resize_u8_vertical(const uint8_t* in, uint8_t* out, const int32_t* bounds, const int32_t* kk, int ksize, int n_img,
                            int H_in, int H_out, int W, int C, int imgs_per_study, int32_t* minmax, gssd_stream_t stream);

int gssd_input_finish_f32(const uint8_t* img, const int32_t* minmax, float mean0, float mean1, float mean2, float* out_nchw,
                          int B, int phases, int S, int C, int normalize, gssd_stream_t stream);

typedef struct gssd_aug_desc {
    int64_t src;
    int64_t work;
    int32_t H, W;
    int32_t s_phase, s_chan, s_y, s_x;
    int32_t top, left;
    int32_t cy, cx, ch, cw;
    int32_t mirror;
    int32_t fill;
    float delta, alpha;
    int32_t hb, hk, hks;
    int32_t vb, vk, vks;
    int32_t row0, nrows;
} gssd_aug_desc;
int gssd_aug_desc_size(void);

int gssd_augment_minmax(const gssd_aug_desc* desc, int B, int max_rows, int p_only, int32_t* minmax, gssd_stream_t stream);
int gssd_augment_horizontal(const gssd_aug_desc* desc, const int32_t* minmax, const int32_t* table, float mean0, float mean1,
                            float mean2, uint8_t* work, int B, int max_rows, int max_cw, int size, int p_only, gssd_stream_t stream);
int gssd_augment_vertical(const gssd_aug_desc* desc, const int32_t* table, const uint8_t* work, float* out_nchw, int B, int size,
                          int p_only, gssd_stream_t stream);

int gssd_pixellink_targets(const float* boxes, const int32_t* offsets, int B, int size, int factor, int64_t* pixel_mask,
                           int64_t* neg_pixel_mask, float* pixel_pos_weight, int64_t* link_mask, gssd_stream_t stream);

int gssd_bgemm_f32(const float* A, const float* B, float* C, int M, int N, int K, int lda, int ldb, int ldc, int transA, int transB,
                   long long strideA, long long strideB, long long strideC, int batch, float alpha, int accumulate,
                   gssd_stream_t stream);
int gssd_bgemm_ex_f32(const float* A, const float* B, float* C, int M, int N, int K, int lda, int ldb, int ldc, int transA, int transB,
                      long long strideA, long long strideB, long long strideC, int batch, float alpha, int mode, const float* rowvec,
                      const float* aux, gssd_stream_t stream);
int gssd_rowdot_f32(const float* a, const float* b, float* out, int64_t rows, int C, gssd_stream_t stream);
int gssd_softmax_bwd_rows_f32(const float* attn, float* dattn, int64_t rows, int n, int row_stride, gssd_stream_t stream);
int gssd_sn_weight_grad_f32(const float* dw_eff, int ld_dw, const float* w_orig, const float* u, const float* v, const float* inv_sigma,
                            const float* scale, double* dot_scratch , float* dw_orig, int rows, int cols,
                            gssd_stream_t stream);
int gssd_scaled_transpose_f32(const float* w, const float* alpha, float* out, int rows, int cols, gssd_stream_t stream);
int gssd_cast_split_f32_bf16(const float* x, void* hi, void* lo, int64_t n, gssd_stream_t stream);
int gssd_cast_rows_f32_bf16(const float* x, void* y, int64_t rows, int cols, int ld_x, int ld_y, gssd_stream_t stream);
int gssd_transpose_cast_f32_bf16(const float* x, void* y, int64_t rows, int cols, int64_t ld_x, int64_t ld_y, gssd_stream_t stream);
int gssd_dot_f32(const float* a, const float* b, int64_t n, double* out, gssd_stream_t stream);
int gssd_axpby_f32(const float* x, const float* y, float* out, int64_t n, float a, float b, gssd_stream_t stream);
int gssd_scale_cast_f64_f32(const double* x, const float* scale, float* y, int n, gssd_stream_t stream);
int gssd_sa_sigma_grad_f32(const double* dot, const double* colsum, const float* bias, int C, float* dsigma, gssd_stream_t stream);


int gssd_match_batch(const float* targets, const int* gt_off, const float* priors, int B, int P,
                     float threshold, float var0, float var1, float* loc_t, int64_t* conf_t, gssd_stream_t stream);

int gssd_reduce_max_f32(const float* x, int64_t n, float* out, int out_n, gssd_stream_t stream);

int gssd_hnm_loss(const float* loc, const float* conf, const float* loc_t, const int64_t* conf_t, const float* xmax,
                  int xmax_n, int B, int P, int C, int negpos_ratio, uint8_t* sel, double* partial, float* loss_c_all,
                  gssd_stream_t stream);
int gssd_loss_finalize(const double* partial, int B, float* losses, double* n_total, gssd_stream_t stream);
int gssd_loss_finalize_global(const double* partial, int B, const double* n_global, int world, float* losses, double* n_total,
                              gssd_stream_t stream);
int gssd_loss_backward(const float* loc, const float* conf, const float* loc_t, const int64_t* conf_t,
                       const uint8_t* sel, const double* n_total, const float* grad_l, const float* grad_c, int B,
                       int P, int C, float* dloc, float* dconf, gssd_stream_t stream);

int gssd_detect(const float* loc, const float* conf, const float* priors, int B, int P, int C, int top_k,
                float conf_thresh, float nms_thresh, float var0, float var1, int conf_is_logits, int loc_is_boxes,
                float* out, int* keep_idx, int* keep_cnt, gssd_stream_t stream);

int gssd_softmax_lastdim_f32(const float* x, float* y, int64_t rows, int C, gssd_stream_t stream);


int gssd_eval_match(const float* det, long long img_stride, int N, int top_k, const float* scales, const double* gt,
                    const int* gt_off, int max_gt, double thresh, const double* thr, int n_iou, int n_iobb, float* conf_out,
                    uint8_t* flag_out, gssd_stream_t stream);

long long gssd_eval_workspace_bytes(int M);
int gssd_eval_ap(const float* conf, const uint8_t* flags, int M, int n_metrics, double npos, int use_07_metric, void* workspace,
                 long long workspace_bytes, double* ap_out, gssd_stream_t stream);

int gssd_heads_reduce_f32(const float* ws, const signed char* splits, float* out, int B, int P, int C, gssd_stream_t stream);


int gssd_interp_add_f32(const float* src, const float* addend, float* out, float* out2, int B, int Hs, int Ws, int Hd, int Wd, int C,
                        gssd_stream_t stream);

int gssd_pixellink_final_f32(const float* f0, const float* f1, const float* f2, const float* f3, int nf, const float* w1,
                             const float* b1, const float* w2, const float* b2, float* out1, float* out2, int B, int HW,
                             gssd_stream_t stream);

int gssd_pixellink_loss_f32(const float* out1, const float* out2, const long long* pixel_target, const unsigned char* neg_pixel_mask,
                            const float* pixel_pos_weight, const long long* link_target, double* per_image, float* neg_weight_out,
                            int B, int H, int W, int neg_pos_ratio, gssd_stream_t stream);

int gssd_interp_add_bwd_f32(const float* d_out, const float* d_out2, float* d_src, float* d_addend, int B, int Hs, int Ws, int Hd, int Wd,
                            int C, int ld, gssd_stream_t stream);
int gssd_pixellink_final_bwd_f32(const float* d_out1, const float* d_out2, const float* f0, const float* f1, const float* f2,
                                 const float* f3, int nf, const float* w1, const float* w2, float* g0, float* g1, float* g2, float* g3,
                                 int accumulate_mask, double* dw1, double* dw2, int B, int HW, int ld, gssd_stream_t stream);
int gssd_pixellink_loss_bwd_f32(const float* out1, const float* out2, const long long* pixel_target, const float* neg_weight,
                                const float* pixel_pos_weight, const long long* link_target, const double* per_image,
                                const float* upstream4, float* d_out1, float* d_out2, int B, int H, int W, gssd_stream_t stream);

int gssd_pixellink_decode_f32(const float* out1, const float* out2, int* labels, float* comps, int* ncomp, int B, int H, int W,
                              float pixel_thr, float link_thr, int max_comp, gssd_stream_t stream);

int gssd_pixellink_final5_f32(const float* f0, const float* f1, const float* f2, const float* f3, const float* f4, int nf, const float* w1,
                              const float* b1, const float* w2, const float* b2, float* out1, float* out2, int B, int HW, gssd_stream_t stream);
int gssd_pixellink_final5_bwd_f32(const float* d_out1, const float* d_out2, const float* f0, const float* f1, const float* f2, const float* f3,
                                  const float* f4, int nf, const float* w1, const float* w2, float* g0, float* g1, float* g2, float* g3,
                                  float* g4, int accumulate_mask, double* dw1, double* dw2, int B, int HW, int ld, gssd_stream_t stream);

int gssd_self_attn_flash_bwd_f32_supported(int D, int C2);
int gssd_self_attn_flash_bwd_f32(const float* tp, int qstride, const float* keys, int krow, const float* gT, int Nkp, const float* dag,
                                 const float* lse, const float* dvec, float* dq, int ld_q, float* dk, float* dv, int ld_kv, int B, int N, int Nk,
                                 int D, int C2, gssd_stream_t stream);

int gssd_self_attn_core_x6_supported(int D, int C2);
long long gssd_self_attn_core_x6_ws_bytes(int B, int N, int D, int C2);
int gssd_self_attn_core_x6_f32(const float* tp, const float* gT, float* out, int B, int N, int Np, int D, int C2, void* ws, float* lse,
                               gssd_stream_t stream);

#define GSSD_PLAN_LAUNCH 0
#define GSSD_PLAN_WAIT 1
#define GSSD_PLAN_MAX_ARGS 24
typedef struct gssd_plan_op {
    int kind;
    int fn;
    int stream;
    int nargs;
    uint64_t args[GSSD_PLAN_MAX_ARGS];
} gssd_plan_op;
int gssd_plan_fn_count(void);
const char* gssd_plan_fn_name(int index);
int gssd_plan_fn_index(const char* name);
int gssd_plan_fn_nargs(int index);
int gssd_plan_op_size(void);
int gssd_plan_run(const gssd_plan_op* ops, int n_ops, const gssd_stream_t* streams, int n_streams, int* failed_at);

int gssd_conv_wino_x6_takes(const gssd_conv_desc* d);
int gssd_conv_thin_x6_takes(const gssd_conv_desc* d);
int gssd_conv_thin_nchw3_takes(const gssd_conv_desc* d);

#ifdef __cplusplus
}
#endif
#endif
```

Baseline: 4641 img/s.

## Fuse SA projection into three-plane bf16 split and BN-ReLU into residual epilogue

The self-attention theta/phi/g projection conv gains an epilogue that writes the three-plane bf16 split (hi/mid/lo) straight into the flash-attention x6 workspace. This removes the separate f32 tp/gT buffers and the split pass inside the attention kernel, and a new attention entry point reads the planes directly. A RESID_XF flag also lets the output conv apply the deferred BN scale/shift+ReLU to the residual, so conv4_3's BN can stay deferred into the SA block. The costs are extra epilogue complexity, LDS staging for the transposed g planes, and more eligibility conditions. The split path only runs when the plan is built in no-grad mode.

```diff
diff --git a/grouped-ssd-pytorch_amd/gssd/_lib.py b/grouped-ssd-pytorch_amd/gssd/_lib.py
--- a/grouped-ssd-pytorch_amd/gssd/_lib.py
+++ b/grouped-ssd-pytorch_amd/gssd/_lib.py
@@ -46,7 +46,7 @@
 
 OUT_NHWC, OUT_TRANSPOSED, OUT_HEADS, OUT_SPLIT_T = 0, 1, 2, 3
 CONV_OUT_F32, CONV_OUTB_BF16_PERM32, CONV_HEADS_SLICES, CONV_POOL2, CONV_RESID_F32, CONV_F16_OK = 1, 2, 4, 8, 16, 32
-CONV_IN_NCHW3, CONV_OUT_GROUPCAT = 64, 128
+CONV_IN_NCHW3, CONV_OUT_GROUPCAT, CONV_OUT_X6PLANES, CONV_RESID_XF = 64, 128, 256, 512
 
 SIGNATURES = {
     'gssd_abi_version': (c_i, []),
@@ -132,6 +132,7 @@
     'gssd_self_attn_core_x6_supported': (c_i, [c_i, c_i]),
     'gssd_self_attn_core_x6_ws_bytes': (C.c_longlong, [c_i, c_i, c_i, c_i]),
     'gssd_self_attn_core_x6_f32': (c_i, [c_fp, c_fp, c_fp, c_i, c_i, c_i, c_i, c_i, c_fp, c_fp, c_fp]),
+    'gssd_self_attn_core_x6_planes_f32': (c_i, [c_fp, c_fp, c_i, c_i, c_i, c_i, c_fp, c_fp]),
     'gssd_self_attn_core_bf16v': (c_i, [c_fp, c_fp, c_fp, c_i, c_i, c_i, c_i, c_i, c_fp, c_fp]),
     'gssd_softmax_rows_f32': (c_i, [c_fp, c_i64, c_i, c_i, c_fp]),
     'gssd_slice_and_cat_f32': (c_i, [c_fp, c_fp, c_fp, c_i64, c_i, c_i, c_i, c_fp]),
diff --git a/grouped-ssd-pytorch_amd/gssd/csrc/conv_bf16.hip b/grouped-ssd-pytorch_amd/gssd/csrc/conv_bf16.hip
--- a/grouped-ssd-pytorch_amd/gssd/csrc/conv_bf16.hip
+++ b/grouped-ssd-pytorch_amd/gssd/csrc/conv_bf16.hip
@@ -484,7 +484,7 @@
     GSSD_CHECK_ARG(dp != nullptr);
     const gssd_conv_desc& d = *dp;
     GSSD_CHECK_ARG(d.in && d.wgt && d.out);
-    GSSD_CHECK_ARG(!(d.flags & (GSSD_CONV_IN_NCHW3 | GSSD_CONV_OUT_GROUPCAT)));
+    GSSD_CHECK_ARG(!(d.flags & (GSSD_CONV_IN_NCHW3 | GSSD_CONV_OUT_GROUPCAT | GSSD_CONV_OUT_X6PLANES | GSSD_CONV_RESID_XF)));
     GSSD_CHECK_ARG(d.B > 0 && d.H > 0 && d.W > 0 && d.Ho > 0 && d.Wo > 0);
     GSSD_CHECK_ARG(d.groups > 0 && d.Cout > 0 && d.Cout % d.groups == 0);
     GSSD_CHECK_ARG(d.cin_g > 0 && d.cin_g % 8 == 0 && d.in_stride % 8 == 0 && d.in_ch_off % 8 == 0);
diff --git a/grouped-ssd-pytorch_amd/gssd/csrc/conv_igemm.hip b/grouped-ssd-pytorch_amd/gssd/csrc/conv_igemm.hip
--- a/grouped-ssd-pytorch_amd/gssd/csrc/conv_igemm.hip
+++ b/grouped-ssd-pytorch_amd/gssd/csrc/conv_igemm.hip
@@ -380,6 +380,18 @@
         gssd_set_error("GSSD_CONV_OUT_GROUPCAT: csrc/conv_x6.hip does not take this descriptor (see gssd_conv_x6_takes)");
         return GSSD_EINVAL;
     }
+    if (d.flags & GSSD_CONV_RESID_XF) {
+        const int rc = d.wgt_x6 ? gssd_try_conv_x6(d, s) : 1;
+        if (rc != 1) return rc;
+        gssd_set_error("GSSD_CONV_RESID_XF: csrc/conv_x6.hip does not take this descriptor (see gssd_conv_x6_takes)");
+        return GSSD_EINVAL;
+    }
+    if (d.flags & GSSD_CONV_OUT_X6PLANES) {
+        const int rc = d.wgt_x6 ? gssd_try_conv_x6(d, s) : 1;
+        if (rc != 1) return rc;
+        gssd_set_error("GSSD_CONV_OUT_X6PLANES: csrc/conv_x6.hip does not take this descriptor (see gssd_conv_x6_takes)");
+        return GSSD_EINVAL;
+    }
     if (d.wgt_patch) {
         const int rc = gssd_try_conv_patch_x6(d, s);
         if (rc != 1) return rc;
diff --git a/grouped-ssd-pytorch_amd/gssd/csrc/conv_x6.hip b/grouped-ssd-pytorch_amd/gssd/csrc/conv_x6.hip
--- a/grouped-ssd-pytorch_amd/gssd/csrc/conv_x6.hip
+++ b/grouped-ssd-pytorch_amd/gssd/csrc/conv_x6.hip
@@ -321,7 +321,16 @@
                 }
             }
             if (p.resid) {
-                const f32x4 r0 = *reinterpret_cast<const f32x4*>(p.resid + ro), r1 = *reinterpret_cast<const f32x4*>(p.resid + ro + 4);
+                f32x4 r0 = *reinterpret_cast<const f32x4*>(p.resid + ro), r1 = *reinterpret_cast<const f32x4*>(p.resid + ro + 4);
+                if (p.flags & GSSD_CONV_RESID_XF) {
+                    const f32x4 s0 = *reinterpret_cast<const f32x4*>(p.in_scale + n), s1 = *reinterpret_cast<const f32x4*>(p.in_scale + n + 4);
+                    const f32x4 h0 = *reinterpret_cast<const f32x4*>(p.in_shift + n), h1 = *reinterpret_cast<const f32x4*>(p.in_shift + n + 4);
+#pragma unroll
+                    for (int c = 0; c < 4; ++c) {
+                        r0[c] = fmaxf(r0[c] * s0[c] + h0[c], 0.f);
+                        r1[c] = fmaxf(r1[c] * s1[c] + h1[c], 0.f);
+                    }
+                }
 #pragma unroll
                 for (int c = 0; c < 4; ++c) {
                     v[c] += r0[c];
@@ -716,6 +725,73 @@
     __syncthreads();
 #undef X6_LOADS_WAIT
 
+    if (p.flags & GSSD_CONV_OUT_X6PLANES) {
+        constexpr int SLD = BM + 4;
+        static_assert(BN * SLD * 4 <= K::LDS_BYTES, "the staging tile lives in the K loop's LDS");
+        float* const stg = reinterpret_cast<float*>(smem_h);
+        u16* const tpp = reinterpret_cast<u16*>(p.out);
+        u16* const gpl = reinterpret_cast<u16*>(p.out_b);
+        const long long tp_plane = (long long)M * p.split_n, g_plane = (long long)p.B * p.outb_batch_stride;
+        const bool g_range = n0g >= p.split_n;
+#pragma unroll
+        for (int u = 0; u < NT / 2; ++u) {
+            const int nl = wn * WTN + 32 * u + 8 * kq;
+            const int n = n0g + nl;
+            float bv[8], av[8];
+#pragma unroll
+            for (int c = 0; c < 8; ++c) {
+                bv[c] = p.bias ? p.bias[n + c] : 0.f;
+                av[c] = p.alpha ? p.alpha[n + c] : 1.f;
+            }
+#pragma unroll
+            for (int i = 0; i < MT; ++i) {
+                const int ml = wm * WTM + i * 16 + r, m = m0 + ml;
+                float v[8];
+#pragma unroll
+                for (int c = 0; c < 8; ++c) v[c] = acc[i][2 * u + (c >> 2)][c & 3] * av[c] + bv[c];
+                if (g_range) {
+#pragma unroll
+                    for (int c = 0; c < 8; ++c) stg[(nl + c) * SLD + ml] = v[c];
+                    continue;
+                }
+                if (m >= M) continue;
+                bf16x8 h8, m8, l8;
+#pragma unroll
+                for (int c = 0; c < 8; ++c) {
+                    __bf16 h, mm, l;
+                    split3(v[c], h, mm, l);
+                    h8[c] = h;
+                    m8[c] = mm;
+                    l8[c] = l;
+                }
+                u16* dst = tpp + (size_t)m * p.split_n + n;
+                *reinterpret_cast<bf16x8*>(dst) = h8;
+                *reinterpret_cast<bf16x8*>(dst + tp_plane) = m8;
+                *reinterpret_cast<bf16x8*>(dst + 2 * tp_plane) = l8;
+            }
+        }
+        if (g_range) {
+            __syncthreads();
+            for (int it = tid; it < BN * (BM / 4); it += 256) {
+                const int ch = it / (BM / 4), gr = it - ch * (BM / 4);
+                const int m = m0 + 4 * gr;
+                if (m >= M) continue;
+                const int bi = m / HoWo, ml = m - bi * HoWo;
+                const f32x4 v = *reinterpret_cast<const f32x4*>(stg + ch * SLD + 4 * gr);
+                __bf16 h[4], mm[4], l[4];
+#pragma unroll
+                for (int e = 0; e < 4; ++e) split3(v[e], h[e], mm[e], l[e]);
+                const int k = ml & 31;
+                u16* dst = gpl + (size_t)bi * p.outb_batch_stride + (size_t)(n0g - p.split_n + ch) * p.out_b_stride + (ml - k) +
+                           8 * ((k >> 2) & 3) + 4 * (k >> 4);
+                *reinterpret_cast<bf16x4*>(dst) = bf16x4{h[0], h[1], h[2], h[3]};
+                *reinterpret_cast<bf16x4*>(dst + g_plane) = bf16x4{mm[0], mm[1], mm[2], mm[3]};
+                *reinterpret_cast<bf16x4*>(dst + 2 * g_plane) = bf16x4{l[0], l[1], l[2], l[3]};
+            }
+        }
+        return;
+    }
+
     float* red = reinterpret_cast<float*>(smem_h);
     const float gate = p.gate ? *p.gate : 0.f;
     const bool split_t = p.out_mode == GSSD_OUT_SPLIT_T && n0g >= p.split_n;
@@ -763,7 +839,16 @@
                 }
             }
             if (p.resid) {
-                const f32x4 r0 = *reinterpret_cast<const f32x4*>(p.resid + ro), r1 = *reinterpret_cast<const f32x4*>(p.resid + ro + 4);
+                f32x4 r0 = *reinterpret_cast<const f32x4*>(p.resid + ro), r1 = *reinterpret_cast<const f32x4*>(p.resid + ro + 4);
+                if (p.flags & GSSD_CONV_RESID_XF) {
+                    const f32x4 s0 = *reinterpret_cast<const f32x4*>(p.in_scale + n), s1 = *reinterpret_cast<const f32x4*>(p.in_scale + n + 4);
+                    const f32x4 h0 = *reinterpret_cast<const f32x4*>(p.in_shift + n), h1 = *reinterpret_cast<const f32x4*>(p.in_shift + n + 4);
+#pragma unroll
+                    for (int c = 0; c < 4; ++c) {
+                        r0[c] = fmaxf(r0[c] * s0[c] + h0[c], 0.f);
+                        r1[c] = fmaxf(r1[c] * s1[c] + h1[c], 0.f);
+                    }
+                }
 #pragma unroll
                 for (int c = 0; c < 4; ++c) {
                     v[c] += r0[c];
@@ -844,7 +929,7 @@
     const int cout_g = d.Cout / d.groups;
     const int ntn = (cout_g + BN - 1) / BN, mtiles = (M + BM - 1) / BM;
     const long long plane = (long long)d.groups * ntn * BN * d.KH * d.KW * d.cin_g;
-    hipLaunchKernelGGL(kern, dim3((mtiles + 7) / 8 * 8 * d.groups * ntn), dim3(256), Cfg<BN>::LDS_BYTES + (d.in_scale ? 8 * d.cin_g : 0), stream, d, M, ntn, mtiles, plane);
+    hipLaunchKernelGGL(kern, dim3((mtiles + 7) / 8 * 8 * d.groups * ntn), dim3(256), Cfg<BN>::LDS_BYTES + ((d.in_scale && !(d.flags & GSSD_CONV_RESID_XF)) ? 8 * d.cin_g : 0), stream, d, M, ntn, mtiles, plane);
     GSSD_CHECK_LAUNCH();
     return GSSD_OK;
 }
@@ -859,7 +944,7 @@
     const int cout_g = d.Cout / d.groups;
     const int ntn = (cout_g + BN - 1) / BN, mtiles = (M + BM - 1) / BM;
     const long long plane = (long long)d.groups * ntn * BN * d.KH * d.KW * d.cin_g;
-    hipLaunchKernelGGL(kern, dim3((mtiles + 7) / 8 * 8 * d.groups * ntn), dim3(256), lds + (d.in_scale ? 8 * d.cin_g : 0), stream, d, M, ntn, mtiles, plane);
+    hipLaunchKernelGGL(kern, dim3((mtiles + 7) / 8 * 8 * d.groups * ntn), dim3(256), lds + ((d.in_scale && !(d.flags & GSSD_CONV_RESID_XF)) ? 8 * d.cin_g : 0), stream, d, M, ntn, mtiles, plane);
     GSSD_CHECK_LAUNCH();
     return GSSD_OK;
 }
@@ -869,6 +954,8 @@
     return launch2_impl<BN, XF, false>(d, M, stream);
 }
 #endif
+
+inline bool x6_in_xf(const gssd_conv_desc& d) { return d.in_scale && !(d.flags & GSSD_CONV_RESID_XF); }
 
 bool shape_ok(int cin_g, int cout_g, int groups) {
     return cin_g > 0 && cin_g % BKC == 0 && cout_g >= 32 && cout_g % 8 == 0 && groups > 0;
@@ -907,7 +994,7 @@
     const gssd_conv_desc& d = *dp;
     if (!d.wgt_x6 || d.groups <= 0 || d.Cout % d.groups != 0) return 0;
     if (!shape_ok(d.cin_g, d.Cout / d.groups, d.groups)) return 0;
-    if (d.split_k > 1 || (d.flags & ~(GSSD_CONV_OUT_F32 | GSSD_CONV_F16_OK | GSSD_CONV_OUT_GROUPCAT)) || (d.out2 && !d.gate)) return 0;
+    if (d.split_k > 1 || (d.flags & ~(GSSD_CONV_OUT_F32 | GSSD_CONV_F16_OK | GSSD_CONV_OUT_GROUPCAT | GSSD_CONV_OUT_X6PLANES | GSSD_CONV_RESID_XF)) || (d.out2 && !d.gate)) return 0;
     if (d.flags & GSSD_CONV_OUT_GROUPCAT) {
         if (d.out_mode != GSSD_OUT_NHWC || d.groups != 1 || d.m_per_image || d.relu || d.stats || d.split_n <= 0 || d.split_n % 8 != 0 ||
             d.Cout % d.split_n != 0 || d.out_stride < 2 * d.Cout)
@@ -916,7 +1003,14 @@
     if (d.out_mode == GSSD_OUT_SPLIT_T) {
         const int bn = gssd_conv_x6_tile(d.Cout / d.groups, d.groups, (long long)d.B * d.Ho * d.Wo);
         if (d.groups != 1 || !d.out_b || d.split_n <= 0 || d.split_n % bn != 0 || d.out_b_stride < d.Ho * d.Wo) return 0;
-    } else if (d.out_mode != GSSD_OUT_NHWC) {
+        if (d.flags & GSSD_CONV_OUT_X6PLANES) {
+            if (!X6_V2 || bn > 128 || d.Cout % bn != 0 || d.out_stride != d.split_n || d.out_ch_off != 0 || d.out_b_stride % 32 != 0 ||
+                (d.Ho * d.Wo) % 4 != 0 || d.outb_batch_stride != (long long)(d.Cout - d.split_n) * d.out_b_stride || d.relu || d.stats ||
+                d.gate || d.resid || d.out2 || ((uintptr_t)d.out_b % 16))
+                return 0;
+            if (d.m_per_image && d.out_batch_stride != (long long)d.Ho * d.Wo * d.out_stride) return 0;
+        }
+    } else if (d.out_mode != GSSD_OUT_NHWC || (d.flags & GSSD_CONV_OUT_X6PLANES)) {
         return 0;
     }
     if (d.m_per_image) {
@@ -925,10 +1019,15 @@
             return 0;
     }
     if ((d.resid && ((uintptr_t)d.resid % 16)) || (d.out2 && ((uintptr_t)d.out2 % 16))) return 0;
+    if (d.flags & GSSD_CONV_RESID_XF) {
+        if (!d.resid || !d.in_scale || !d.in_shift || d.out_mode != GSSD_OUT_NHWC || d.out_ch_off != 0 || ((uintptr_t)d.in_scale % 16) ||
+            ((uintptr_t)d.in_shift % 16))
+            return 0;
+    }
     if (d.in_stride % 4 || d.in_ch_off % 4 || d.out_stride % 4 || d.out_ch_off % 4) return 0;
     if (((uintptr_t)d.in % 16) || ((uintptr_t)d.out % 16) || ((uintptr_t)d.wgt_x6 % 16)) return 0;
     if ((long long)d.B * d.H * d.W * d.in_stride >= (1ll << 31)) return 0;
-    if (d.in_scale && d.cin_g > 512) return 0;
+    if (x6_in_xf(d) && d.cin_g > 512) return 0;
     return 1;
 }
 
@@ -938,12 +1037,12 @@
     const int M = (int)Mll;
     switch (gssd_conv_x6_tile(d.Cout / d.groups, d.groups, Mll)) {
 #if X6_V2
-        case 64: return d.in_scale ? launch2<64, true>(d, M, stream) : launch2<64, false>(d, M, stream);
-        case 128: return d.in_scale ? launch2<128, true>(d, M, stream) : launch2<128, false>(d, M, stream);
+        case 64: return x6_in_xf(d) ? launch2<64, true>(d, M, stream) : launch2<64, false>(d, M, stream);
+        case 128: return x6_in_xf(d) ? launch2<128, true>(d, M, stream) : launch2<128, false>(d, M, stream);
 #else
-        case 64: return d.in_scale ? launch<64, true>(d, M, stream) : launch<64, false>(d, M, stream);
-        case 128: return d.in_scale ? launch<128, true>(d, M, stream) : launch<128, false>(d, M, stream);
-#endif
-        default: return d.in_scale ? launch<256, true>(d, M, stream) : launch<256, false>(d, M, stream);
-    }
-}
+        case 64: return x6_in_xf(d) ? launch<64, true>(d, M, stream) : launch<64, false>(d, M, stream);
+        case 128: return x6_in_xf(d) ? launch<128, true>(d, M, stream) : launch<128, false>(d, M, stream);
+#endif
+        default: return x6_in_xf(d) ? launch<256, true>(d, M, stream) : launch<256, false>(d, M, stream);
+    }
+}
diff --git a/grouped-ssd-pytorch_amd/gssd/csrc/flash_attn_x6.hip b/grouped-ssd-pytorch_amd/gssd/csrc/flash_attn_x6.hip
--- a/grouped-ssd-pytorch_amd/gssd/csrc/flash_attn_x6.hip
+++ b/grouped-ssd-pytorch_amd/gssd/csrc/flash_attn_x6.hip
@@ -316,3 +316,18 @@
     if (f16) return N > 1024 ? launch_x6<64, 256, 32, 12, true>(tpp, gp, out, B, N, Np32, lse, s) : launch_x6<64, 256, 32, 4, true>(tpp, gp, out, B, N, Np32, lse, s);
     return N > 1024 ? launch_x6<64, 256, 32, 12, false>(tpp, gp, out, B, N, Np32, lse, s) : launch_x6<64, 256, 32, 4, false>(tpp, gp, out, B, N, Np32, lse, s);
 }
+
+extern "C" int gssd_self_attn_core_x6_planes_f32(const void* ws, float* out, int B, int N, int D, int C2, float* lse, gssd_stream_t stream) {
+    GSSD_CHECK_ARG(ws && out && B > 0 && N > 0);
+    GSSD_CHECK_ARG(((uintptr_t)out % 16) == 0 && ((uintptr_t)ws % 16) == 0);
+    GSSD_CHECK_ARG((long long)B * ((N + 63) / 64) < (1ll << 31));
+    if (!gssd_self_attn_core_x6_supported(D, C2)) {
+        gssd_set_error("self-attention core (three-plane): unsupported (theta/phi channels %d, g channels %d); built: (64,256)", D, C2);
+        return GSSD_EINVAL;
+    }
+    hipStream_t s = as_stream(stream);
+    const int Np32 = (int)round32(N);
+    const u16* tpp = reinterpret_cast<const u16*>(ws);
+    const u16* gp = tpp + NP * ((long long)B * N * 2 * D);
+    return N > 1024 ? launch_x6<64, 256, 32, 12, false>(tpp, gp, out, B, N, Np32, lse, s) : launch_x6<64, 256, 32, 4, false>(tpp, gp, out, B, N, Np32, lse, s);
+}
diff --git a/grouped-ssd-pytorch_amd/gssd/csrc/plan_run.hip b/grouped-ssd-pytorch_amd/gssd/csrc/plan_run.hip
--- a/grouped-ssd-pytorch_amd/gssd/csrc/plan_run.hip
+++ b/grouped-ssd-pytorch_amd/gssd/csrc/plan_run.hip
@@ -93,6 +93,7 @@
     GSSD_PLAN_FN(gssd_sa_unpool_f32),
     GSSD_PLAN_FN(gssd_self_attn_core_bf16v),
     GSSD_PLAN_FN(gssd_self_attn_core_x6_f32),
+    GSSD_PLAN_FN(gssd_self_attn_core_x6_planes_f32),
     GSSD_PLAN_FN(gssd_self_attn_flash_bwd_bf16),
     GSSD_PLAN_FN(gssd_softmax_rows_f32),
     GSSD_PLAN_FN(gssd_slice_and_cat_f32),
diff --git a/grouped-ssd-pytorch_amd/gssd/plan_common.py b/grouped-ssd-pytorch_amd/gssd/plan_common.py
--- a/grouped-ssd-pytorch_amd/gssd/plan_common.py
+++ b/grouped-ssd-pytorch_amd/gssd/plan_common.py
@@ -22,6 +22,9 @@
 USE_BRANCH_STREAMS = os.environ.get('GSSD_NO_BRANCH_STREAMS', '0') != '1'
 FUSE_PACK = os.environ.get('GSSD_FUSE_PACK', '1') != '0'
 FUSE_CAT = os.environ.get('GSSD_FUSE_CAT', '1') != '0'
+FUSE_SPLIT = os.environ.get('GSSD_FUSE_SPLIT', '1') != '0'
+FUSE_SA_BN = os.environ.get('GSSD_FUSE_SA_BN', '1') != '0'
+FUSE_HEAD_BN = os.environ.get('GSSD_FUSE_HEAD_BN', '1') != '0'
 SN_STREAM = 9
 ALL_STREAMS = -1
 
diff --git a/grouped-ssd-pytorch_amd/gssd/plan_graph.py b/grouped-ssd-pytorch_amd/gssd/plan_graph.py
--- a/grouped-ssd-pytorch_amd/gssd/plan_graph.py
+++ b/grouped-ssd-pytorch_amd/gssd/plan_graph.py
@@ -69,7 +69,7 @@
                 pool = (2, 2, 0, nxt == 'C')
             if last:
                 pool = (3, 1, 1, False)
-            defer = (pool is None and not is_conv4_3)
+            defer = (pool is None and not is_conv4_3) or (is_conv4_3 and self._sa_base_reads_raw(H, conv.out_channels))
             cur, H, Cc, xf = self._conv_bn(f'vgg.{vi}', conv, bn, cur, H, Cc, g, relu=True, pool=pool, in_xf=xf,
                                            defer_bn=defer)
             vi += 3
@@ -79,7 +79,8 @@
             i += 1
             if is_conv4_3:
                 x43 = cur
-                cur, H, Cc, src0 = self._after_conv4_3(cur, H, Cc)
+                cur, H, Cc, src0 = self._after_conv4_3(cur, H, Cc, xf)
+                xf = None
         vi += 1
         xf = None
         for li in range(2):
@@ -176,14 +177,19 @@
         self.steps[self._reduce_steps[0]].args[2] = loc.data_ptr()
         self.steps[self._reduce_steps[1]].args[2] = conf.data_ptr()
 
-    def _after_conv4_3(self, x, H, Cc):
+    def _sa_base_reads_raw(self, H, Cc):
+        net = self.eng.net
+        return bool(plan_common.FUSE_SA_BN and getattr(self, 'nograd', False) and not self.bf16 and not self.want_maps
+                    and net.use_self_attention_base and Cc <= 512 and (Cc // 4) % 64 == 0 and all(self._sa_on_x6(H, Cc)))
+
+    def _after_conv4_3(self, x, H, Cc, xf=None):
         net, B = self.eng.net, self.B
         attn_g, cat_g = None, 0
         if net.use_self_attention_base:
             cat_g = (net.groups_vgg if (plan_common.FUSE_CAT and getattr(self, 'nograd', False) and not self.bf16 and net.use_dcn
                                         and net.dcn_cat_sab) else 0)
             x, attn_g = self._self_attn('self_attn_base_list', 0, x, H, Cc, need_out2=bool(net.dcn_cat_sab), want_map=self.want_maps,
-                                        cat_groups=cat_g)
+                                        cat_groups=cat_g, in_xf=xf)
         if net.use_dcn:
             xin, Cin = x, Cc
             if net.dcn_cat_sab and cat_g and attn_g is None:
@@ -214,14 +220,18 @@
 
     def _branch(self, s, H, Cc, sa_i, fuse):
         net = self.eng.net
+        xf = None
         prev, self._sid = getattr(self, '_sid', 0), sa_i + 1
         if net.use_self_attention:
             s, _ = self._self_attn('self_attn_list', sa_i, s, H, Cc, need_out2=False, want_map=self.want_maps)
         if net.use_fuseconv and net.batch_norm:
             conv, bn = getattr(net, f'fuse_{fuse}'), getattr(net, f'bn_fuse_{fuse}')
-            s, H, Cc, _ = self._conv_bn(f'fuse_{fuse}', conv, bn, s, H, Cc, 1, relu=True)
+            defer = bool(plan_common.FUSE_HEAD_BN and getattr(self, 'nograd', False) and not self.bf16 and not self.want_maps
+                         and conv.out_channels <= 512)
+            s, H, Cc, xf = self._conv_bn(f'fuse_{fuse}', conv, bn, s, H, Cc, 1, relu=True, defer_bn=defer)
         elif net.use_fuseconv:
             s, H, Cc = self._conv_act(f'fuse_{fuse}', getattr(net, f'fuse_{fuse}'), s, H, Cc, 1)
-        self._head(sa_i, s, H, Cc)
+        self._head(sa_i, s, H, Cc, in_xf=xf)
         self._sid = prev
+        self.__dict__.setdefault('sources_xf', {})[sa_i] = xf
         return (s, H, Cc)
diff --git a/grouped-ssd-pytorch_amd/gssd/plan_ops.py b/grouped-ssd-pytorch_amd/gssd/plan_ops.py
--- a/grouped-ssd-pytorch_amd/gssd/plan_ops.py
+++ b/grouped-ssd-pytorch_amd/gssd/plan_ops.py
@@ -3,6 +3,7 @@
 import torch
 from . import _lib, ops
 from ._lib import lib
+from . import plan_common
 from .plan_common import DCN_X6, HEAD_OFF, MBOX, SN_STREAM, USE_CONV_X6, USE_FLASH_X6, USE_HEADS_WINO, USE_PATCH_X6, USE_WINOGRAD
 
 
@@ -27,7 +28,7 @@
                                           stride=s, pad=p, dil=dl, groups=groups)))
         return out, Ho, Cout
 
-    def _head(self, i, s, Hs, Cs):
+    def _head(self, i, s, Hs, Cs, in_xf=None):
         eng, net, B, dev, f32 = self.eng, self.eng.net, self.B, self.dev, torch.float32
         off = HEAD_OFF[i]
         A = MBOX[i]
@@ -64,6 +65,8 @@
                                      pad=1, bias=bp, out_mode=_lib.OUT_HEADS, out_b=None, split_n=nloc,
                                      out_batch_stride=self.P * 4, outb_batch_stride=self.P * self.nc,
                                      out_off=off * 4, outb_off=off * self.nc, split_k=split, wgt_wino=U,
+                                     in_scale=in_xf[0] if in_xf else None, in_shift=in_xf[1] if in_xf else None,
+                                     in_pad=in_xf[2] if in_xf else None,
                                      flags=_lib.CONV_OUT_F32 | (self.f16_ok if U is not None else 0))
         self.head_descs.append(d)
         self._add(self.conv_fn, (C.byref(d),), keep=d)
@@ -195,7 +198,13 @@
         self.rec.append(('pool', dict(x_in=x, out=out, H=H, C=Cc, k=k, s=s, p=p, Hp=Hp)))
         return out, Hp
 
-    def _self_attn(self, lst_name, idx, x, H, Cc, need_out2, want_map=False, cat_groups=0):
+    def _sa_on_x6(self, H, Cc):
+        M, C4, C2 = self.B * H * H, Cc // 4, Cc // 2
+        on = not self.bf16 and USE_CONV_X6
+        return (bool(on and ops.x6_wanted(1, Cc, C4 + C2, 1, M) and C4 % ops.x6_tile(C4 + C2, 1, M) == 0),
+                bool(on and ops.x6_wanted(1, C2, Cc, 1, M)))
+
+    def _self_attn(self, lst_name, idx, x, H, Cc, need_out2, want_map=False, cat_groups=0, in_xf=None):
         eng, B = self.eng, self.B
         sa = getattr(eng.net, lst_name)[idx]
         a_tpg, a_o = self.sa_state[(lst_name, idx)]
@@ -231,41 +240,57 @@
         w_tpg = eng._pack(name + '.tpg.w', build_w)
         b_tpg = eng._pack(name + '.tpg.b', build_b)
         w_o = eng._pack(name + '.o.w', build_wo) if self.bf16 else sa.snconv1x1_attn.weight_orig.detach().view(Cc, C2)
-        tp = self._buf(B, N, C4)
         if self.bf16:
             Np = ops.round_up(N, 32)
-            gT = self._abuf(B, C2, Np)
-        else:
-            gT = self._buf(B, C2, Np)
         ag = self._abuf(B, N, C2)
         out = self._abuf(B, H, H, Cc)
         out2 = self._abuf(B, H, H, Cc) if need_out2 else None
         mk = ops.make_conv_desc
         flat = not self.bf16 and N % 4 == 0 and Np == N
+        xin = dict(in_scale=in_xf[0], in_shift=in_xf[1], in_pad=in_xf[2]) if in_xf else {}
+        rxf = _lib.CONV_RESID_XF if in_xf else 0
+        tpg_on_x6, o_on_x6 = self._sa_on_x6(H, Cc)
         x6_tpg = None
-        if (not self.bf16 and USE_CONV_X6 and ops.x6_wanted(1, Cc, C4 + C2, 1, B * N) and C4 % ops.x6_tile(C4 + C2, 1, B * N) == 0):
+        if tpg_on_x6:
             def build_x6p(out, key=name + '.tpg.w', bn=ops.x6_tile(C4 + C2, 1, B * N)):
                 return ops.x6_weight(eng._packed[key], 1, Cc, 1, bn, out)
             x6_tpg = eng._pack(name + f'.tpg.x6@{ops.x6_tile(C4 + C2, 1, B * N)}', build_x6p)
-            gT.zero_()
-        d1, _, _ = mk(x, w_tpg, tp, B=B, H=H, W=H, in_stride=Cc, cin_g=Cc, Cout=C4 + C2, bias=b_tpg, alpha=a_tpg, wgt_x6=x6_tpg,
-                      out_mode=_lib.OUT_SPLIT_T, out_b=gT, split_n=C4, out_stride=C4, out_b_stride=Np, m_per_image=not flat,
-                      in_batch_stride=N * Cc, out_batch_stride=N * C4, outb_batch_stride=C2 * Np,
-                      flags=_lib.CONV_OUT_F32 | (_lib.CONV_OUTB_BF16_PERM32 if self.bf16 else self.f16_ok))
+        d1 = ws_planes = tp = gT = None
+        if (plan_common.FUSE_SPLIT and getattr(self, 'nograd', False) and not want_map and x6_tpg is not None and flat and C4 % 64 == 0
+                and max(H // int(sa.max_pool_factor), 1) == H and USE_FLASH_X6 and N >= 1024 and C8 == 64
+                and lib.gssd_self_attn_core_x6_supported(C8, C2) and os.environ.get('GSSD_FLASH_X6_F16', '0') != '1'):
+            Np32 = ops.round_up(N, 32)
+            ws = torch.zeros(int(lib.gssd_self_attn_core_x6_ws_bytes(B, N, C8, C2)) // 2, device=dev, dtype=torch.int16)
+            dp, _, _ = mk(x, w_tpg, ws, B=B, H=H, W=H, in_stride=Cc, cin_g=Cc, Cout=C4 + C2, bias=b_tpg, alpha=a_tpg, wgt_x6=x6_tpg,
+                          out_mode=_lib.OUT_SPLIT_T, out_b=ws[3 * B * N * C4:], split_n=C4, out_stride=C4, out_b_stride=Np32,
+                          in_batch_stride=N * Cc, out_batch_stride=N * C4, outb_batch_stride=C2 * Np32,
+                          flags=_lib.CONV_OUT_F32 | self.f16_ok | _lib.CONV_OUT_X6PLANES, **xin)
+            if lib.gssd_conv_x6_takes(C.byref(dp)) == 1:
+                d1, ws_planes = dp, ws
+                self.bufs.append(ws)
+        if d1 is None:
+            tp = self._buf(B, N, C4)
+            gT = self._abuf(B, C2, Np) if self.bf16 else self._buf(B, C2, Np)
+            if x6_tpg is not None:
+                gT.zero_()
+            d1, _, _ = mk(x, w_tpg, tp, B=B, H=H, W=H, in_stride=Cc, cin_g=Cc, Cout=C4 + C2, bias=b_tpg, alpha=a_tpg, wgt_x6=x6_tpg,
+                          out_mode=_lib.OUT_SPLIT_T, out_b=gT, split_n=C4, out_stride=C4, out_b_stride=Np, m_per_image=not flat,
+                          in_batch_stride=N * Cc, out_batch_stride=N * C4, outb_batch_stride=C2 * Np,
+                          flags=_lib.CONV_OUT_F32 | (_lib.CONV_OUTB_BF16_PERM32 if self.bf16 else self.f16_ok), **xin)
         x6_o = None
-        if not self.bf16 and USE_CONV_X6 and ops.x6_wanted(1, C2, Cc, 1, B * N):
+        if o_on_x6:
             def build_x6o(out, bn=ops.x6_tile(Cc, 1, B * N)):
                 return ops.x6_weight(sa.snconv1x1_attn.weight_orig.detach().view(Cc, C2), 1, C2, 1, bn, out)
             x6_o = eng._pack(name + f'.o.x6@{ops.x6_tile(Cc, 1, B * N)}', build_x6o)
         d5, _, _ = mk(ag, w_o, out, B=B, H=H, W=H, in_stride=C2, cin_g=C2, Cout=Cc, bias=sa.snconv1x1_attn.bias.detach(),
-                      alpha=a_o, gate=sa.sigma.detach(), resid=x, out2=out2, wgt_x6=x6_o, flags=self.f16_ok)
+                      alpha=a_o, gate=sa.sigma.detach(), resid=x, out2=out2, wgt_x6=x6_o, flags=self.f16_ok | rxf, **xin)
         xc = None
         if cat_groups and need_out2 and x6_o is not None and Cc % cat_groups == 0:
             ga = Cc // cat_groups
             xc = self._abuf(B, H, H, 2 * Cc)
             dc, _, _ = mk(ag, w_o, xc, B=B, H=H, W=H, in_stride=C2, cin_g=C2, Cout=Cc, bias=sa.snconv1x1_attn.bias.detach(),
                           alpha=a_o, gate=sa.sigma.detach(), resid=x, out2=xc.view(-1)[ga:], wgt_x6=x6_o, out_stride=2 * Cc, split_n=ga,
-                          flags=self.f16_ok | _lib.CONV_OUT_GROUPCAT)
+                          flags=self.f16_ok | _lib.CONV_OUT_GROUPCAT | rxf, **xin)
             if lib.gssd_conv_x6_takes(C.byref(dc)) == 1:
                 d5 = dc
                 self.bufs[:] = [t for t in self.bufs if t is not out and t is not out2]
@@ -275,6 +300,8 @@
                 self.bufs[:] = [t for t in self.bufs if t is not xc]
                 xc = None
         fn = self.conv_fn
+        if in_xf and (want_map or C4 % 64 != 0 or lib.gssd_conv_x6_takes(C.byref(d1)) != 1 or lib.gssd_conv_x6_takes(C.byref(d5)) != 1):
+            raise _lib.GssdError(f'{name}: the block was handed a raw input map, but csrc/conv_x6.hip does not take its projection and o conv')
         if C4 % 64 == 0:
             self._add(fn, (C.byref(d1),), keep=(d1, w_tpg, b_tpg))
         else:
@@ -303,6 +330,10 @@
             self._add(lib.gssd_self_attn_core_bf16v, (tp.data_ptr(), gT.data_ptr(), ag.data_ptr(), B, N, Np, C8, C2,
                                                       lse.data_ptr() if lse is not None else 0),
                       tag=(f'flash_attn_bf16v<{C8},{C2}>', 2.0 * B * N * N * (C8 + C2), B * (4.0 * N * C4 + 2.0 * C2 * Np + 2.0 * N * C2)))
+        elif ws_planes is not None:
+            self._add(lib.gssd_self_attn_core_x6_planes_f32, (ws_planes.data_ptr(), ag.data_ptr(), B, N, C8, C2,
+                                                              lse.data_ptr() if lse is not None else 0),
+                      tag=(f'flash_attn_x6<{C8},{C2}>', 2.0 * B * N * N * (C8 + C2), 2.0 * 3 * B * (N * C4 + C2 * Np) + 4.0 * B * N * C2))
         elif USE_FLASH_X6 and N >= 1024 and C8 == 64 and lib.gssd_self_attn_core_x6_supported(C8, C2):
             ws = self._buf(int(lib.gssd_self_attn_core_x6_ws_bytes(B, N, C8, C2)) // 4)
             self._add(lib.gssd_self_attn_core_x6_f32, (tp.data_ptr(), gT.data_ptr(), ag.data_ptr(), B, N, Np, C8, C2, ws.data_ptr(),
diff --git a/include/gssd_hip.h b/include/gssd_hip.h
--- a/include/gssd_hip.h
+++ b/include/gssd_hip.h
@@ -103,6 +103,8 @@
 #define GSSD_CONV_F16_OK 32
 #define GSSD_CONV_IN_NCHW3 64
 #define GSSD_CONV_OUT_GROUPCAT 128
+#define GSSD_CONV_OUT_X6PLANES 256
+#define GSSD_CONV_RESID_XF 512
 int gssd_conv2d_nhwc_bf16(const gssd_conv_desc* d, gssd_stream_t stream);
 int gssd_pack_conv_weight_bf16(const float* w_oihw, void* w_packed, int Cout, int cin_g, int KH, int KW, int cin_g_pad, int Kpad,
                                gssd_stream_t stream);
@@ -384,6 +386,7 @@
 long long gssd_self_attn_core_x6_ws_bytes(int B, int N, int D, int C2);
 int gssd_self_attn_core_x6_f32(const float* tp, const float* gT, float* out, int B, int N, int Np, int D, int C2, void* ws, float* lse,
                                gssd_stream_t stream);
+int gssd_self_attn_core_x6_planes_f32(const void* ws, float* out, int B, int N, int D, int C2, float* lse, gssd_stream_t stream);
 
 #define GSSD_PLAN_LAUNCH 0
 #define GSSD_PLAN_WAIT 1
```

Result: faster. 4729 img/s (median of 6 runs) (+1.9%).
